# EpicDuckPotato/stereo_vo

Measured on AMD Instinct MI355X. Metric: stereo frames/sec on 1241x376 KITTI pairs, higher is better.
Workload: dtype u8/f32/f64; 1 GPU; kitti_1241x376_1500corners_5kf_window (BASELINE configs[1]); streams_per_gpu=96, max_corners=1500, window=5, pipeline_groups=3, hardware_queues=4

## Files before the change

### include/svo.h

```cpp
#ifndef SVO_H_
#define SVO_H_

#include <stddef.h>
#include <stdint.h>

#ifdef __cplusplus
extern "C" {
#endif

typedef enum svo_status {
  SVO_OK = 0,
  SVO_ERR_INVALID = -1,
  SVO_ERR_HIP = -2,
  SVO_ERR_CAPACITY = -3,
  SVO_ERR_NO_DEVICE = -4,
  SVO_ERR_NUMERIC = -5
} svo_status;

typedef struct svo_camera_info {
  double focal, cx, cy;
  double k1, k2, p1, p2;
  double baseline;
} svo_camera_info;

// ... 297 lines not shown
int svo_ba_set_bulk_control(svo_ba* ba, int mode);
int svo_ba_last_stats(svo_ba* ba, svo_lm_stats* stats);
int svo_ba_wave_chunks_limit(void);
int svo_ba_set_wave_chunks(svo_ba* ba, int k);
int svo_ba_solve_forms(svo_ba* ba, long* counts, int n, long* gave_up);
int svo_ba_set_yield_iterations(svo_ba* ba, int n);
int svo_ba_solve_problem(svo_ba* ba, svo_ba_summary* summary);
int svo_ba_solve_problems(svo_ba** bas, int n, svo_ba_summary* summaries);
int svo_ba_read_problem(svo_ba* ba, double* poses7, double* points3);

typedef struct svo_pipeline svo_pipeline;
typedef struct svo_pipeline_params {
  svo_camera_info cam;
  int width, height;
  int max_corners;
  double quality;
  float min_feature_distance;
  float parallax_thresh;
  int window_size;
  int max_features;
  int ba_max_iterations;
  double ba_max_time_s;
} svo_pipeline_params;

typedef struct svo_frame_result {
  int n_detected, n_tracked, n_inliers, n_new;
  int is_keyframe;
  float av_parallax, percent_lost;
  double pose7[7];
  int ba_iterations;
} svo_frame_result;

void svo_pipeline_default_params(svo_pipeline_params* p);
int svo_pipeline_create(svo_ctx* ctx, svo_pipeline** out, const svo_pipeline_params* p);
void svo_pipeline_destroy(svo_pipeline* p);
int svo_pipeline_reset(svo_pipeline* p);
int svo_pipeline_process_batch_dev(svo_pipeline* p, const uint8_t* left, const uint8_t* right,
                                   int batch, svo_frame_result* results);
int svo_pipeline_process_batch(svo_pipeline* p, const uint8_t* left, const uint8_t* right,
                               int batch, svo_frame_result* results);
int svo_pipeline_set_rectification(svo_pipeline* p, const svo_rectify_eye* left, const svo_rectify_eye* right);
int svo_pipeline_set_keyframe_clouds(svo_pipeline* p, const svo_cloud_params* params, int max_keyframes_per_call);
int svo_pipeline_set_keyframe_speckle_filter(svo_pipeline* p, const svo_speckle_params* params);
int svo_pipeline_set_keyframe_lr_check(svo_pipeline* p, const svo_lr_check_params* params);
int svo_pipeline_set_keyframe_sgm(svo_pipeline* p, const svo_sgm_params* params);
typedef struct svo_keyframe_cloud {
  int frame;
  int lane;
  int n_total, n_stored;
  const svo_cloud_point* dev;
} svo_keyframe_cloud;
int svo_pipeline_keyframe_clouds(svo_pipeline* p, int* n, const svo_keyframe_cloud** table);
int svo_pipeline_copy_keyframe_cloud(svo_pipeline* p, int i, svo_cloud_point* host, int capacity);
int svo_pipeline_keyframe_disparity(svo_pipeline* p, int i, const int16_t** dev);
int svo_pipeline_copy_keyframe_disparity(svo_pipeline* p, int i, int16_t* host);
int svo_pipeline_get_tracked(svo_pipeline* p, int64_t* ids, float* xy, int capacity, int* n);

typedef struct svo_pipeline_group svo_pipeline_group;
int svo_pipeline_group_create(svo_ctx* ctx, svo_pipeline_group** out, const svo_pipeline_params* p, int n_lanes);
void svo_pipeline_group_destroy(svo_pipeline_group* g);
int svo_pipeline_group_reset(svo_pipeline_group* g);
int svo_pipeline_group_lanes(const svo_pipeline_group* g);
int svo_pipeline_group_process_batch_dev(svo_pipeline_group* g, const uint8_t* left, const uint8_t* right, size_t lane_stride,
                                         int batch, svo_frame_result* results);
int svo_pipeline_group_staging(svo_pipeline_group* g, int slot, uint8_t** left, uint8_t** right, size_t* lane_stride);
int svo_pipeline_group_upload(svo_pipeline_group* g, int slot, int batch);
int svo_pipeline_group_process_uploaded(svo_pipeline_group* g, int slot, svo_frame_result* results);
int svo_pipeline_group_process_batch(svo_pipeline_group* g, const uint8_t* left, const uint8_t* right, size_t lane_stride,
                                     int batch, svo_frame_result* results);
int svo_pipeline_group_set_rectification(svo_pipeline_group* g, int lane, const svo_rectify_eye* left, const svo_rectify_eye* right);
int svo_pipeline_group_set_keyframe_clouds(svo_pipeline_group* g, int lane, const svo_cloud_params* params, int max_keyframes_per_call);
int svo_pipeline_group_set_keyframe_speckle_filter(svo_pipeline_group* g, const svo_speckle_params* params);
int svo_pipeline_group_set_keyframe_lr_check(svo_pipeline_group* g, const svo_lr_check_params* params);
int svo_pipeline_group_set_keyframe_sgm(svo_pipeline_group* g, const svo_sgm_params* params);
int svo_pipeline_group_keyframe_clouds(svo_pipeline_group* g, int* n, const svo_keyframe_cloud** table);
int svo_pipeline_group_copy_keyframe_cloud(svo_pipeline_group* g, int i, svo_cloud_point* host, int capacity);
int svo_pipeline_group_keyframe_disparity(svo_pipeline_group* g, int i, const int16_t** dev);
int svo_pipeline_group_copy_keyframe_disparity(svo_pipeline_group* g, int i, int16_t* host);
int svo_pipeline_group_get_tracked(svo_pipeline_group* g, int lane, int64_t* ids, float* xy, int capacity, int* n);
int svo_pipeline_group_last_stats(const svo_pipeline_group* g, long* launches6, long* lanes6);
int svo_pipeline_group_solve_work(svo_pipeline_group* g, double* out4, int reset);
int svo_pipeline_group_solve_forms(svo_pipeline_group* g, long* counts, int n, long* gave_up);
int svo_pipeline_group_set_solve_yield(svo_pipeline_group* g, int n);

int svo_draw_track(const uint8_t* gray, int width, int height, int row_stride, const float* from_xy,
                   const float* to_xy, int n, uint8_t* rgb);
int svo_pipeline_draw_track(svo_pipeline* p, const uint8_t* keyframe_gray, int row_stride, uint8_t* rgb);

typedef struct svo_synth_params {
  uint64_t seed;
  int width, height;
  double focal, cx, cy, baseline;
  double step_z, step_x, yaw_per_frame;
  int n_billboards;
} svo_synth_params;
void svo_synth_default_params(svo_synth_params* p, int width, int height);
int svo_synth_render(const svo_synth_params* p, int frame, uint8_t* left, uint8_t* right);
int svo_synth_pose(const svo_synth_params* p, int frame, double* rt12);

int svo_image_read_gray(const char* path, uint8_t* buf, size_t capacity, int* width, int* height);
int svo_kitti_read_poses(const char* poses_file, double* rt12, int capacity_frames, int* n_frames);
int svo_ate_rmse(const double* est_xyz, const double* gt_xyz, int n, int with_scale, double* rmse);
typedef struct svo_run_stats {
  int frames, keyframes;
  double ate_rmse;
  double seconds;
} svo_run_stats;
int svo_kitti_run(svo_ctx* ctx, const svo_pipeline_params* params, const char* data_path, int sequence,
                  int max_frames, double* traj_rt12, svo_run_stats* stats);

#ifdef __cplusplus
}
#endif
#endif
```

### stereo_vo_amd/api.py

```python
import ctypes as C
import os

import numpy as np

_HERE = os.path.dirname(os.path.abspath(__file__))
_LIB = None


class SvoError(RuntimeError):
    pass


def lib_path():
    return os.path.join(_HERE, "libsvo_hip.so")


class Limits(C.Structure):
    _fields_ = [("max_width", C.c_int), ("max_height", C.c_int), ("max_batch", C.c_int),
                ("max_corners", C.c_int), ("max_candidates", C.c_int), ("max_features", C.c_int)]


class CameraInfo(C.Structure):
    _fields_ = [(n, C.c_double) for n in ("focal", "cx", "cy", "k1", "k2", "p1", "p2", "baseline")]

# ... 270 lines not shown
    return {n: getattr(c, n) for n in REFERENCE_CONSTANT_NAMES}


class LmStats(C.Structure):
    _fields_ = [("linearize_calls", C.c_int), ("step_calls", C.c_int), ("speculations", C.c_int), ("speculation_hits", C.c_int),
                ("single_exchange", C.c_int), ("collectives", C.c_int), ("device_control", C.c_int), ("fallbacks", C.c_int),
                ("host_us", C.c_double)]


class LmStepCtl(C.Structure):
    _fields_ = [("cost", C.c_double), ("mcc", C.c_double), ("decrease_factor", C.c_double), ("spec_radius", C.c_double),
                ("chain", C.c_int)]


LM_LINEARIZE_FN = C.CFUNCTYPE(C.c_int, C.c_void_p, C.c_double, C.c_int, C.POINTER(C.c_double))
LM_STEP_FN = C.CFUNCTYPE(C.c_int, C.c_void_p, C.POINTER(C.c_double), C.POINTER(C.c_double), C.c_double, C.POINTER(LmStepCtl),
                         C.POINTER(C.c_double), C.POINTER(C.c_double), C.POINTER(C.c_double), C.POINTER(C.c_int))
LM_ACCEPT_FN = C.CFUNCTYPE(C.c_int, C.c_void_p)


class LmOps(C.Structure):
    _fields_ = [("user", C.c_void_p), ("linearize", LM_LINEARIZE_FN), ("step", LM_STEP_FN), ("accept", LM_ACCEPT_FN)]


def lm_decide_step(cost, mcc, radius, decrease_factor, cost_new, model_change_points):
    acc, rad = C.c_int(0), C.c_double(0.0)
    lib().svo_lm_decide_step(C.c_double(cost), C.c_double(mcc), C.c_double(radius), C.c_double(decrease_factor), C.c_double(cost_new),
                             C.c_double(model_change_points), C.byref(acc), C.byref(rad))
    return bool(acc.value), rad.value


def lm_solve(poses7, linearize, step, accept, max_iterations=50, max_time_s=0.0):
    poses = np.ascontiguousarray(poses7, np.float64).copy()
    K = poses.shape[0]
    n = 6 * (K - 1)
    pay1 = n * n + 3 * n + 2

    def _lin(user, radius, first, out):
        np.ctypeslib.as_array(out, shape=(pay1,))[:] = linearize(radius, first)
        return 0

    def _step(user, dc, cand, radius, ctl, out2, out1, out_radius, out_at_cand):
        d = np.ctypeslib.as_array(dc, shape=(max(n, 1),))[:n].copy()
        c = np.ctypeslib.as_array(cand, shape=(K, 7)).copy()
        p2, p1, nr, at_cand = step(d, c, radius, ctl.contents)
        np.ctypeslib.as_array(out2, shape=(4,))[:] = p2
        if p1 is not None:
            np.ctypeslib.as_array(out1, shape=(pay1,))[:] = p1
        out_radius[0] = nr if p1 is not None else 0.0
        out_at_cand[0] = int(bool(at_cand))
        return 0

    def _acc(user):
        accept()
        return 0
    ops = LmOps(None, LM_LINEARIZE_FN(_lin), LM_STEP_FN(_step), LM_ACCEPT_FN(_acc))
    opt = ba_default_options()
    opt.max_iterations, opt.max_time_s = max_iterations, max_time_s
    s, st = BASummary(), LmStats()
    rc = lib().svo_lm_solve(K, _p(poses), C.byref(ops), C.byref(opt), C.byref(s), C.byref(st))
    if rc:
        raise SvoError(f"svo_lm_solve failed ({rc})")
    return poses, s, st


ALLREDUCE_FN = C.CFUNCTYPE(C.c_int, C.c_void_p, C.c_size_t, C.c_void_p)

SYMBOLS = [
    "svo_create", "svo_destroy", "svo_last_error", "svo_stream", "svo_sync", "svo_version", "svo_reference_constants",
    "svo_profile_select", "svo_profile_read", "svo_measure_peak",
    "svo_reproj_eval", "svo_reproj_eval_dev",
    "svo_corner_detect", "svo_corner_detect_batch_dev", "svo_corner_response",
    "svo_stereo_bm", "svo_stereo_disparity_at", "svo_stereo_disparity_at_dev",
    "svo_triangulate", "svo_lk_track", "svo_build_pyramid", "svo_track_features", "svo_dedup",
    "svo_pnp_ransac",
    "svo_ba_default_options", "svo_ba_create", "svo_ba_destroy", "svo_ba_reset", "svo_ba_add_keyframe", "svo_ba_solve",
    "svo_ba_get_pose", "svo_ba_window_count", "svo_ba_get_points", "svo_ba_load_problem",
    "svo_ba_set_allreduce", "svo_ba_set_device_lm", "svo_ba_set_bulk_control", "svo_ba_set_solve_form", "svo_ba_wave_chunks_limit", "svo_ba_set_wave_chunks", "svo_ba_set_yield_iterations", "svo_ba_solve_forms", "svo_ba_solve_problem", "svo_ba_solve_problems", "svo_ba_read_problem", "svo_ba_set_comm", "svo_ba_last_stats", "svo_lm_solve", "svo_lm_decide_step",
    "svo_rccl_unique_id", "svo_rccl_comm_create", "svo_rccl_comm_destroy",
    "svo_pipeline_default_params", "svo_pipeline_create", "svo_pipeline_destroy", "svo_pipeline_reset",
    "svo_pipeline_process_batch_dev", "svo_pipeline_process_batch", "svo_pipeline_get_tracked",
    "svo_pipeline_group_create", "svo_pipeline_group_destroy", "svo_pipeline_group_reset", "svo_pipeline_group_lanes",
    "svo_pipeline_group_process_batch_dev", "svo_pipeline_group_get_tracked", "svo_pipeline_group_last_stats",
    "svo_pipeline_group_solve_work", "svo_pipeline_group_solve_forms", "svo_pipeline_group_set_solve_yield", "svo_pipeline_group_staging", "svo_pipeline_group_upload", "svo_pipeline_group_process_uploaded", "svo_pipeline_group_process_batch",
    "svo_synth_default_params", "svo_synth_render", "svo_synth_pose",
    "svo_image_read_gray", "svo_kitti_read_poses", "svo_ate_rmse", "svo_kitti_run", "svo_cholesky_solve", "svo_cholesky_solve_dev", "svo_draw_track", "svo_pipeline_draw_track",
    "svo_rectify_eye_from_camera_info", "svo_rectify_build_map", "svo_rectify_remap", "svo_rectify_remap_batch_dev",
    "svo_pipeline_set_rectification", "svo_pipeline_group_set_rectification",
    "svo_stereo_bm_batch_dev", "svo_cloud_default_params", "svo_disparity_cloud_batch_dev", "svo_stereo_cloud",
    "svo_pipeline_set_keyframe_clouds", "svo_pipeline_keyframe_clouds", "svo_pipeline_copy_keyframe_cloud",
    "svo_pipeline_group_set_keyframe_clouds", "svo_pipeline_group_keyframe_clouds", "svo_pipeline_group_copy_keyframe_cloud",
    "svo_speckle_workspace_bytes", "svo_disparity_speckle_filter_batch_dev", "svo_disparity_speckle_filter",
    "svo_pipeline_set_keyframe_speckle_filter", "svo_pipeline_group_set_keyframe_speckle_filter",
    "svo_stereo_bm_cost_batch_dev", "svo_disparity_lr_check_batch_dev", "svo_disparity_lr_check",
    "svo_pipeline_set_keyframe_lr_check", "svo_pipeline_group_set_keyframe_lr_check",
    "svo_sgm_default_params", "svo_sgm_workspace_bytes", "svo_stereo_sgm_batch_dev", "svo_stereo_sgm",
    "svo_pipeline_set_keyframe_sgm", "svo_pipeline_group_set_keyframe_sgm",
    "svo_voxel_map_default_params", "svo_voxel_map_bytes", "svo_voxel_map_create", "svo_voxel_map_destroy", "svo_voxel_map_clear",
    "svo_voxel_map_insert_dev", "svo_pose7_to_cam_to_world", "svo_voxel_map_insert_pose7_dev", "svo_voxel_map_stats",
    "svo_voxel_map_extract_dev", "svo_voxel_map_extract", "svo_voxel_map_download",
    "svo_voxel_carve_default_params", "svo_voxel_map_carve_dev", "svo_pose7_to_world_to_cam", "svo_voxel_map_carve_pose7_dev",
    "svo_voxel_map_carve", "svo_voxel_map_copy_live_dev", "svo_pipeline_keyframe_disparity", "svo_pipeline_group_keyframe_disparity",
    "svo_pipeline_copy_keyframe_disparity", "svo_pipeline_group_copy_keyframe_disparity",
    "svo_voxel_render_default_params", "svo_voxel_render_workspace_bytes", "svo_voxel_map_render_dev", "svo_voxel_map_render_pose7_dev",
    "svo_voxel_map_render", "svo_voxel_render_set_mode",
    "svo_voxel_map_remove_dev", "svo_voxel_map_remove_pose7_dev", "svo_voxel_map_remove_sync", "svo_voxel_map_move_dev", "svo_voxel_map_move_pose7_dev",
    "svo_voxel_ledger_bytes", "svo_voxel_ledger_create", "svo_voxel_ledger_destroy", "svo_voxel_ledger_insert_pose7_dev",
    "svo_voxel_ledger_update_pose7", "svo_voxel_ledger_retire", "svo_voxel_ledger_remove", "svo_voxel_ledger_ids", "svo_voxel_ledger_get",
]


def lib():
    global _LIB
    if _LIB is None:
        p = lib_path()
        if not os.path.exists(p):
            raise SvoError(f"{p} not built — run `python -c 'import __graft_entry__ as g; g.build()'`")
        L = C.CDLL(p)
        L.svo_version.restype = C.c_char_p
        L.svo_last_error.restype = C.c_char_p
        L.svo_last_error.argtypes = [C.c_void_p]
        L.svo_stream.restype = C.c_void_p
        L.svo_stream.argtypes = [C.c_void_p]
        L.svo_destroy.argtypes = [C.c_void_p]
        L.svo_destroy.restype = None
        vp, ci, sz = C.c_void_p, C.c_int, C.c_size_t
        L.svo_cloud_default_params.argtypes = [vp, ci, ci]
        L.svo_stereo_bm_batch_dev.argtypes = [vp, vp, vp, ci, ci, ci, ci, sz, ci, ci, vp]
        L.svo_disparity_cloud_batch_dev.argtypes = [vp, vp, vp, ci, ci, ci, ci, sz, vp, vp, vp, vp, vp]
        L.svo_stereo_cloud.argtypes = [vp, vp, vp, ci, ci, ci, ci, ci, vp, vp, vp, vp, vp, vp]
        L.svo_pipeline_set_keyframe_clouds.argtypes = [vp, vp, ci]
        L.svo_pipeline_keyframe_clouds.argtypes = [vp, vp, vp]
        L.svo_pipeline_copy_keyframe_cloud.argtypes = [vp, ci, vp, ci]
        L.svo_pipeline_group_set_keyframe_clouds.argtypes = [vp, ci, vp, ci]
        L.svo_pipeline_group_keyframe_clouds.argtypes = [vp, vp, vp]
        L.svo_pipeline_group_copy_keyframe_cloud.argtypes = [vp, ci, vp, ci]
        for f in ("svo_cloud_default_params", "svo_stereo_bm_batch_dev", "svo_disparity_cloud_batch_dev", "svo_stereo_cloud",
                  "svo_pipeline_set_keyframe_clouds", "svo_pipeline_keyframe_clouds", "svo_pipeline_copy_keyframe_cloud",
                  "svo_pipeline_group_set_keyframe_clouds", "svo_pipeline_group_keyframe_clouds", "svo_pipeline_group_copy_keyframe_cloud"):
            getattr(L, f).restype = ci
        L.svo_speckle_workspace_bytes.argtypes = [ci, ci, ci]
        L.svo_speckle_workspace_bytes.restype = sz
        L.svo_disparity_speckle_filter_batch_dev.argtypes = [vp, vp, ci, ci, ci, vp, vp, sz, vp]
        L.svo_disparity_speckle_filter.argtypes = [vp, vp, ci, ci, vp, vp]
        L.svo_pipeline_set_keyframe_speckle_filter.argtypes = [vp, vp]
        L.svo_pipeline_group_set_keyframe_speckle_filter.argtypes = [vp, vp]
        for f in ("svo_disparity_speckle_filter_batch_dev", "svo_disparity_speckle_filter", "svo_pipeline_set_keyframe_speckle_filter",
                  "svo_pipeline_group_set_keyframe_speckle_filter"):
            getattr(L, f).restype = ci
        L.svo_stereo_bm_cost_batch_dev.argtypes = [vp, vp, vp, ci, ci, ci, ci, sz, ci, ci, vp, vp]
        L.svo_disparity_lr_check_batch_dev.argtypes = [vp, vp, vp, ci, ci, ci, vp, vp]
        L.svo_disparity_lr_check.argtypes = [vp, vp, vp, ci, ci, vp, vp]
        L.svo_pipeline_set_keyframe_lr_check.argtypes = [vp, vp]
        L.svo_pipeline_group_set_keyframe_lr_check.argtypes = [vp, vp]
        for f in ("svo_stereo_bm_cost_batch_dev", "svo_disparity_lr_check_batch_dev", "svo_disparity_lr_check",
                  "svo_pipeline_set_keyframe_lr_check", "svo_pipeline_group_set_keyframe_lr_check"):
            getattr(L, f).restype = ci
        L.svo_sgm_default_params.argtypes = [vp, ci]
        L.svo_sgm_workspace_bytes.argtypes = [ci, ci, ci, ci, ci]
        L.svo_sgm_workspace_bytes.restype = sz
        L.svo_stereo_sgm_batch_dev.argtypes = [vp, vp, vp, ci, ci, ci, ci, sz, ci, ci, vp, vp, sz, vp, vp]
        L.svo_stereo_sgm.argtypes = [vp, vp, vp, ci, ci, ci, ci, ci, vp, vp, vp]
        L.svo_pipeline_set_keyframe_sgm.argtypes = [vp, vp]
        L.svo_pipeline_group_set_keyframe_sgm.argtypes = [vp, vp]
        for f in ("svo_sgm_default_params", "svo_stereo_sgm_batch_dev", "svo_stereo_sgm", "svo_pipeline_set_keyframe_sgm",
                  "svo_pipeline_group_set_keyframe_sgm"):
            getattr(L, f).restype = ci
# ... 818 lines not shown

    def close(self):
        if self.h:
            self.L.svo_pipeline_group_destroy(self.h)
            self.h = C.c_void_p()

    def __del__(self):
        try:
            self.close()
        except Exception:
            pass

    def reset(self):
        self.ctx._chk(self.L.svo_pipeline_group_reset(self.h), "svo_pipeline_group_reset")

    def set_rectification(self, lane, left=None, right=None):
        self.L.svo_pipeline_group_set_rectification.argtypes = [C.c_void_p, C.c_int, C.c_void_p, C.c_void_p]
        self.ctx._chk(self.L.svo_pipeline_group_set_rectification(self.h, lane, _ref(left), _ref(right)), "svo_pipeline_group_set_rectification")

    def set_keyframe_clouds(self, lane=-1, params=None, max_keyframes_per_call=0):
        if params is True:
            params = cloud_default_params(self.prm.width, self.prm.height)
        self.ctx._chk(self.L.svo_pipeline_group_set_keyframe_clouds(self.h, lane, _ref(params), max_keyframes_per_call),
                      "svo_pipeline_group_set_keyframe_clouds")

    def process_batch_dev(self, left_ptr, right_ptr, lane_stride, batch):
        res = (FrameResult * (self.n_lanes * batch))()
        self.ctx._chk(self.L.svo_pipeline_group_process_batch_dev(self.h, C.c_void_p(left_ptr), C.c_void_p(right_ptr), C.c_size_t(lane_stride),
                                                                  batch, res), "svo_pipeline_group_process_batch_dev")
        self.last_raw = bytes(res)
        return [list(res[l * batch:(l + 1) * batch]) for l in range(self.n_lanes)]

    def staging(self, slot):
        lp, rp, stride = C.POINTER(C.c_uint8)(), C.POINTER(C.c_uint8)(), C.c_size_t(0)
        self.L.svo_pipeline_group_staging.argtypes = [C.c_void_p, C.c_int, C.c_void_p, C.c_void_p, C.c_void_p]
        self.ctx._chk(self.L.svo_pipeline_group_staging(self.h, slot, C.byref(lp), C.byref(rp), C.byref(stride)), "svo_pipeline_group_staging")
        h, w = self.prm.height, self.prm.width
        mb = stride.value // (h * w)
        shape = (self.n_lanes, mb, h, w)
        n = self.n_lanes * mb * h * w
        return (np.ctypeslib.as_array(lp, shape=(n,)).reshape(shape), np.ctypeslib.as_array(rp, shape=(n,)).reshape(shape))

    def upload(self, slot, batch):
        self.ctx._chk(self.L.svo_pipeline_group_upload(self.h, slot, batch), "svo_pipeline_group_upload")

    def process_uploaded(self, slot, batch):
        res = (FrameResult * (self.n_lanes * batch))()
        self.L.svo_pipeline_group_process_uploaded.argtypes = [C.c_void_p, C.c_int, C.c_void_p]
        self.ctx._chk(self.L.svo_pipeline_group_process_uploaded(self.h, slot, res), "svo_pipeline_group_process_uploaded")
        self.last_raw = bytes(res)
        return [list(res[l * batch:(l + 1) * batch]) for l in range(self.n_lanes)]

    def process_batch(self, left, right):
        left, right = _u8(left), _u8(right)
        batch = left.shape[1]
        res = (FrameResult * (self.n_lanes * batch))()
        self.L.svo_pipeline_group_process_batch.argtypes = [C.c_void_p, C.c_void_p, C.c_void_p, C.c_size_t, C.c_int, C.c_void_p]
        self.ctx._chk(self.L.svo_pipeline_group_process_batch(self.h, _p(left), _p(right), C.c_size_t(batch * left.shape[2] * left.shape[3]), batch, res),
                      "svo_pipeline_group_process_batch")
        self.last_raw = bytes(res)
        return [list(res[l * batch:(l + 1) * batch]) for l in range(self.n_lanes)]

    def get_tracked(self, lane, capacity=8192):
        ids = np.empty(capacity, np.int64)
        xy = np.empty((capacity, 2), np.float32)
        n = C.c_int(0)
        self.ctx._chk(self.L.svo_pipeline_group_get_tracked(self.h, lane, _p(ids), _p(xy), capacity, C.byref(n)), "svo_pipeline_group_get_tracked")
        return ids[:n.value].copy(), xy[:n.value].copy()

    def solve_work(self, reset=False):
        out = (C.c_double * 4)()
        self.ctx._chk(self.L.svo_pipeline_group_solve_work(self.h, out, int(reset)), "svo_pipeline_group_solve_work")
        return list(out)

    def solve_forms(self):
        n = self.L.svo_ba_wave_chunks_limit() + 1
        out, gu = (C.c_long * n)(), C.c_long(0)
        self.ctx._chk(self.L.svo_pipeline_group_solve_forms(self.h, out, n, C.byref(gu)), "svo_pipeline_group_solve_forms")
        return list(out), gu.value

    def set_solve_yield(self, n):
        self.ctx._chk(self.L.svo_pipeline_group_set_solve_yield(self.h, int(n)), "svo_pipeline_group_set_solve_yield")

    def solve_resumes(self):
        n = self.L.svo_ba_wave_chunks_limit() + 2
        out = (C.c_long * n)()
        self.ctx._chk(self.L.svo_pipeline_group_solve_forms(self.h, out, n, None), "svo_pipeline_group_solve_forms")
        return out[n - 1]

    def last_stats(self):
        a, b = (C.c_long * 6)(), (C.c_long * 6)()
        self.ctx._chk(self.L.svo_pipeline_group_last_stats(self.h, a, b), "svo_pipeline_group_last_stats")
        return {s: (a[i], b[i]) for i, s in enumerate(self.STAGES) if s != "unused"}


class RunStats(C.Structure):
    _fields_ = [("frames", C.c_int), ("keyframes", C.c_int), ("ate_rmse", C.c_double), ("seconds", C.c_double)]


def image_read_gray(path, max_pixels=1 << 24):
    buf = np.empty(max_pixels, np.uint8)
    w, h = C.c_int(0), C.c_int(0)
    rc = lib().svo_image_read_gray(path.encode(), _p(buf), C.c_size_t(max_pixels), C.byref(w), C.byref(h))
    if rc:
        raise SvoError(f"svo_image_read_gray({path}) rc={rc}")
    return buf[:w.value * h.value].reshape(h.value, w.value).copy()


def kitti_read_poses(path, max_frames=100000):
    rt = np.empty((max_frames, 12))
    n = C.c_int(0)
    rc = lib().svo_kitti_read_poses(path.encode(), _p(rt), max_frames, C.byref(n))
    if rc:
        raise SvoError(f"svo_kitti_read_poses({path}) rc={rc}")
    return rt[:n.value].reshape(-1, 3, 4).copy()


def ate_rmse(est_xyz, gt_xyz, with_scale=False):
    est_xyz, gt_xyz = _f64(est_xyz), _f64(gt_xyz)
    out = C.c_double(0)
    rc = lib().svo_ate_rmse(_p(est_xyz), _p(gt_xyz), est_xyz.shape[0], int(with_scale), C.byref(out))
    if rc:
        raise SvoError(f"svo_ate_rmse rc={rc}")
    return out.value


def kitti_run(ctx, params, data_path, sequence, max_frames):
    traj = np.zeros((max_frames, 12))
    st = RunStats()
    ctx._chk(lib().svo_kitti_run(ctx.h, C.byref(params), data_path.encode(), sequence, max_frames, _p(traj), C.byref(st)),
             "svo_kitti_run")
    return traj[:st.frames].reshape(-1, 3, 4).copy(), st


def cholesky_solve(A, b):
    A = np.array(A, np.float64, order="C")
    b = np.array(b, np.float64)
    rc = lib().svo_cholesky_solve(_p(A), _p(b), b.shape[0])
    if rc != 0:
        raise SvoError(f"svo_cholesky_solve rc={rc}")
    return b


def draw_track(gray, from_xy, to_xy):
    g = np.ascontiguousarray(gray, np.uint8)
    a = np.ascontiguousarray(from_xy, np.float32).reshape(-1, 2)
    b = np.ascontiguousarray(to_xy, np.float32).reshape(-1, 2)
    out = np.empty(g.shape + (3,), np.uint8)
    rc = lib().svo_draw_track(_p(g), g.shape[1], g.shape[0], g.shape[1], _p(a), _p(b), a.shape[0], _p(out))
    if rc:
        raise SvoError(f"svo_draw_track rc={rc}")
    return out
```

### stereo_vo_amd/csrc/corner.hip

```cpp
#include "common.h"

namespace {
constexpr int SEL_THREADS = 1024;
constexpr int SEL_MAX_ACCEPT = 16384;
constexpr int SEL_CAP_K = 12288;
constexpr int SEL_CAP_C = 8192;
constexpr int SEL_LDS_BYTES = SEL_CAP_K * 8 + SEL_CAP_C * 2 + SEL_CAP_K + SEL_CAP_K * 2;
constexpr int NC_STRIDE = 32;

__device__ __forceinline__ unsigned f32_key(float v) {
  const unsigned b = __float_as_uint(v);
  return (b & 0x80000000u) ? ~b : (b | 0x80000000u);
}
__device__ __forceinline__ float key_f32(unsigned k) {
  return __uint_as_float((k & 0x80000000u) ? (k & 0x7fffffffu) : ~k);
}
__device__ __forceinline__ unsigned pack_xy(int x, int y) { return ((unsigned)y << 16) | (unsigned)x; }
__device__ __forceinline__ int key_x(unsigned lo) { return (int)(lo & 0xFFFFu); }
__device__ __forceinline__ int key_y(unsigned lo) { return (int)(lo >> 16); }
template <typename T>
__device__ __forceinline__ T ld_l2(const T* p) { return __hip_atomic_load(p, __ATOMIC_RELAXED, __HIP_MEMORY_SCOPE_AGENT); }
template <typename T>
__device__ __forceinline__ void st_l2(T* p, T v) { __hip_atomic_store(p, v, __ATOMIC_RELAXED, __HIP_MEMORY_SCOPE_AGENT); }
}

namespace {
constexpr int RS_COLS = 62;
constexpr int RS_ROWS = 48;
constexpr int RS_PF = 3;

__device__ __forceinline__ int wave_from_lower(int v) { return __builtin_amdgcn_mov_dpp(v, 0x138, 0xf, 0xf, false); }
__device__ __forceinline__ int wave_from_upper(int v) { return __builtin_amdgcn_mov_dpp(v, 0x130, 0xf, 0xf, false); }
__device__ __forceinline__ float wave_from_lower(float v) { return __int_as_float(wave_from_lower(__float_as_int(v))); }
__device__ __forceinline__ float wave_from_upper(float v) { return __int_as_float(wave_from_upper(__float_as_int(v))); }
}

__global__ __launch_bounds__(256) void corner_response_kernel(const uint8_t* __restrict__ imgs, int W, int H,
                                                              int row_stride, size_t image_stride,
                                                              float* __restrict__ eig,
                                                              unsigned* __restrict__ maxkey) {
  const int b = blockIdx.z;
  const uint8_t* img = imgs + (size_t)b * image_stride;
  const int lane = threadIdx.x & 63;
  const int ncs = (W + RS_COLS - 1) / RS_COLS, nrs = (H + RS_ROWS - 1) / RS_ROWS;
  const int wid = blockIdx.x * 4 + __builtin_amdgcn_readfirstlane(threadIdx.x >> 6);
  if (wid >= ncs * nrs) return;
  const int cs = wid % ncs, rs = wid / ncs;
  const int x = cs * RS_COLS - 1 + lane;
  const int y0 = rs * RS_ROWS, y1 = min(y0 + RS_ROWS, H);
  const int xr = reflect101(x, W);
  const int xe = reflect101(lane == 0 ? x - 1 : x + 1, W);
  const bool edge = lane == 0 || lane == 63;
  const bool fix_lo = x == -1, fix_hi = x == W;
  const bool border_wave = cs == 0 || (cs + 1) * RS_COLS - 1 + 1 >= W;
  const double scale = 1.0 / (4.0 * 3.0 * 255.0);
  const float k1 = (float)(1.0 * scale), k0 = (float)(2.0 * scale);
  float* E = eig + (size_t)b * W * H;
  const bool out_lane = lane >= 1 && lane <= RS_COLS && x < W;

  const int j0 = y0 > 0 ? y0 - 1 : 0, j1 = y1 < H ? y1 : H - 1;
  auto load_row = [&](int py, int& c, int& e) {
    const uint8_t* row = img + (size_t)reflect101(py, H) * row_stride;
    c = row[xr];
    e = edge ? (int)row[xe] : 0;
  };
  auto row_terms = [&](int c, int e, float& rdx, float& rdy) {
    int l = wave_from_lower(c), r = wave_from_upper(c);
    if (lane == 0) l = e;
    if (lane == 63) r = e;
    rdx = (float)(r - l);
    rdy = (float)c * k0 + (float)(l + r) * k1;
  };
  const int p_first = j0 - 1;
  const int p_last = j1 + 1;
  unsigned lmax = 0u;
  auto emit = [&](int y, const double* top, const double* mid, const double* bot) {
    const float a = (float)((top[0] + mid[0]) + bot[0]) * 0.5f;
    const float bq = (float)((top[1] + mid[1]) + bot[1]);
    const float c = (float)((top[2] + mid[2]) + bot[2]) * 0.5f;
    const float d = a - c;
    const float e = (a + c) - sqrtf(d * d + bq * bq);
    if (out_lane) {
      E[(size_t)y * W + x] = e;
      const unsigned k = f32_key(e);
      lmax = k > lmax ? k : lmax;
    }
  };
  auto step = [&](int p, int& c, int& e, float& dxA, float& dyA, float& dxB, float& dyB, float& dxC, float& dyC, double* HA,
                  double* HB, double* HC) {
    const int cc = c, ee = e;
    if (p + RS_PF <= p_last) load_row(p + RS_PF, c, e);
    row_terms(cc, ee, dxC, dyC);
    const int j = p - 1;
    if (j < j0) return;
    const float dx = (dxA + dxC) * k1 + dxB * k0;
    const float dy = dyC - dyA;
    float xx = dx * dx, xy = dx * dy, yy = dy * dy;
    if (border_wave) {
      const int src = fix_lo ? lane + 2 : lane - 2;
      const float x2 = __shfl(xx, src), y2 = __shfl(xy, src), z2 = __shfl(yy, src);
      if (fix_lo || fix_hi) { xx = x2; xy = y2; yy = z2; }
    }
    HC[0] = ((double)wave_from_lower(xx) + (double)xx) + (double)wave_from_upper(xx);
    HC[1] = ((double)wave_from_lower(xy) + (double)xy) + (double)wave_from_upper(xy);
    HC[2] = ((double)wave_from_lower(yy) + (double)yy) + (double)wave_from_upper(yy);
    const int y = j - 1;
    if (y < y0) return;
    if (y == 0) emit(0, HC, HB, HC);
    else emit(y, HA, HB, HC);
  };
  int c0, e0, c1, e1, c2, e2;
  load_row(p_first, c0, e0); load_row(p_first + 1, c1, e1); load_row(p_first + 2, c2, e2);
  float dx0 = 0.f, dy0 = 0.f, dx1 = 0.f, dy1 = 0.f, dx2 = 0.f, dy2 = 0.f;
  double h0[3] = {0, 0, 0}, h1[3] = {0, 0, 0}, h2[3] = {0, 0, 0};
  int p = p_first;
  for (; p + 2 <= p_last; p += 3) {
    step(p, c0, e0, dx1, dy1, dx2, dy2, dx0, dy0, h1, h2, h0);
    step(p + 1, c1, e1, dx2, dy2, dx0, dy0, dx1, dy1, h2, h0, h1);
    step(p + 2, c2, e2, dx0, dy0, dx1, dy1, dx2, dy2, h0, h1, h2);
  }
  double hp[3] = {h1[0], h1[1], h1[2]}, hl[3] = {h2[0], h2[1], h2[2]};
  if (p <= p_last) {
    step(p, c0, e0, dx1, dy1, dx2, dy2, dx0, dy0, h1, h2, h0);
    for (int q = 0; q < 3; ++q) { hp[q] = h2[q]; hl[q] = h0[q]; }
    ++p;
    if (p <= p_last) {
      step(p, c1, e1, dx2, dy2, dx0, dy0, dx1, dy1, h2, h0, h1);
      for (int q = 0; q < 3; ++q) { hp[q] = h0[q]; hl[q] = h1[q]; }
    }
  }
  if (j1 == H - 1 && y1 == H && H - 1 >= y0) emit(H - 1, hp, hl, hp);
  for (int off = 32; off > 0; off >>= 1) {
    const unsigned o = __shfl_xor(lmax, off);
    lmax = o > lmax ? o : lmax;
  }
  if (lane == 0 && lmax) atomicMax(&maxkey[b], lmax);
}


constexpr int RN_HALO = 2, RN_COLS = 64 - 2 * RN_HALO;
constexpr int RN_BUF = 320;
constexpr int NC_RAW = 16;

__global__ __launch_bounds__(256) void corner_response_nms_kernel(const uint8_t* __restrict__ imgs, int W, int H, int row_stride,
                                                                  size_t image_stride, unsigned* __restrict__ maxkey, double quality,
                                                                  unsigned long long* __restrict__ raw, size_t raw_stride ,
                                                                  int* __restrict__ ncand, int* __restrict__ status) {
  __shared__ unsigned long long sBuf[4][RN_BUF];
  const int b = blockIdx.z;
  const uint8_t* img = imgs + (size_t)b * image_stride;
  const int lane = threadIdx.x & 63, wave = __builtin_amdgcn_readfirstlane(threadIdx.x >> 6);
  const int ncs = (W + RN_COLS - 1) / RN_COLS, nrs = (H + RS_ROWS - 1) / RS_ROWS;
  const int wid = blockIdx.x * 4 + wave;
  if (wid >= ncs * nrs) return;
  const int cs = wid % ncs, rs = wid / ncs;
  const int x = cs * RN_COLS - RN_HALO + lane;
  const int y0 = rs * RS_ROWS, y1 = min(y0 + RS_ROWS, H);
  const int ey0 = y0 > 0 ? y0 - 1 : 0, ey1 = y1 < H ? y1 + 1 : H;
  const int xr = reflect101(x, W);
  const int xe = reflect101(lane == 0 ? x - 1 : x + 1, W);
  const bool edge = lane == 0 || lane == 63;
  const bool fix_lo = x == -1, fix_hi = x == W;
  const bool border_wave = cs == 0 || cs * RN_COLS - RN_HALO + 63 >= W;
  const double scale = 1.0 / (4.0 * 3.0 * 255.0);
  const float k1 = (float)(1.0 * scale), k0 = (float)(2.0 * scale);
  const bool test_lane = lane >= RN_HALO && lane < RN_HALO + RN_COLS && x >= 1 && x <= W - 2;
  unsigned long long* list = raw + (size_t)b * raw_stride;
  int* count = &ncand[b * NC_STRIDE + NC_RAW];
  unsigned long long* buf = sBuf[wave];
  int nbuf = 0;
  auto flush = [&]() {
    if (nbuf == 0) return;
    __builtin_amdgcn_fence(__ATOMIC_RELEASE, "workgroup");
    __builtin_amdgcn_wave_barrier();
    __builtin_amdgcn_fence(__ATOMIC_ACQUIRE, "workgroup");
    int base = 0;
    if (lane == 0) base = atomicAdd(count, nbuf);
    base = __builtin_amdgcn_readfirstlane(base);
    for (int i = lane; i < nbuf; i += 64) {
      if ((size_t)(base + i) < raw_stride) list[base + i] = buf[i];
      else atomicOr(status, 8);
    }
    __builtin_amdgcn_fence(__ATOMIC_RELEASE, "workgroup");
    __builtin_amdgcn_wave_barrier();
    __builtin_amdgcn_fence(__ATOMIC_ACQUIRE, "workgroup");
    nbuf = 0;
  };

  const int j0 = ey0 > 0 ? ey0 - 1 : 0, j1 = ey1 < H ? ey1 : H - 1;
  auto load_row = [&](int py, int& c, int& e) {
    const uint8_t* row = img + (size_t)reflect101(py, H) * row_stride;
    c = row[xr];
    e = edge ? (int)row[xe] : 0;
  };
  auto row_terms = [&](int c, int e, float& rdx, float& rdy) {
    int l = wave_from_lower(c), r = wave_from_upper(c);
    if (lane == 0) l = e;
    if (lane == 63) r = e;
    rdx = (float)(r - l);
    rdy = (float)c * k0 + (float)(l + r) * k1;
  };
  const int p_first = j0 - 1, p_last = j1 + 1;
  unsigned lmax = 0u;
  float thr_lb = (float)((double)key_f32(ld_l2(&maxkey[b])) * quality);
  if (!(thr_lb >= 0.0f)) thr_lb = 0.0f;
  float eA = 0.f, eB = 0.f;
  auto emit = [&](int y, const double* top, const double* mid, const double* bot) {
    const float a = (float)((top[0] + mid[0]) + bot[0]) * 0.5f;
    const float bq = (float)((top[1] + mid[1]) + bot[1]);
    const float c = (float)((top[2] + mid[2]) + bot[2]) * 0.5f;
    const float d = a - c;
    const float e = (a + c) - sqrtf(d * d + bq * bq);
    if (lane >= 1 && lane <= 62 && x >= 0 && x < W && y >= y0 && y < y1) {
      if (lane >= RN_HALO && lane < RN_HALO + RN_COLS) { const unsigned k = f32_key(e); lmax = k > lmax ? k : lmax; }
    }
    const int yt = y - 1;
    if (yt >= y0 && yt < y1 && yt >= 1 && yt <= H - 2) {
      const float m0 = fmaxf(fmaxf(wave_from_lower(eA), eA), wave_from_upper(eA));
      const float m2 = fmaxf(fmaxf(wave_from_lower(e), e), wave_from_upper(e));
      const float m1 = fmaxf(wave_from_lower(eB), wave_from_upper(eB));
      const bool cand = test_lane && eB > thr_lb && eB >= fmaxf(fmaxf(m0, m1), m2);
      const unsigned long long mask = __ballot(cand);
      if (mask) {
        if (cand) buf[nbuf + __popcll(mask & ((1ull << lane) - 1ull))] = ((unsigned long long)f32_key(eB) << 32) | pack_xy(x, yt);
        nbuf += __popcll(mask);
        if (nbuf > RN_BUF - 64) {
          flush();
          unsigned wm = lmax;
          for (int off = 32; off > 0; off >>= 1) { const unsigned o = __shfl_xor(wm, off); wm = o > wm ? o : wm; }
          const unsigned gm = ld_l2(&maxkey[b]);
          const float lb = (float)((double)key_f32(gm > wm ? gm : wm) * quality);
          if (lb > thr_lb) thr_lb = lb;
        }
      }
    }
    eA = eB; eB = e;
  };
  auto step = [&](int p, int& c, int& e, float& dxA, float& dyA, float& dxB, float& dyB, float& dxC, float& dyC, double* HA,
                  double* HB, double* HC) {
    const int cc = c, ee = e;
    if (p + RS_PF <= p_last) load_row(p + RS_PF, c, e);
    row_terms(cc, ee, dxC, dyC);
    const int j = p - 1;
    if (j < j0) return;
    const float dx = (dxA + dxC) * k1 + dxB * k0;
    const float dy = dyC - dyA;
    float xx = dx * dx, xy = dx * dy, yy = dy * dy;
    if (border_wave) {
      const int src = fix_lo ? lane + 2 : lane - 2;
      const float x2 = __shfl(xx, src), y2 = __shfl(xy, src), z2 = __shfl(yy, src);
      if (fix_lo || fix_hi) { xx = x2; xy = y2; yy = z2; }
    }
    HC[0] = ((double)wave_from_lower(xx) + (double)xx) + (double)wave_from_upper(xx);
    HC[1] = ((double)wave_from_lower(xy) + (double)xy) + (double)wave_from_upper(xy);
    HC[2] = ((double)wave_from_lower(yy) + (double)yy) + (double)wave_from_upper(yy);
    const int y = j - 1;
    if (y < ey0) return;
    if (y == 0) emit(0, HC, HB, HC);
    else emit(y, HA, HB, HC);
  };
  int c0, e0, c1, e1, c2, e2;
  load_row(p_first, c0, e0); load_row(p_first + 1, c1, e1); load_row(p_first + 2, c2, e2);
  float dx0 = 0.f, dy0 = 0.f, dx1 = 0.f, dy1 = 0.f, dx2 = 0.f, dy2 = 0.f;
  double h0[3] = {0, 0, 0}, h1[3] = {0, 0, 0}, h2[3] = {0, 0, 0};
  int p = p_first;
  for (; p + 2 <= p_last; p += 3) {
    step(p, c0, e0, dx1, dy1, dx2, dy2, dx0, dy0, h1, h2, h0);
    step(p + 1, c1, e1, dx2, dy2, dx0, dy0, dx1, dy1, h2, h0, h1);
    step(p + 2, c2, e2, dx0, dy0, dx1, dy1, dx2, dy2, h0, h1, h2);
  }
  double hp[3] = {h1[0], h1[1], h1[2]}, hl[3] = {h2[0], h2[1], h2[2]};
  if (p <= p_last) {
    step(p, c0, e0, dx1, dy1, dx2, dy2, dx0, dy0, h1, h2, h0);
    for (int q = 0; q < 3; ++q) { hp[q] = h2[q]; hl[q] = h0[q]; }
    ++p;
    if (p <= p_last) {
      step(p, c1, e1, dx2, dy2, dx0, dy0, dx1, dy1, h2, h0, h1);
      for (int q = 0; q < 3; ++q) { hp[q] = h0[q]; hl[q] = h1[q]; }
    }
  }
  if (j1 == H - 1 && ey1 == H && H - 1 >= ey0) emit(H - 1, hp, hl, hp);
  flush();
  for (int off = 32; off > 0; off >>= 1) {
    const unsigned o = __shfl_xor(lmax, off);
    lmax = o > lmax ? o : lmax;
  }
  if (lane == 0 && lmax) atomicMax(&maxkey[b], lmax);
}

__global__ __launch_bounds__(256) void corner_threshold_kernel(const unsigned long long* __restrict__ raw, size_t raw_stride,
                                                               const unsigned* __restrict__ maxkey, double quality,
                                                               unsigned long long* __restrict__ cand, int* __restrict__ ncand, int cap,
                                                               int* __restrict__ status) {
  const int b = blockIdx.z;
  const int n = min(ncand[b * NC_STRIDE + NC_RAW], (int)raw_stride);
  const float thr = (float)((double)key_f32(maxkey[b]) * quality);
  __shared__ int sCount, sBase;
  for (int i0 = blockIdx.x * 256; i0 < n; i0 += gridDim.x * 256) {
    if (threadIdx.x == 0) sCount = 0;
    __syncthreads();
    const int i = i0 + (int)threadIdx.x;
    unsigned long long e = 0;
    bool keep = false;
    if (i < n) {
      e = raw[(size_t)b * raw_stride + i];
      keep = key_f32((unsigned)(e >> 32)) > thr;
    }
    int local = 0;
    if (keep) local = atomicAdd(&sCount, 1);
    __syncthreads();
    if (threadIdx.x == 0 && sCount > 0) sBase = atomicAdd(&ncand[b * NC_STRIDE], sCount);
    __syncthreads();
    if (keep) {
      const int pos = sBase + local;
      if (pos < cap) cand[(size_t)b * cap + pos] = e;
      else atomicOr(status, 1);
    }
    __syncthreads();
  }
}

constexpr int NMS_ROWS = 8;
__global__ __launch_bounds__(256) void corner_nms_kernel(const float* __restrict__ eig, int W, int H,
                                                         const unsigned* __restrict__ maxkey, double quality,
                                                         unsigned long long* __restrict__ cand,
                                                         int* __restrict__ ncand, int cap, int* __restrict__ status) {
  const int b = blockIdx.z;
  const float* E = eig + (size_t)b * W * H;
  const float maxv = key_f32(maxkey[b]);
  const float thr = (float)((double)maxv * quality);
  const int x = blockIdx.x * 64 + (threadIdx.x & 63);
  const int yb = blockIdx.y * (4 * NMS_ROWS) + (threadIdx.x >> 6);
  __shared__ int sCount, sBase;
  if (threadIdx.x == 0) sCount = 0;
  __syncthreads();
  float val[NMS_ROWS];
  unsigned found = 0u;
#pragma unroll
  for (int k = 0; k < NMS_ROWS; ++k) {
    const int y = yb + 4 * k;
    val[k] = 0.f;
    if (x < 1 || x > W - 2 || y < 1 || y > H - 2) continue;
    const float c = E[(size_t)y * W + x];
    const float v = c > thr ? c : 0.0f;
    if (v == 0.0f) continue;
    float m = v;
#pragma unroll
    for (int j = -1; j <= 1; ++j)
#pragma unroll
      for (int i = -1; i <= 1; ++i) {
        const float nv = E[(size_t)(y + j) * W + (x + i)];
        const float t = nv > thr ? nv : 0.0f;
        m = t > m ? t : m;
      }
    if (v == m) { val[k] = v; found |= 1u << k; }
  }
  int local = 0;
  if (found) local = atomicAdd(&sCount, __popc(found));
  __syncthreads();
  if (threadIdx.x == 0 && sCount > 0) sBase = atomicAdd(&ncand[b * NC_STRIDE], sCount);
  __syncthreads();
  if (found) {
    int pos = sBase + local;
#pragma unroll
    for (int k = 0; k < NMS_ROWS; ++k) {
      if (!((found >> k) & 1u)) continue;
      if (pos < cap)
        cand[(size_t)b * cap + pos] = ((unsigned long long)f32_key(val[k]) << 32) | pack_xy(x, yb + 4 * k);
      else
        atomicOr(status, 1);
      ++pos;
    }
  }
}

__global__ __launch_bounds__(SEL_THREADS) void corner_select_kernel(
    const unsigned long long* __restrict__ cand, const int* __restrict__ ncand, int cap, int W, int H,
    float min_distance, int max_corners, int* __restrict__ cell_count, int* __restrict__ cell_start, int max_cells,
    unsigned long long* __restrict__ sorted, uint8_t* __restrict__ state_g, float* __restrict__ out_xy,
    int* __restrict__ out_n, int* __restrict__ status) {
  extern __shared__ __align__(16) unsigned char lds_raw[];
  unsigned long long* sKeys = reinterpret_cast<unsigned long long*>(lds_raw);
  __shared__ int sPart[SEL_THREADS];
  __shared__ int sFlag, sCount;
  const int b = blockIdx.x, tid = threadIdx.x;
  const unsigned long long* C = cand + (size_t)b * cap;
  int n = ncand[b * NC_STRIDE];
  if (n > cap) n = cap;
  float* oxy = out_xy + (size_t)b * max_corners * 2;
  if (min_distance < 1.0f) {
    if (n > SEL_MAX_ACCEPT) { if (tid == 0) { atomicOr(status, 2); out_n[b] = 0; } return; }
    int np2 = 1; while (np2 < n) np2 <<= 1;
    for (int i = tid; i < np2; i += SEL_THREADS) sKeys[i] = i < n ? C[i] : 0ull;
    __syncthreads();
    for (int k = 2; k <= np2; k <<= 1)
      for (int j = k >> 1; j > 0; j >>= 1) {
        for (int i = tid; i < np2; i += SEL_THREADS) {
          const int l = i ^ j;
          if (l > i) {
            const unsigned long long a = sKeys[i], c = sKeys[l];
            const bool desc = (i & k) == 0;
            if (desc ? a < c : a > c) { sKeys[i] = c; sKeys[l] = a; }
          }
        }
        __syncthreads();
      }
    const int m = n < max_corners ? n : max_corners;
    for (int i = tid; i < m; i += SEL_THREADS) {
      const unsigned idx = (unsigned)(sKeys[i] & 0xffffffffu);
      oxy[2 * i] = (float)key_x(idx); oxy[2 * i + 1] = (float)key_y(idx);
    }
    if (tid == 0) out_n[b] = m;
    return;
  }
  const int cell = (int)rintf(min_distance);
  const int gw = (W + cell - 1) / cell, gh = (H + cell - 1) / cell;
  const int ncell = gw * gh;
  int* cc = cell_count + (size_t)b * max_cells;
  int* cs = cell_start + (size_t)b * (max_cells + 1);
  unsigned long long* S = sorted + (size_t)b * cap;
  uint8_t* st = state_g + (size_t)b * cap;
  if (ncell > max_cells) { if (tid == 0) { atomicOr(status, 4); out_n[b] = 0; } return; }
  unsigned long long* keysL = reinterpret_cast<unsigned long long*>(lds_raw);
  unsigned short* cellL = reinterpret_cast<unsigned short*>(lds_raw + (size_t)SEL_CAP_K * 8);
  uint8_t* stateL = lds_raw + (size_t)SEL_CAP_K * 8 + (size_t)SEL_CAP_C * 2;
  unsigned short* blkL = reinterpret_cast<unsigned short*>(lds_raw + (size_t)SEL_CAP_K * 8 + (size_t)SEL_CAP_C * 2 + SEL_CAP_K);
  const bool use_lds = n <= SEL_CAP_K && ncell + 1 <= SEL_CAP_C;
  if (use_lds) {
    static_assert(3 * SEL_CAP_K >= 4 * SEL_CAP_C, "the cell counters must fit the state + blocker arrays");
    int* cntL = reinterpret_cast<int*>(stateL);
    for (int i = tid; i < ncell; i += SEL_THREADS) cntL[i] = 0;
    __syncthreads();
    for (int i = tid; i < n; i += SEL_THREADS) {
      const unsigned idx = (unsigned)(C[i] & 0xffffffffu);
      atomicAdd(&cntL[(key_y(idx) / cell) * gw + key_x(idx) / cell], 1);
    }
    __syncthreads();
    {
      const int chunk = (ncell + SEL_THREADS - 1) / SEL_THREADS;
      const int lo = tid * chunk, hi = (lo + chunk < ncell) ? lo + chunk : ncell;
      int s = 0;
      for (int i = lo; i < hi; ++i) s += cntL[i];
      sPart[tid] = s;
      __syncthreads();
      for (int off = 1; off < SEL_THREADS; off <<= 1) {
        int v = tid >= off ? sPart[tid - off] : 0;
        __syncthreads();
        sPart[tid] += v;
        __syncthreads();
      }
      int run = sPart[tid] - s;
      for (int i = lo; i < hi; ++i) { cellL[i] = (unsigned short)run; run += cntL[i]; }
      if (tid == 0) cellL[ncell] = (unsigned short)n;
    }
    __syncthreads();
    for (int i = tid; i < n; i += SEL_THREADS) {
      const unsigned long long k = C[i];
      const unsigned idx = (unsigned)(k & 0xffffffffu);
      const int cid = (key_y(idx) / cell) * gw + key_x(idx) / cell;
      const int slot = atomicSub(&cntL[cid], 1) - 1;
      keysL[(int)cellL[cid] + slot] = k;
    }
    __syncthreads();
    for (int i = tid; i < n; i += SEL_THREADS) { stateL[i] = 0; blkL[i] = 0xFFFFu; }
    __syncthreads();
  } else {
  for (int i = tid; i < ncell; i += SEL_THREADS) st_l2(&cc[i], 0);
  __syncthreads();
// ... 100 lines not shown
      for (int yy = y1; yy <= y2 && !rejected; ++yy) {
        const int p0 = CELL(yy * gw + x1), p1 = CELL(yy * gw + x2 + 1);
        for (int p = p0; p < p1; ++p) {
          const unsigned long long km = KEY(p);
          if (km <= k) continue;
          const unsigned im = (unsigned)(km & 0xffffffffu);
          const float dx = (float)(x - key_x(im)), dy = (float)(y - key_y(im));
          if (!(dx * dx + dy * dy < md2)) continue;
          const uint8_t sm = STATE(p);
          if (sm == 1) { rejected = true; break; }
          if (sm == 0) blocked = true;
        }
      }
      if (rejected) SET_STATE(i, (uint8_t)2);
      else if (!blocked) SET_STATE(i, (uint8_t)1);
      else pending = 1;
    }
    }
    }
    if (pending) sFlag = 1;
    __syncthreads();
    const int again = sFlag;
    __syncthreads();
    if (!again) break;
  }
  if (tid == 0) sCount = 0;
  __syncthreads();
  int A, np2 = 1;
  if (use_lds) {
    constexpr int PER = SEL_CAP_K / SEL_THREADS;
    unsigned long long mine[PER];
    int cnt = 0;
#pragma unroll
    for (int r = 0; r < PER; ++r) {
      const int i = tid + r * SEL_THREADS;
      const bool acc = i < n && stateL[i] == 1;
      mine[r] = acc ? keysL[i] : 0ull;
      cnt += acc;
    }
    __syncthreads();
    int pos = cnt ? atomicAdd(&sCount, cnt) : 0;
    __syncthreads();
    A = sCount;
    while (np2 < A) np2 <<= 1;
#pragma unroll
    for (int r = 0; r < PER; ++r) if (mine[r]) sKeys[pos++] = mine[r];
    for (int i = A + tid; i < np2; i += SEL_THREADS) sKeys[i] = 0ull;
    __syncthreads();
  } else {
    unsigned long long* Cw = const_cast<unsigned long long*>(C);
    for (int i = tid; i < n; i += SEL_THREADS) {
      if (STATE(i) == 1) {
        const int p = atomicAdd(&sCount, 1);
        if (p < SEL_MAX_ACCEPT) st_l2(&Cw[p], KEY(i));
      }
    }
    __syncthreads();
    A = sCount;
    if (A > SEL_MAX_ACCEPT) { if (tid == 0) { atomicOr(status, 2); out_n[b] = 0; } return; }
    while (np2 < A) np2 <<= 1;
    for (int i = tid; i < np2; i += SEL_THREADS) sKeys[i] = i < A ? ld_l2(&Cw[i]) : 0ull;
    __syncthreads();
  }
  for (int k = 2; k <= np2; k <<= 1)
    for (int j = k >> 1; j > 0; j >>= 1) {
      for (int i = tid; i < np2; i += SEL_THREADS) {
        const int l = i ^ j;
        if (l > i) {
          const unsigned long long a = sKeys[i], c = sKeys[l];
          const bool desc = (i & k) == 0;
          if (desc ? a < c : a > c) { sKeys[i] = c; sKeys[l] = a; }
        }
      }
      __syncthreads();
    }
  const int m = A < max_corners ? A : max_corners;
  for (int i = tid; i < m; i += SEL_THREADS) {
    const unsigned idx = (unsigned)(sKeys[i] & 0xffffffffu);
    oxy[2 * i] = (float)key_x(idx); oxy[2 * i + 1] = (float)key_y(idx);
  }
  if (tid == 0) out_n[b] = m;
}

static int corner_launch(svo_ctx* ctx, const uint8_t* imgs, int batch, int W, int H, int row_stride,
                         size_t image_stride, int max_corners, double quality, double min_distance,
                         float* xy, int* n) {
  SVO_REQUIRE(ctx, W <= 65535 && H <= 65535, "corner_detect: image sides above 65535 (candidate keys pack y << 16 | x)");
  hipStream_t st = ctx->stream;
  SVO_HIP_CHECK(ctx, hipMemsetAsync(ctx->d_maxkey, 0, sizeof(unsigned) * batch, st));
  SVO_HIP_CHECK(ctx, hipMemsetAsync(ctx->d_ncand, 0, sizeof(int) * NC_STRIDE * batch, st));
  static const bool two_pass = [] { const char* e = getenv("SVO_CORNER_TWO_PASS"); return e && *e && atoi(e) != 0; }();
  if (two_pass) {
    { const int rce = svo_ensure_eig(ctx, (size_t)ctx->lim.max_batch); if (rce) return rce; }
    {
      SvoProfScope prof(ctx, SVO_PROF_CORNER_RESPONSE);
      hipLaunchKernelGGL(corner_response_kernel, dim3(svo_div_up(svo_div_up(W, RS_COLS) * svo_div_up(H, RS_ROWS), 4), 1, batch), dim3(256), 0, st,
                         imgs, W, H, row_stride, image_stride, ctx->d_eig, ctx->d_maxkey);
    }
    SvoProfScope prof(ctx, SVO_PROF_CORNER_NMS);
    hipLaunchKernelGGL(corner_nms_kernel, dim3(svo_div_up(W, 64), svo_div_up(H, 4 * NMS_ROWS), batch), dim3(256), 0, st,
                       ctx->d_eig, W, H, ctx->d_maxkey, quality, ctx->d_cand, ctx->d_ncand, ctx->lim.max_candidates,
                       ctx->d_status);
  } else {
    unsigned long long* raw = ctx->d_raw;
    const size_t raw_stride = ctx->raw_cap;
    {
      SvoProfScope prof(ctx, SVO_PROF_CORNER_RESPONSE);
      hipLaunchKernelGGL(corner_response_nms_kernel, dim3(svo_div_up(svo_div_up(W, RN_COLS) * svo_div_up(H, RS_ROWS), 4), 1, batch), dim3(256), 0, st,
                         imgs, W, H, row_stride, image_stride, ctx->d_maxkey, quality, raw, raw_stride, ctx->d_ncand, ctx->d_status);
    }
    SvoProfScope prof(ctx, SVO_PROF_CORNER_NMS);
    hipLaunchKernelGGL(corner_threshold_kernel, dim3(32, 1, batch), dim3(256), 0, st, raw, raw_stride, ctx->d_maxkey, quality, ctx->d_cand,
                       ctx->d_ncand, ctx->lim.max_candidates, ctx->d_status);
  }
  static bool attr_set = false;
  if (!attr_set) {
    SVO_HIP_CHECK(ctx, hipFuncSetAttribute((const void*)corner_select_kernel,
                                           hipFuncAttributeMaxDynamicSharedMemorySize, SEL_LDS_BYTES));
    attr_set = true;
  }
  SvoProfScope ps(ctx, SVO_PROF_CORNER_SELECT);
  hipLaunchKernelGGL(corner_select_kernel, dim3(batch), dim3(SEL_THREADS), SEL_LDS_BYTES, st, ctx->d_cand,
                     ctx->d_ncand, ctx->lim.max_candidates, W, H, (float)min_distance, max_corners,
                     ctx->d_cell_count, ctx->d_cell_start, ctx->max_cells, ctx->d_sorted, ctx->d_state, xy, n,
                     ctx->d_status);
  SVO_HIP_CHECK(ctx, hipGetLastError());
  return SVO_OK;
}

static int corner_check_args(svo_ctx* ctx, const void* img, int batch, int W, int H, int row_stride,
                             int max_corners, const void* xy, const void* n) {
  if (!ctx) return SVO_ERR_INVALID;
  svo_use_device(ctx);
  SVO_REQUIRE(ctx, img && xy && n, "corner_detect: null buffer");
  SVO_REQUIRE(ctx, W >= 3 && H >= 3 && W <= ctx->lim.max_width && H <= ctx->lim.max_height && row_stride >= W,
              "corner_detect: image size outside the limits given to svo_create");
  SVO_REQUIRE(ctx, batch >= 1 && batch <= ctx->lim.max_batch, "corner_detect: batch outside limits");
  SVO_REQUIRE(ctx, max_corners >= 1, "corner_detect: max_corners must be >= 1");
  return SVO_OK;
}

static int corner_status(svo_ctx* ctx) {
  int* h = (int*)ctx->h_pinned;
  SVO_HIP_CHECK(ctx, hipMemcpyAsync(h, ctx->d_status, sizeof(int), hipMemcpyDeviceToHost, ctx->stream));
  SVO_HIP_CHECK(ctx, hipStreamSynchronize(ctx->stream));
  if (*h) {
    const int s = *h;
    (void)hipMemsetAsync(ctx->d_status, 0, sizeof(int), ctx->stream);
    ctx->err = (s & 1)   ? "corner_detect: more NMS candidates than svo_limits.max_candidates"
               : (s & 8) ? "corner_detect: more raw local maxima than the streaming pass's list holds (svo_ctx raw_cap: width x height / 4 per image under a 1 GiB budget)"
               : (s & 2) ? "corner_detect: more accepted corners than the select kernel holds (16384)"
                         : "corner_detect: min-distance grid larger than the workspace";
    return SVO_ERR_CAPACITY;
  }
  return SVO_OK;
}

extern "C" int svo_corner_detect_batch_dev(svo_ctx* ctx, const uint8_t* imgs, int batch, int width, int height,
                                           int row_stride, size_t image_stride, int max_corners, double quality,
                                           double min_distance, float* xy, int* n) {
  int rc = corner_check_args(ctx, imgs, batch, width, height, row_stride, max_corners, xy, n);
  if (rc) return rc;
  return corner_launch(ctx, imgs, batch, width, height, row_stride, image_stride, max_corners, quality,
                       min_distance, xy, n);
}

extern "C" int svo_corner_detect(svo_ctx* ctx, const uint8_t* img, int width, int height, int row_stride,
                                 int max_corners, double quality, double min_distance, float* xy, int* n) {
  int rc = corner_check_args(ctx, img, 1, width, height, row_stride, max_corners, xy, n);
  if (rc) return rc;
  SvoScratch s(ctx);
  uint8_t* d_img = s.take<uint8_t>((size_t)width * height);
  float* d_xy = s.take<float>(2 * (size_t)max_corners);
  int* d_n = s.take<int>(1);
  if (!d_img || !d_xy || !d_n) { ctx->err = "corner_detect: workspace too small"; return SVO_ERR_CAPACITY; }
  hipStream_t st = ctx->stream;
  SVO_HIP_CHECK(ctx, hipMemcpy2DAsync(d_img, width, img, row_stride, width, height, hipMemcpyHostToDevice, st));
  rc = corner_launch(ctx, d_img, 1, width, height, width, (size_t)width * height, max_corners, quality,
                     min_distance, d_xy, d_n);
  if (rc) return rc;
  SVO_HIP_CHECK(ctx, hipMemcpyAsync(n, d_n, sizeof(int), hipMemcpyDeviceToHost, st));
  rc = corner_status(ctx);
  if (rc) return rc;
  if (*n > 0) SVO_HIP_CHECK(ctx, hipMemcpy(xy, d_xy, sizeof(float) * 2 * (size_t)*n, hipMemcpyDeviceToHost));
  return SVO_OK;
}

extern "C" int svo_corner_response(svo_ctx* ctx, const uint8_t* img, int width, int height, int row_stride,
                                   float* eig) {
  if (!ctx) return SVO_ERR_INVALID;
  svo_use_device(ctx);
  SVO_REQUIRE(ctx, img && eig, "corner_response: null buffer");
  SVO_REQUIRE(ctx, width >= 3 && height >= 3 && width <= ctx->lim.max_width && height <= ctx->lim.max_height,
              "corner_response: image size outside limits");
  SvoScratch s(ctx);
  uint8_t* d_img = s.take<uint8_t>((size_t)width * height);
  if (!d_img) { ctx->err = "corner_response: workspace too small"; return SVO_ERR_CAPACITY; }
  hipStream_t st = ctx->stream;
  SVO_HIP_CHECK(ctx, hipMemcpy2DAsync(d_img, width, img, row_stride, width, height, hipMemcpyHostToDevice, st));
  { const int rce = svo_ensure_eig(ctx, 1); if (rce) return rce; }
  SVO_HIP_CHECK(ctx, hipMemsetAsync(ctx->d_maxkey, 0, sizeof(unsigned), st));
  hipLaunchKernelGGL(corner_response_kernel, dim3(svo_div_up(svo_div_up(width, RS_COLS) * svo_div_up(height, RS_ROWS), 4), 1, 1), dim3(256), 0,
                     st, d_img, width, height, width, (size_t)width * height, ctx->d_eig, ctx->d_maxkey);
  SVO_HIP_CHECK(ctx, hipGetLastError());
  SVO_HIP_CHECK(ctx, hipMemcpyAsync(eig, ctx->d_eig, sizeof(float) * (size_t)width * height, hipMemcpyDeviceToHost, st));
  SVO_HIP_CHECK(ctx, hipStreamSynchronize(st));
  return SVO_OK;
}
```

### stereo_vo_amd/csrc/kernels.h

```cpp
#ifndef SVO_KERNELS_H_
#define SVO_KERNELS_H_
#include "common.h"

struct SvoMat4 { float m[16]; };

SvoMat4 svo_k_reprojection_matrix(const float* pose16, float focal, float cx, float cy, float baseline);
SvoMat4 svo_k_reprojection_q(float focal, float cx, float cy, float baseline);
int svo_k_triangulate(svo_ctx* ctx, const float* xy, const float* disp, const int* n_dev, int n_max,
                      const SvoMat4& M, float* kept_xy, float* xyz, int* kept_index, int* n_kept,
                      const SvoPublish* pub = nullptr);
int svo_k_stereo_triangulate(svo_ctx* ctx, const uint8_t* left, const uint8_t* right, int width, int height, int row_stride,
                             int num_disparities, int block_size, const float* xy, const int* n_dev, int n_max, float* disp,
                             const SvoMat4& M, float* kept_xy, float* xyz, int* kept_index, int* n_kept, int word, SvoPublish* pub_out);
int svo_k_dedup(svo_ctx* ctx, const float* det_xy, const int* n_det_dev, int n_det_max, const float* trk_xy,
                const int* n_trk_dev, int n_trk_max, float min_distance, float* kept_xy, int* n_kept);
size_t svo_k_pyramid_bytes(int w, int h);
int svo_k_build_pyramid(svo_ctx* ctx, const uint8_t* imgs, int batch, int w, int h, int row_stride,
                        size_t image_stride, uint8_t* pyr, size_t pyr_stride, bool level0_in_place = false);
int svo_k_pyramid_level0(svo_ctx* ctx, const uint8_t* imgs, int batch, int w, int h, int row_stride, size_t image_stride, uint8_t* pyr,
                         size_t pyr_stride, hipStream_t st);
struct SvoTrackCarry {
  const float* init_src = nullptr; const long long* ids_src = nullptr;
  float* init_dst = nullptr; long long* ids_dst = nullptr;
  int* host_n = nullptr; float* host_av = nullptr;
  float* host_xy = nullptr; long long* host_ids = nullptr;
  SvoPublish pub;
};
int svo_k_track(svo_ctx* ctx, const uint8_t* pyr_prev, const uint8_t* pyr_next, int w, int h, const float* xy,
                const float* initial_xy, const int* n_dev, int n_max, float* fwd_xy, uint8_t* keep_flag,
                float* parallax, float* kept_xy, int* kept_index, int* n_kept, float* av_parallax,
                const SvoTrackCarry* carry = nullptr);
int svo_k_lk(svo_ctx* ctx, const uint8_t* pyr_prev, const uint8_t* pyr_next, int w, int h, const float* xy,
             int n, float* out_xy, uint8_t* status);
int svo_k_gather_track(svo_ctx* ctx, const int* idx, const int* n_dev, int n_max, const float* init_src,
                       const long long* ids_src, float* init_dst, long long* ids_dst);
int svo_k_tracker_init(svo_ctx* ctx, const float* h_xy, const float* h_init, const long long* h_ids, int n, float* d_xy, float* d_init,
                       long long* d_ids, const SvoPublish* pub);
int svo_k_gather_xy_ids(svo_ctx* ctx, const int* idx, int n, const float* xy_src, const long long* ids_src,
                        float* xy_dst, long long* ids_dst);
int svo_k_pnp(svo_ctx* ctx, SvoScratch& s, const float* d_xyz, const float* d_xy, int n, float focal, float cx, float cy,
              double* rvec3, double* tvec3, int iterations, float reproj_err, double confidence, int* d_inliers,
              int* n_inliers, int* h_inliers = nullptr ,
              float* d_inlier_xy = nullptr );
constexpr int SVO_RECT_MAX_LANES = 64;
constexpr int SVO_RECT_SENTINEL = (int)0x80008000u;
struct SvoRectifyArgs {
  const uint8_t* src[2];
  uint8_t* dst[2];
  size_t src_lane_stride, src_image_stride, dst_lane_stride, dst_image_stride;
  int src_row_stride, width, height, frames, eyes, n_active;
  const int* map[SVO_RECT_MAX_LANES][2];
  unsigned char lane[SVO_RECT_MAX_LANES];
};
int svo_k_rectify_remap(svo_ctx* ctx, const SvoRectifyArgs& a, hipStream_t st);
struct SvoRectModel {
  svo_rectify_eye eye[2];
  int* d_map[2] = {nullptr, nullptr};
  int refs = 0;
};
int svo_rect_model_create(svo_ctx* ctx, const svo_rectify_eye* left, const svo_rectify_eye* right, const svo_camera_info* cam,
                          int width, int height, SvoRectModel** out);
void svo_rect_model_destroy(SvoRectModel* m);
struct SvoCloudPair { const uint8_t* left; const uint8_t* right; };
struct SvoDensePairs {
  const uint8_t* left;
  const uint8_t* right;
  size_t image_stride;
  const SvoCloudPair* tab;
};
int svo_k_stereo_dense_batch(svo_ctx* ctx, const SvoDensePairs& src, int batch, int W, int H, int stride, int ndisp, int block, int16_t* disp16,
                             uint16_t* cost16 = nullptr);
int svo_k_cloud(svo_ctx* ctx, const int16_t* disp16, const SvoDensePairs& src, int batch, int W, int H, int stride, const svo_camera_info* cam,
                const float* pose16, const svo_cloud_params* prm, svo_cloud_point* points, int* counts, int* seg);
int svo_k_speckle(svo_ctx* ctx, int16_t* disp16, int batch, int W, int H, const svo_speckle_params* prm, void* workspace, int* n_removed);
int svo_k_lr_check(svo_ctx* ctx, int16_t* disp16, const uint16_t* cost16, int batch, int W, int H, const svo_lr_check_params* prm, int* n_removed);
int svo_k_stereo_sgm(svo_ctx* ctx, const SvoDensePairs& src, int batch, int W, int H, int stride, int ndisp, int block,
                     const svo_sgm_params* prm, void* workspace, int16_t* disp16, uint16_t* cost16);
struct SvoKfClouds;
int svo_kfc_create(svo_ctx* ctx, const svo_cloud_params* params, int W, int H, int max_keyframes, SvoKfClouds** out);
void svo_kfc_destroy(SvoKfClouds* k);
int svo_kfc_replace(svo_ctx* ctx, SvoKfClouds** slot, const svo_cloud_params* params, int W, int H, int max_keyframes);
const svo_cloud_params* svo_kfc_params(const SvoKfClouds* k);
int svo_kfc_max_keyframes(const SvoKfClouds* k);
void svo_kfc_clear(SvoKfClouds* k);
int svo_kfc_set_speckle(SvoKfClouds* k, const svo_speckle_params* prm);
int svo_kfc_set_lr_check(SvoKfClouds* k, const svo_lr_check_params* prm);
int svo_kfc_set_sgm(SvoKfClouds* k, const svo_sgm_params* prm);
int svo_kfc_run(SvoKfClouds* k, const svo_camera_info* cam, const SvoCloudPair* pairs, const int* frame, const int* lane, int n);
int svo_kfc_table(SvoKfClouds* k, int* n, const svo_keyframe_cloud** table);
int svo_kfc_copy(SvoKfClouds* k, int i, svo_cloud_point* host, int capacity);
int svo_kfc_disparity(SvoKfClouds* k, int i, const int16_t** dev);
int svo_kfc_copy_disparity(SvoKfClouds* k, int i, int16_t* host);
const char* svo_rectify_error_text();
#endif
```

### stereo_vo_amd/csrc/lk.hip

```cpp
#include "kernels.h"
#include "group_kernels.h"
#include "tail_device.h"

namespace {
#include "ref_constants.h"
#ifndef SVO_LK_MAX_ITER
#define SVO_LK_MAX_ITER svo_ref::LK_MAX_ITERATIONS
#endif
constexpr int WIN = svo_ref::LK_WIN, HALF = WIN / 2, LEVELS = svo_ref::LK_MAX_LEVEL + 1, MAX_ITER = SVO_LK_MAX_ITER;
static_assert(WIN == 21 && LEVELS == 4, "the LDS layout and the exact-sum bounds below are derived for a 21x21 window, 4 levels");
constexpr int G = WIN + 1;
constexpr int RP = WIN + 3;
constexpr float MIN_EIG = svo_ref::LK_MIN_EIG_THRESHOLD;
constexpr double LK_EPS = svo_ref::LK_EPSILON;
constexpr float FLT_SCALE = 1.0f / (float)(1 << 20);
constexpr float FLT_EPS = 1.1920928955078125e-7f;

struct Pyr {
  const uint8_t* base;
  const uint8_t* l0;
  int w0, h0;
};

__device__ __forceinline__ Pyr make_pyr(const uint8_t* base, int w, int h, const uint8_t* l0 = nullptr) { return Pyr{base, l0 ? l0 : base, w, h}; }
// ... 369 lines not shown
    const float A11 = (float)(double)sA[0] * FLT_SCALE;
    const float A12 = (float)(double)sA[1] * FLT_SCALE;
    const float A22 = (float)(double)sA[2] * FLT_SCALE;
    float D = A11 * A22 - A12 * A12;
    const float dif = A11 - A22;
    const float minEig = (A22 + A11 - sqrtf(dif * dif + 4.f * A12 * A12)) / (float)(2 * WIN * WIN);
    if (minEig < MIN_EIG || D < FLT_EPS) {
      if (level == 0) status = 0;
      continue;
    }
    D = 1.f / D;
    float outx = nx, outy = ny;
    nx -= (float)HALF; ny -= (float)HALF;
    float pdx = 0.f, pdy = 0.f;
    int rx0 = 0, ry0 = 0;
    bool staged = false;
    const uint32_t* jw = reinterpret_cast<const uint32_t*>(S.jreg);
    for (int j = 0; j < MAX_ITER; ++j) {
      const int inx = __builtin_amdgcn_readfirstlane((int)floorf(nx)), iny = __builtin_amdgcn_readfirstlane((int)floorf(ny));
      if (inx < -WIN || inx >= Jw_ || iny < -WIN || iny >= Jh_) {
        if (level == 0) status = 0;
        break;
      }
      a = nx - (float)inx; b = ny - (float)iny;
      iw00 = __float2int_rn((1.f - a) * (1.f - b) * (float)(1 << 14));
      iw01 = __float2int_rn(a * (1.f - b) * (float)(1 << 14));
      iw10 = __float2int_rn((1.f - a) * b * (float)(1 << 14));
      iw11 = (1 << 14) - iw00 - iw01 - iw10;
      if (!staged || inx < rx0 || inx > rx0 + 2 * RM || iny < ry0 || iny > ry0 + 2 * RM) {
        rx0 = inx - RM; ry0 = iny - RM;
        lk_sync();
        stage_tile<RS, RS * RS>(S.jreg, Jp, Jw_, Jh_, rx0, ry0, lane);
        lk_sync();
        staged = true;
      }
      const int base = (iny - ry0 + r) * RS + (inx - rx0) + c0;
      const int wi = base >> 2, sh = base & 3;
      const uint32_t u0 = jw[wi], u1 = jw[wi + 1], u2 = jw[wi + 2];
      const uint32_t v0 = jw[wi + RS / 4], v1 = jw[wi + RS / 4 + 1], v2 = jw[wi + RS / 4 + 2];
      const uint32_t tl = __builtin_amdgcn_alignbyte(u1, u0, sh), th = __builtin_amdgcn_alignbyte(u2, u1, sh);
      const uint32_t bl = __builtin_amdgcn_alignbyte(v1, v0, sh), bh = __builtin_amdgcn_alignbyte(v2, v1, sh);
      const lk_s2 wtop = pack_s2(iw00, iw01), wbot = pack_s2(iw10, iw11);
      int diff[8];
#pragma unroll
      for (int p = 0; p < 7; ++p) {
        const uint32_t sel = 0x0c000c00u | ((uint32_t)(p + 1) << 16) | (uint32_t)p;
        const lk_s2 tp = __builtin_bit_cast(lk_s2, __builtin_amdgcn_perm(th, tl, sel)), bp = __builtin_bit_cast(lk_s2, __builtin_amdgcn_perm(bh, bl, sel));
        diff[p] = __builtin_amdgcn_sdot2(tp, wtop, __builtin_amdgcn_sdot2(bp, wbot, tI[p], false), false) >> 9;
      }
      diff[7] = 0;
      int pb[2] = {0, 0};
#pragma unroll
      for (int q = 3; q >= 0; --q) {
        const lk_s2 d = pack_s2(diff[2 * q], diff[2 * q + 1]);
        pb[0] = __builtin_amdgcn_sdot2(d, tXp[q], pb[0], false);
        pb[1] = __builtin_amdgcn_sdot2(d, tYp[q], pb[1], false);
      }
      const float b1 = wave_sum_f32(pb[0]) * FLT_SCALE;
      const float b2 = wave_sum_f32(pb[1]) * FLT_SCALE;
      const float dx = (A12 * b2 - A22 * b1) * D;
      const float dy = (A12 * b1 - A11 * b2) * D;
      nx += dx; ny += dy;
      outx = nx + (float)HALF; outy = ny + (float)HALF;
      if (step_below_eps(dx, dy)) break;
      if (j > 0 && ((int)below_eps(dx + pdx) & (int)below_eps(dy + pdy))) {
        outx -= dx * 0.5f; outy -= dy * 0.5f;
        break;
      }
      pdx = dx; pdy = dy;
    }
    nx = outx; ny = outy;
    if (status && level == 0) {
      const float fx = nx - (float)HALF, fy = ny - (float)HALF;
      const int ix = (int)floorf(fx), iy = (int)floorf(fy);
      if (ix < -WIN || ix >= Jw_ || iy < -WIN || iy >= Jh_) status = 0;
    }
  }
  *ox = nx; *oy = ny;
  return status;
}
}

__global__ __launch_bounds__(256) void pyr_copy_kernel(const uint8_t* __restrict__ imgs, int w, int h, int row_stride,
                                                       size_t image_stride, uint8_t* __restrict__ pyr, size_t pyr_stride) {
  const int x = blockIdx.x * 64 + (threadIdx.x & 63), y = blockIdx.y * 4 + (threadIdx.x >> 6);
  if (x >= w || y >= h) return;
  pyr[(size_t)blockIdx.z * pyr_stride + (size_t)y * w + x] = imgs[(size_t)blockIdx.z * image_stride + (size_t)y * row_stride + x];
}

__global__ __launch_bounds__(256) void pyr_down_kernel(uint8_t* __restrict__ pyr, size_t pyr_stride, size_t src_off, int sw,
                                                       int sh, size_t dst_off, int dw, int dh, const uint8_t* __restrict__ src_imgs,
                                                       size_t src_image_stride, int src_row_stride) {
  const int x = blockIdx.x * 64 + (threadIdx.x & 63), y = blockIdx.y * 4 + (threadIdx.x >> 6);
  if (x >= dw || y >= dh) return;
  const uint8_t* src = src_imgs ? src_imgs + (size_t)blockIdx.z * src_image_stride : pyr + (size_t)blockIdx.z * pyr_stride + src_off;
  const int k[5] = {1, 4, 6, 4, 1};
  int s = 0;
#pragma unroll
  for (int j = 0; j < 5; ++j) {
    const uint8_t* row = src + (size_t)reflect101(2 * y + j - 2, sh) * (src_imgs ? src_row_stride : sw);
    int r = 0;
#pragma unroll
    for (int i = 0; i < 5; ++i) r += k[i] * row[reflect101(2 * x + i - 2, sw)];
    s += k[j] * r;
  }
  pyr[(size_t)blockIdx.z * pyr_stride + dst_off + (size_t)y * dw + x] = (uint8_t)((s + 128) >> 8);
}

constexpr int PB_T1W = 128, PB_T1H = 64;
constexpr int PB_R0W = 2 * PB_T1W + 21, PB_R0H = 2 * PB_T1H + 21;
constexpr int PB_R1W = PB_T1W + 9, PB_R1H = PB_T1H + 9;
constexpr int PB_R2W = PB_T1W / 2 + 3, PB_R2H = PB_T1H / 2 + 3;
constexpr int PB_P0 = 280, PB_P1 = 140, PB_P2 = 68;
__global__ __launch_bounds__(256) void pyr_build_kernel(const uint8_t* __restrict__ imgs, size_t image_stride, int row_stride, int w0, int h0,
                                                        uint8_t* __restrict__ pyr, size_t pyr_stride, int tiles_x, int tiles_y, int n_images) {
  __shared__ __align__(16) uint8_t s0[PB_R0H * PB_P0];
  __shared__ __align__(16) uint8_t s1[PB_R1H * PB_P1];
  __shared__ __align__(16) uint8_t s2[PB_R2H * PB_P2];
  const int per_img = tiles_x * tiles_y, total = per_img * n_images;
  const int per_xcd = (total + 7) >> 3, v = ((int)blockIdx.x & 7) * per_xcd + ((int)blockIdx.x >> 3);
  if (v >= total) return;
  const int img = v / per_img, t = v - img * per_img, ty = t / tiles_x, tx = t - ty * tiles_x;
  const int w1 = (w0 + 1) >> 1, h1 = (h0 + 1) >> 1, w2 = (w1 + 1) >> 1, h2 = (h1 + 1) >> 1, w3 = (w2 + 1) >> 1, h3 = (h2 + 1) >> 1;
  const int x0lo = max(0, 2 * PB_T1W * tx - 14), x0hi = min(w0 - 1, 2 * PB_T1W * tx + 2 * PB_T1W + 6);
  const int y0lo = max(0, 2 * PB_T1H * ty - 14), y0hi = min(h0 - 1, 2 * PB_T1H * ty + 2 * PB_T1H + 6);
  const int x1lo = max(0, PB_T1W * tx - 6), x1hi = min(w1 - 1, PB_T1W * tx + PB_T1W + 2);
  const int y1lo = max(0, PB_T1H * ty - 6), y1hi = min(h1 - 1, PB_T1H * ty + PB_T1H + 2);
  const int x2lo = max(0, PB_T1W / 2 * tx - 2), x2hi = min(w2 - 1, PB_T1W / 2 * tx + PB_T1W / 2);
  const int y2lo = max(0, PB_T1H / 2 * ty - 2), y2hi = min(h2 - 1, PB_T1H / 2 * ty + PB_T1H / 2);
  const uint8_t* src = imgs + (size_t)img * image_stride;
  uint8_t* dst = pyr + (size_t)img * pyr_stride;
  const size_t off1 = (size_t)w0 * h0, off2 = off1 + (size_t)w1 * h1, off3 = off2 + (size_t)w2 * h2;
  {
    const int rw = x0hi - x0lo + 1, rh = y0hi - y0lo + 1, dw = rw >> 2;
    for (int i = threadIdx.x; i < rh * dw; i += 256) {
      const int r = i / dw, c = i - r * dw;
      uint32_t val;
      __builtin_memcpy(&val, src + (size_t)(y0lo + r) * row_stride + x0lo + 4 * c, 4);
      *reinterpret_cast<uint32_t*>(&s0[r * PB_P0 + 4 * c]) = val;
    }
    const int tail = rw - 4 * dw;
    for (int i = threadIdx.x; i < rh * tail; i += 256) {
      const int r = i / tail, c = 4 * dw + (i - r * tail);
      s0[r * PB_P0 + c] = src[(size_t)(y0lo + r) * row_stride + x0lo + c];
    }
  }
  __syncthreads();
  const int k5[5] = {1, 4, 6, 4, 1};
  {
    const int rw = x1hi - x1lo + 1, rh = y1hi - y1lo + 1;
    for (int i = threadIdx.x; i < rw * rh; i += 256) {
      const int ry = i / rw, rx = i - ry * rw, x = x1lo + rx, y = y1lo + ry;
      int sum = 0;
#pragma unroll
      for (int j = 0; j < 5; ++j) {
        const uint8_t* row = &s0[(reflect101(2 * y + j - 2, h0) - y0lo) * PB_P0];
        int r = 0;
#pragma unroll
        for (int q = 0; q < 5; ++q) r += k5[q] * row[reflect101(2 * x + q - 2, w0) - x0lo];
        sum += k5[j] * r;
      }
      const uint8_t o = (uint8_t)((sum + 128) >> 8);
      s1[ry * PB_P1 + rx] = o;
      if (x >= PB_T1W * tx && x < PB_T1W * tx + PB_T1W && y >= PB_T1H * ty && y < PB_T1H * ty + PB_T1H) dst[off1 + (size_t)y * w1 + x] = o;
    }
  }
  __syncthreads();
  {
    const int rw = x2hi - x2lo + 1, rh = y2hi - y2lo + 1;
    for (int i = threadIdx.x; i < rw * rh; i += 256) {
      const int ry = i / rw, rx = i - ry * rw, x = x2lo + rx, y = y2lo + ry;
      int sum = 0;
#pragma unroll
      for (int j = 0; j < 5; ++j) {
        const uint8_t* row = &s1[(reflect101(2 * y + j - 2, h1) - y1lo) * PB_P1];
        int r = 0;
#pragma unroll
        for (int q = 0; q < 5; ++q) r += k5[q] * row[reflect101(2 * x + q - 2, w1) - x1lo];
        sum += k5[j] * r;
      }
      const uint8_t o = (uint8_t)((sum + 128) >> 8);
      s2[ry * PB_P2 + rx] = o;
      if (x >= PB_T1W / 2 * tx && x < PB_T1W / 2 * tx + PB_T1W / 2 && y >= PB_T1H / 2 * ty && y < PB_T1H / 2 * ty + PB_T1H / 2) dst[off2 + (size_t)y * w2 + x] = o;
    }
  }
  __syncthreads();
  {
    const int x3lo = PB_T1W / 4 * tx, y3lo = PB_T1H / 4 * ty, rw = min(w3, x3lo + PB_T1W / 4) - x3lo, rh = min(h3, y3lo + PB_T1H / 4) - y3lo;
    for (int i = threadIdx.x; i < rw * rh; i += 256) {
      const int ry = i / rw, rx = i - ry * rw, x = x3lo + rx, y = y3lo + ry;
      int sum = 0;
#pragma unroll
      for (int j = 0; j < 5; ++j) {
        const uint8_t* row = &s2[(reflect101(2 * y + j - 2, h2) - y2lo) * PB_P2];
        int r = 0;
#pragma unroll
        for (int q = 0; q < 5; ++q) r += k5[q] * row[reflect101(2 * x + q - 2, w2) - x2lo];
        sum += k5[j] * r;
      }
      dst[off3 + (size_t)y * w3 + x] = (uint8_t)((sum + 128) >> 8);
    }
  }
}

__global__ __launch_bounds__(LKT * FPB) void lk_kernel(const uint8_t* __restrict__ pyrA, const uint8_t* __restrict__ pyrB, int w,
// ... 100 lines not shown
  }
  if (lane == 0) {
    *a.host_n = base;
    *a.host_av = n > 0 ? sum / (float)n : 0.f;
  }
  __builtin_amdgcn_fence(__ATOMIC_RELEASE, "");
  if (lane == 0) __hip_atomic_store(a.word, a.seq, __ATOMIC_RELAXED, __HIP_MEMORY_SCOPE_SYSTEM);
}

__global__ __launch_bounds__(1024) void track_compact_kernel(const float* __restrict__ fwd, const uint8_t* __restrict__ keep,
                                                             const float* __restrict__ parallax, const int* __restrict__ n_dev,
                                                             int n_host, float* __restrict__ kept_xy, int* __restrict__ kept_index,
                                                             int* __restrict__ n_kept, float* __restrict__ av_parallax,
                                                             SvoTrackCarry carry) {
  svo_latency_critical();
  __shared__ int sWave[16];
  __shared__ __align__(16) float sPar[4096];
  const int n = n_dev ? *n_dev : n_host;
  const int lane = threadIdx.x & 63, wave = threadIdx.x >> 6;
  int base = 0;
  for (int c0 = 0; c0 < n; c0 += 1024) {
    const int i = c0 + threadIdx.x;
    const bool k = i < n && keep[i];
    if (i < 4096) sPar[i] = k ? parallax[i] : 0.0f;
    const unsigned long long mask = __ballot(k);
    if (lane == 0) sWave[wave] = __popcll(mask);
    __syncthreads();
    int off = 0, total = 0;
    for (int w = 0; w < 16; ++w) { const int c = sWave[w]; if (w < wave) off += c; total += c; }
    if (k) {
      const int slot = base + off + __popcll(mask & ((1ull << lane) - 1ull));
      kept_xy[2 * slot] = fwd[2 * i]; kept_xy[2 * slot + 1] = fwd[2 * i + 1];
      kept_index[slot] = i;
      if (carry.init_src) {
        carry.init_dst[2 * slot] = carry.init_src[2 * i]; carry.init_dst[2 * slot + 1] = carry.init_src[2 * i + 1];
        const long long id = carry.ids_src[i];
        carry.ids_dst[slot] = id;
        if (carry.host_xy) { carry.host_xy[2 * slot] = fwd[2 * i]; carry.host_xy[2 * slot + 1] = fwd[2 * i + 1]; carry.host_ids[slot] = id; }
      }
    }
    base += total;
    __syncthreads();
  }
  float sum = 0.f;
  for (int c0 = 0; c0 < n; c0 += 4096) {
    if (c0 > 0) {
      __syncthreads();
      for (int i = threadIdx.x; i < 4096 && c0 + i < n; i += 1024) sPar[i] = keep[c0 + i] ? parallax[c0 + i] : 0.0f;
      __syncthreads();
    }
    if (threadIdx.x == 0) {
      const int m = n - c0 < 4096 ? n - c0 : 4096;
      int i = 0;
      for (; i + 32 <= m; i += 32) {
        float4 q[8];
#pragma unroll
        for (int u = 0; u < 8; ++u) q[u] = *reinterpret_cast<const float4*>(&sPar[i + 4 * u]);
#pragma unroll
        for (int u = 0; u < 8; ++u) { sum += q[u].x; sum += q[u].y; sum += q[u].z; sum += q[u].w; }
      }
      for (; i < m; ++i) sum += sPar[i];
    }
  }
  if (threadIdx.x == 0) {
    const float av = n > 0 ? sum / (float)n : 0.f;
    *n_kept = base;
    *av_parallax = av;
    if (carry.host_n) {
      *carry.host_n = base;
      *carry.host_av = av;
    }
  }
  svo_publish_block(carry.pub);
}

size_t svo_k_pyramid_bytes(int w, int h) {
  size_t s = 0;
  for (int l = 0; l < LEVELS; ++l) { s += (size_t)w * h; w = (w + 1) / 2; h = (h + 1) / 2; }
  return s;
}

int svo_k_build_pyramid(svo_ctx* ctx, const uint8_t* imgs, int batch, int w, int h, int row_stride, size_t image_stride,
                        uint8_t* pyr, size_t pyr_stride, bool level0_in_place) {
  hipStream_t st = ctx->stream;
  if (!level0_in_place)
    hipLaunchKernelGGL(pyr_copy_kernel, dim3(svo_div_up(w, 64), svo_div_up(h, 4), batch), dim3(256), 0, st, imgs, w, h,
                       row_stride, image_stride, pyr, pyr_stride);
  static const bool per_level = [] { const char* e = getenv("SVO_PYR_PER_LEVEL"); return e && *e && atoi(e) != 0; }();
  if (LEVELS == 4 && !per_level && w >= 64 && h >= 64) {
    const int w1 = (w + 1) / 2, h1 = (h + 1) / 2, tiles_x = svo_div_up(w1, PB_T1W), tiles_y = svo_div_up(h1, PB_T1H);
    const long long total = (long long)tiles_x * tiles_y * batch;
    if (total > 0 && total < (1ll << 30)) {
      SvoProfScope prof(ctx, SVO_PROF_PYR_DOWN);
      hipLaunchKernelGGL(pyr_build_kernel, dim3((unsigned)(8 * ((total + 7) / 8))), dim3(256), 0, st, imgs, image_stride, row_stride, w, h, pyr, pyr_stride,
                         tiles_x, tiles_y, batch);
      SVO_HIP_CHECK(ctx, hipGetLastError());
      return SVO_OK;
    }
  }
  size_t src_off = 0;
  int sw = w, sh = h;
  for (int l = 1; l < LEVELS; ++l) {
    const size_t dst_off = src_off + (size_t)sw * sh;
    const int dw = (sw + 1) / 2, dh = (sh + 1) / 2;
    SvoProfScope prof(ctx, SVO_PROF_PYR_DOWN);
    const bool from_images = level0_in_place && l == 1;
    hipLaunchKernelGGL(pyr_down_kernel, dim3(svo_div_up(dw, 64), svo_div_up(dh, 4), batch), dim3(256), 0, st, pyr, pyr_stride,
                       src_off, sw, sh, dst_off, dw, dh, from_images ? imgs : (const uint8_t*)nullptr, image_stride, row_stride);
    src_off = dst_off; sw = dw; sh = dh;
  }
  SVO_HIP_CHECK(ctx, hipGetLastError());
  return SVO_OK;
}

int svo_k_pyramid_level0(svo_ctx* ctx, const uint8_t* imgs, int batch, int w, int h, int row_stride, size_t image_stride, uint8_t* pyr,
                         size_t pyr_stride, hipStream_t st) {
  hipLaunchKernelGGL(pyr_copy_kernel, dim3(svo_div_up(w, 64), svo_div_up(h, 4), batch), dim3(256), 0, st, imgs, w, h, row_stride, image_stride,
                     pyr, pyr_stride);
  SVO_HIP_CHECK(ctx, hipGetLastError());
  return SVO_OK;
}

int svo_k_lk(svo_ctx* ctx, const uint8_t* pyr_prev, const uint8_t* pyr_next, int w, int h, const float* xy, int n,
             float* out_xy, uint8_t* status) {
  if (n <= 0) return SVO_OK;
  hipLaunchKernelGGL(lk_kernel, dim3(svo_div_up(n, FPB)), dim3(LKT * FPB), 0, ctx->stream, pyr_prev, pyr_next, w, h, xy, n, out_xy, status);
  SVO_HIP_CHECK(ctx, hipGetLastError());
  return SVO_OK;
}

int svo_k_track(svo_ctx* ctx, const uint8_t* pyr_prev, const uint8_t* pyr_next, int w, int h, const float* xy,
                const float* initial_xy, const int* n_dev, int n_max, float* fwd_xy, uint8_t* keep_flag, float* parallax,
                float* kept_xy, int* kept_index, int* n_kept, float* av_parallax, const SvoTrackCarry* carry) {
  if (n_max > 0) {
    SvoProfScope prof(ctx, SVO_PROF_LK_FB);
    hipLaunchKernelGGL(lk_fb_kernel, dim3(svo_div_up(n_max, FPB)), dim3(LKT * FPB), 0, ctx->stream, pyr_prev, pyr_next, w, h, xy, initial_xy, n_dev,
                       n_max, fwd_xy, keep_flag, parallax);
  }
  hipLaunchKernelGGL(track_compact_kernel, dim3(1), dim3(1024), 0, ctx->stream, fwd_xy, keep_flag, parallax, n_dev, n_max,
                     kept_xy, kept_index, n_kept, av_parallax, carry ? *carry : SvoTrackCarry{});
  SVO_HIP_CHECK(ctx, hipGetLastError());
  return SVO_OK;
}

int svo_kg_track(svo_ctx* ctx, hipStream_t st, const SvoLkLanes& lanes, int n_lanes, int grid_x) {
  SvoProfScope prof(ctx, SVO_PROF_LK_FB, st);
  if (lanes.map.per_chunk > 0) hipLaunchKernelGGL(lk_fb_group_kernel, dim3(lanes.map.grid()), dim3(64), 0, st, lanes);
  else hipLaunchKernelGGL(lk_fb_group_kernel, dim3(grid_x, n_lanes), dim3(64), 0, st, lanes);
  SVO_HIP_CHECK(ctx, hipGetLastError());
  return SVO_OK;
}

static int lk_check(svo_ctx* ctx, const void* a, const void* b, int w, int h, int stride) {
  if (!ctx) return SVO_ERR_INVALID;
  svo_use_device(ctx);
  SVO_REQUIRE(ctx, a && b, "lk: null image");
  SVO_REQUIRE(ctx, w >= 8 && h >= 8 && w <= ctx->lim.max_width && h <= ctx->lim.max_height && stride >= w,
              "lk: image size outside limits");
  return SVO_OK;
}

extern "C" int svo_build_pyramid(svo_ctx* ctx, const uint8_t* img, int width, int height, int row_stride, uint8_t* levels,
                                 size_t levels_bytes) {
  int rc = lk_check(ctx, img, levels, width, height, row_stride);
  if (rc) return rc;
  const size_t pb = svo_k_pyramid_bytes(width, height);
  SVO_REQUIRE(ctx, levels_bytes >= pb, "build_pyramid: output buffer too small");
  SvoScratch s(ctx);
  uint8_t* dI = s.take<uint8_t>((size_t)width * height);
  uint8_t* dP = s.take<uint8_t>(pb);
  if (!dI || !dP) { ctx->err = "build_pyramid: workspace too small"; return SVO_ERR_CAPACITY; }
  hipStream_t st = ctx->stream;
  SVO_HIP_CHECK(ctx, hipMemcpy2DAsync(dI, width, img, row_stride, width, height, hipMemcpyHostToDevice, st));
  rc = svo_k_build_pyramid(ctx, dI, 1, width, height, width, (size_t)width * height, dP, pb);
  if (rc) return rc;
  SVO_HIP_CHECK(ctx, hipMemcpyAsync(levels, dP, pb, hipMemcpyDeviceToHost, st));
  SVO_HIP_CHECK(ctx, hipStreamSynchronize(st));
  return SVO_OK;
}

static int lk_upload(svo_ctx* ctx, SvoScratch& s, const uint8_t* prev, const uint8_t* next, int w, int h, int stride,
                     uint8_t** pA, uint8_t** pB) {
  const size_t pb = svo_k_pyramid_bytes(w, h);
  uint8_t* dI = s.take<uint8_t>(2 * (size_t)w * h);
  uint8_t* dP = s.take<uint8_t>(2 * pb);
  if (!dI || !dP) { ctx->err = "lk: workspace too small"; return SVO_ERR_CAPACITY; }
  hipStream_t st = ctx->stream;
  SVO_HIP_CHECK(ctx, hipMemcpy2DAsync(dI, w, prev, stride, w, h, hipMemcpyHostToDevice, st));
  SVO_HIP_CHECK(ctx, hipMemcpy2DAsync(dI + (size_t)w * h, w, next, stride, w, h, hipMemcpyHostToDevice, st));
  int rc = svo_k_build_pyramid(ctx, dI, 2, w, h, w, (size_t)w * h, dP, pb);
  if (rc) return rc;
  *pA = dP; *pB = dP + pb;
  return SVO_OK;
}

extern "C" int svo_lk_track(svo_ctx* ctx, const uint8_t* prev, const uint8_t* next, int width, int height, int row_stride,
                            const float* xy, int n, float* out_xy, uint8_t* status) {
  int rc = lk_check(ctx, prev, next, width, height, row_stride);
  if (rc) return rc;
  SVO_REQUIRE(ctx, n >= 0 && (n == 0 || (xy && out_xy && status)), "lk_track: null buffer");
  if (n == 0) return SVO_OK;
// ... 60 lines not shown
```

### stereo_vo_amd/host/group.cpp

```cpp
#include <math.h>
#include <stdio.h>
#include <stdlib.h>
#include <string.h>

#include <sched.h>

#include <algorithm>
#include <atomic>
#include <chrono>
#include <condition_variable>
#include <deque>
#include <mutex>
#include <thread>
#include <vector>

#include "chain_math.h"
#include "dense_args.h"
#include "det_trig.h"
#include "group_kernels.h"
#include "group_lines.h"
#include "ref_constants.h"
#include "svo.h"

namespace {

constexpr int GROUP_SOLVE_YIELD_DEFAULT = 8;
int group_solve_yield_default() {
  const char* e = getenv("SVO_BA_YIELD_ITERS");
  return e && *e ? std::max(0, atoi(e)) : GROUP_SOLVE_YIELD_DEFAULT;
}

enum LaneState { L_IDLE = 0, L_TRACK_WAIT, L_NEED_SOLVE, L_PNP_WAIT, L_TRI_WAIT, L_DONE };
enum BaState { BA_NONE = 0, BA_ASSEMBLING, BA_READY, BA_INFLIGHT, BA_HOST_SOLVING, BA_HOST_DONE };
enum Word { W_TRACK = 0, W_PNP, W_TRI, W_COUNT };
enum Counter { C_LK = 0, C_PNP, C_TRI, C_COUNT };
enum Stat { ST_TRACK = 0, ST_PNP, ST_HOST_US, ST_TRI, ST_SOLVE, ST_FRONT_END, ST_COUNT };

struct Lane {
  int lk_line = 0, chain_line = 0;
  float* d_xy[2] = {nullptr, nullptr}; float* d_init[2] = {nullptr, nullptr}; long long* d_ids[2] = {nullptr, nullptr};
  float* d_fwd = nullptr; float* d_par = nullptr; uint8_t* d_keep = nullptr;
  float* h_xy[2] = {nullptr, nullptr}; long long* h_ids[2] = {nullptr, nullptr};
  float* h_kf_xy = nullptr; long long* h_kf_ids = nullptr;
  int* h_n = nullptr; float* h_av = nullptr;
  int cur = 0, n = 0, n_initial = 0;
  bool from_host = false;
  const uint8_t* last_pyr = nullptr;
  const uint8_t* last_l0 = nullptr;
  uint8_t* d_own_pyr = nullptr;
  float4* d_store = nullptr; unsigned store_mask = 0;
  double* d_hyp_pose = nullptr; int* d_hyp_count = nullptr; unsigned long long* d_hyp_mask = nullptr;
  double* d_out = nullptr; int* d_nin = nullptr; int* d_inl = nullptr; float* d_trk_xy = nullptr;
  bool pnp_all = false;
  int* h_best = nullptr; int* h_bad = nullptr; double* h_out = nullptr; int* h_nin = nullptr; int* h_inl = nullptr;
  float* d_disp = nullptr;
  int* h_tri_cnt = nullptr; float* h_tri_xy = nullptr; float* h_tri_xyz = nullptr;
  int* words = nullptr;
  int seq[W_COUNT] = {};
  unsigned* d_arrive = nullptr;
  unsigned arrive_total[C_COUNT] = {0, 0, 0};
  svo_ba* ba = nullptr;
  std::atomic<int> ba_state{BA_NONE};
  svo_ba_summary ba_summary{};
  int ba_rc = 0;
  int ba_launch = 0, ba_line = 0;
  unsigned long long ba_ready_seq = 0;
  bool ba_yielded = false;
  bool has_keyframe = false;
  double solved_pose[7] = {1, 0, 0, 0, 0, 0, 0};
  int last_iterations = 0;
  float rvec[3] = {0, 0, 0}, tvec[3] = {0, 0, 0};
  int state = L_IDLE;
  bool queued = false;
  int frame = 0;
  int pending_from = -1;
  bool first_keyframe = false;
  SvoChainRec* d_chain = nullptr;
  double t_q = 0.0;
  bool fused = false;
  int m_tracked = 0, num_inliers = 0, best = -1;
  float rmat[9], quat[4];
  std::vector<long long> kf_tracked_ids; std::vector<float> kf_tracked_xy;
  std::vector<long long> ids64; std::vector<int64_t> new_ids;
};

struct Pool {
  std::vector<std::thread> th;
  std::mutex mu;
  std::condition_variable cv;
  std::deque<std::pair<Lane*, int>> jobs;
  bool quit = false;
  int device = 0;
  void start(int n, int dev) {
    device = dev;
    for (int i = 0; i < n; ++i) th.emplace_back([this] { run(); });
  }
  void post(Lane* l, int what) {
    { std::lock_guard<std::mutex> g(mu); jobs.emplace_back(l, what); }
    cv.notify_one();
  }
  void run() {
    (void)hipSetDevice(device);
    for (;;) {
      std::pair<Lane*, int> j;
      {
        std::unique_lock<std::mutex> lk(mu);
        cv.wait(lk, [this] { return quit || !jobs.empty(); });
        if (quit && jobs.empty()) return;
        j = jobs.front(); jobs.pop_front();
      }
      Lane* l = j.first;
      if (j.second == 0) {
        l->ba_rc = svo_ba_solve_prepare(l->ba);
        l->ba_state.store(BA_READY, std::memory_order_release);
      } else {
        l->ba_rc = svo_ba_solve_finish(l->ba, &l->ba_summary);
        l->ba_state.store(BA_HOST_DONE, std::memory_order_release);
      }
    }
  }
  void stop() {
    { std::lock_guard<std::mutex> g(mu); quit = true; }
    cv.notify_all();
    for (auto& t : th) t.join();
    th.clear();
  }
};

}

struct svo_pipeline_group {
  svo_ctx* ctx = nullptr;
  svo_pipeline_params prm{};
  int n_lanes = 0, max_batch = 0;
  float K[9];
  std::vector<Lane*> lanes;
  std::vector<void*> dev_allocs, pin_allocs;
  static constexpr int MAX_LINES = 8;
  int n_lk = 1, n_chain = 1, n_ba = 2;
  int n_cmp = 0;
  int xcd_chunks = SVO_XCD_CHUNKS;
  bool xcd_map = true, xcd_map_tri = true;
  double t_get_points = 0, t_add_keyframe = 0, t_finish = 0, t_loop = 0; long n_kf = 0; bool timing = false;
  double gather_us = 0.0;
  hipStream_t st_lk[MAX_LINES] = {}, st_chain[MAX_LINES] = {}, st_ba[MAX_LINES] = {};
  int ba_launch_id = 0;
  unsigned long long ba_ready_counter = 0;
  float* d_corners = nullptr; int* d_ncorners = nullptr; uint8_t* d_pyr[2] = {nullptr, nullptr}; int pyr_cur = 0;
  size_t pyr_stride = 0;
  int* h_counts = nullptr;
  Pool pool;
  int pnp_iterations = 0, mask_words_cap = 0;
  long launches[ST_COUNT] = {}, lanes_carried[ST_COUNT] = {};
  uint8_t* h_stage[2][2] = {{nullptr, nullptr}, {nullptr, nullptr}};
  uint8_t* d_stage[2][2] = {{nullptr, nullptr}, {nullptr, nullptr}};
  hipStream_t st_copy = nullptr;
  hipEvent_t ev_up[2] = {nullptr, nullptr};
  int up_batch[2] = {0, 0};
  std::vector<SvoRectModel*> rect_models;
  SvoRectModel* lane_rect[SVO_MAX_LANES] = {};
  uint8_t* d_rect[2] = {nullptr, nullptr};
  SvoKfClouds* kfc = nullptr;
  bool lane_cloud[SVO_MAX_LANES] = {};
};

namespace {

int fail(svo_pipeline_group* g, const char* what, hipError_t e) {
  g->ctx->err = std::string("pipeline group: ") + what + ": " + hipGetErrorString(e);
  return SVO_ERR_HIP;
}

template <typename T>
int dev_alloc(svo_pipeline_group* g, T** p, size_t count) {
  const hipError_t e = hipMalloc((void**)p, sizeof(T) * (count ? count : 1));
  if (e != hipSuccess) return fail(g, "hipMalloc", e);
  g->dev_allocs.push_back(*p);
  return SVO_OK;
}

int word_ready(const Lane* l, int w) { return __atomic_load_n(&l->words[16 * w], __ATOMIC_ACQUIRE) == l->seq[w]; }

SvoPublish make_pub(Lane* l, int w, int counter, int nblocks) {
  SvoPublish p;
  p.word = &l->words[16 * w];
  p.seq = ++l->seq[w];
  if (counter >= 0) {
    l->arrive_total[counter] += (unsigned)nblocks;
    p.arrive = l->d_arrive + 16 * counter;
    p.target = l->arrive_total[counter];
  }
  return p;
}

void fill_pending(Lane* l, svo_frame_result* res, int upto) {
  if (l->pending_from < 0) return;
  for (int j = l->pending_from; j < upto; ++j) {
    memcpy(res[j].pose7, l->solved_pose, sizeof(res[j].pose7));
    if (j == l->pending_from && res[j].is_keyframe) res[j].ba_iterations = l->last_iterations;
  }
  l->pending_from = -1;
}

int finish_solve(svo_pipeline_group* g, Lane* l) {
  const int st = l->ba_state.load(std::memory_order_acquire);
  l->ba_ready_seq = 0;
  l->ba_yielded = false;
  if (st == BA_NONE) return SVO_OK;
  int rc = SVO_OK;
  const auto tf0 = std::chrono::steady_clock::now();
  if (st == BA_INFLIGHT) rc = svo_ba_solve_finish(l->ba, &l->ba_summary);
  else rc = l->ba_rc;
  if (g->timing) g->t_finish += std::chrono::duration<double, std::nano>(std::chrono::steady_clock::now() - tf0).count();
  l->ba_state.store(BA_NONE, std::memory_order_release);
  if (rc) return rc;
  l->last_iterations = l->ba_summary.iterations;
  double p[7];
  if ((rc = svo_ba_get_pose(l->ba, -1, p))) return rc;
  for (int i = 0; i < 7; ++i) l->solved_pose[i] = (double)(float)p[i];
  (void)g;
  return SVO_OK;
}

void quiesce_after_error(svo_pipeline_group* g) {
  for (int i = 0; i < svo_pipeline_group::MAX_LINES; ++i) {
    if (g->st_lk[i]) (void)hipStreamSynchronize(g->st_lk[i]);
    if (g->st_chain[i]) (void)hipStreamSynchronize(g->st_chain[i]);
    if (g->st_ba[i]) (void)hipStreamSynchronize(g->st_ba[i]);
  }
  for (Lane* l : g->lanes) {
    (void)hipMemset(l->d_arrive, 0, sizeof(unsigned) * 16 * C_COUNT);
    for (int c = 0; c < C_COUNT; ++c) l->arrive_total[c] = 0;
    for (int w = 0; w < W_COUNT; ++w) { l->seq[w] = 0; l->words[16 * w] = 0; }
    if (l->h_bad) *l->h_bad = 0;
    l->fused = false; l->pnp_all = false;
    l->queued = false;
  }
  (void)hipDeviceSynchronize();
}

}

extern "C" void svo_pipeline_group_destroy(svo_pipeline_group* g) {
  if (!g) return;
  (void)hipSetDevice(g->ctx->device);
  g->pool.stop();
  for (Lane* l : g->lanes) {
    if (l->ba_state.load() == BA_INFLIGHT) { svo_ba_summary s; (void)svo_ba_solve_finish(l->ba, &s); }
  }
  if (g->timing && g->n_kf)
    fprintf(stderr, "[svo group] %d lanes, %ld keyframes; group thread per keyframe (us): get_world_points %.1f, add_keyframe %.1f, join + write-back of the solve %.1f\n",
            g->n_lanes, g->n_kf, 1e-3 * g->t_get_points / g->n_kf, 1e-3 * g->t_add_keyframe / g->n_kf, 1e-3 * g->t_finish / g->n_kf);
  (void)hipStreamSynchronize(g->ctx->stream);
  for (Lane* l : g->lanes) { if (l->ba) { svo_ba_destroy(l->ba); l->ba = nullptr; } }
  for (int i = 0; i < svo_pipeline_group::MAX_LINES; ++i) {
    if (g->st_lk[i] && g->st_lk[i] != g->ctx->stream) { (void)hipStreamSynchronize(g->st_lk[i]); (void)hipStreamDestroy(g->st_lk[i]); }
    if (g->st_chain[i]) { (void)hipStreamSynchronize(g->st_chain[i]); (void)hipStreamDestroy(g->st_chain[i]); }
    if (g->st_ba[i]) { (void)hipStreamSynchronize(g->st_ba[i]); (void)hipStreamDestroy(g->st_ba[i]); }
  }
  if (g->st_copy) { (void)hipStreamSynchronize(g->st_copy); (void)hipStreamDestroy(g->st_copy); }
  for (int sl = 0; sl < 2; ++sl) {
    if (g->ev_up[sl]) (void)hipEventDestroy(g->ev_up[sl]);
    for (int e = 0; e < 2; ++e) { if (g->h_stage[sl][e]) (void)hipHostFree(g->h_stage[sl][e]); if (g->d_stage[sl][e]) (void)hipFree(g->d_stage[sl][e]); }
  }
  for (Lane* l : g->lanes) { if (l->ba) svo_ba_destroy(l->ba); delete l; }
  svo_kfc_destroy(g->kfc);
  for (SvoRectModel* m : g->rect_models) svo_rect_model_destroy(m);
  for (int e = 0; e < 2; ++e) if (g->d_rect[e]) (void)hipFree(g->d_rect[e]);
  for (void* p : g->dev_allocs) (void)hipFree(p);
  for (void* p : g->pin_allocs) (void)hipHostFree(p);
  delete g;
}

extern "C" int svo_pipeline_group_create(svo_ctx* ctx, svo_pipeline_group** out, const svo_pipeline_params* p, int n_lanes) {
  if (!ctx || !out || !p) return SVO_ERR_INVALID;
  *out = nullptr;
  SVO_HIP_CHECK(ctx, hipSetDevice(ctx->device));
  SVO_REQUIRE(ctx, n_lanes >= 1 && n_lanes <= SVO_MAX_LANES, "pipeline_group_create: 1..64 lanes");
  SVO_REQUIRE(ctx, p->width >= 32 && p->height >= 32 && p->width <= ctx->lim.max_width && p->height <= ctx->lim.max_height,
              "pipeline_group_create: image size outside the context limits");
  SVO_REQUIRE(ctx, p->max_corners >= 4 && p->max_corners <= ctx->lim.max_corners && p->max_features >= 4 &&
                       p->max_features <= ctx->lim.max_features, "pipeline_group_create: feature counts outside the context limits");
  SVO_REQUIRE(ctx, p->window_size >= 1 && p->window_size <= 63, "pipeline_group_create: window size must be 1..63");
  SVO_REQUIRE(ctx, ctx->lim.max_batch >= n_lanes, "pipeline_group_create: svo_limits.max_batch must hold lanes x frames per call");
  {
    static std::atomic<bool> warned{false};
    const char* q = getenv("GPU_MAX_HW_QUEUES");
    const int nq = q && *q ? atoi(q) : 4;
    if (n_lanes > 4 && nq < 8 && !warned.exchange(true))
      fprintf(stderr, "[svo] pipeline group of %d lanes with GPU_MAX_HW_QUEUES=%d: its launches will share hardware queues and serialise; "
                      "export GPU_MAX_HW_QUEUES=16 before the first HIP call (INTEGRATION.md)\n", n_lanes, nq);
  }
  svo_pipeline_group* g = new svo_pipeline_group();
  g->ctx = ctx; g->prm = *p; g->n_lanes = n_lanes;
  g->max_batch = ctx->lim.max_batch / n_lanes;
  const float K[9] = {(float)p->cam.focal, 0.f, (float)p->cam.cx, 0.f, (float)p->cam.focal, (float)p->cam.cy, 0.f, 0.f, 1.f};
  memcpy(g->K, K, sizeof(K));
  g->pnp_iterations = svo_ref::PNP_ITERATIONS;
  const size_t mc = (size_t)p->max_corners, mf = (size_t)ctx->lim.max_features, B = (size_t)g->max_batch, S = (size_t)n_lanes;
  const int words = (int)((mf + 63) / 64);
  g->mask_words_cap = words;
  int rc = SVO_OK;
  auto chk = [&](hipError_t e, const char* what) { if (rc == SVO_OK && e != hipSuccess) rc = fail(g, what, e); };
  {
    auto knob = [](const char* name, int dflt, int hi) { const char* e = getenv(name); int v = e && *e ? atoi(e) : dflt; return v < 1 ? 1 : (v > hi ? hi : v); };
    g->n_lk = knob("SVO_GROUP_LK_LINES", 1, svo_pipeline_group::MAX_LINES);
    g->timing = getenv("SVO_TIMING") != nullptr;
    { const char* e = getenv("SVO_GROUP_GATHER_US"); g->gather_us = e && *e ? std::max(0.0, atof(e)) : 0.0; }
    g->n_chain = knob("SVO_GROUP_CHAIN_LINES", 2, svo_pipeline_group::MAX_LINES);
    { const char* e = getenv("SVO_GROUP_LK_XCD"); g->xcd_map = !(e && *e && atoi(e) == 0); }
    { const char* e = getenv("SVO_GROUP_TRI_XCD"); g->xcd_map_tri = !(e && *e && atoi(e) == 0); }
    { const char* e = getenv("SVO_GROUP_XCD_CHUNKS"); if (e && *e) g->xcd_chunks = std::max(8, std::min(64, atoi(e) / 8 * 8)); }
    g->n_ba = knob("SVO_GROUP_BA_LINES", 4, svo_pipeline_group::MAX_LINES);
    { const char* e = getenv("SVO_GROUP_COMPACT_LINES"); g->n_cmp = e && *e ? std::max(0, std::min(atoi(e), svo_pipeline_group::MAX_LINES - g->n_ba)) : 0; }
    g->st_lk[0] = ctx->stream;
    for (int i = 1; i < g->n_lk; ++i) chk(hipStreamCreateWithFlags(&g->st_lk[i], hipStreamNonBlocking), "stream");
    for (int i = 0; i < g->n_chain; ++i) chk(hipStreamCreateWithFlags(&g->st_chain[i], hipStreamNonBlocking), "stream");
    for (int i = 0; i < g->n_ba + g->n_cmp; ++i) chk(hipStreamCreateWithFlags(&g->st_ba[i], hipStreamNonBlocking), "stream");
  }
  g->pyr_stride = svo_k_pyramid_bytes(p->width, p->height);
  if (!rc) rc = dev_alloc(g, &g->d_corners, 2 * mc * S * B);
  if (!rc) {
    const char* e = getenv("SVO_GROUP_TOUCH");
    if (!(e && *e && atoi(e) == 0)) {
      hipStream_t order[3 * svo_pipeline_group::MAX_LINES];
      int no = 0;
      for (int i = 0; i < g->n_ba + g->n_cmp; ++i) order[no++] = g->st_ba[i];
      for (int i = 0; i < g->n_chain; ++i) order[no++] = g->st_chain[i];
      for (int i = 0; i < g->n_lk; ++i) order[no++] = g->st_lk[i];
      for (int i = 0; i < no && !rc; ++i) {
        chk(hipMemsetAsync(g->d_corners, 0, 16, order[i]), "hipMemsetAsync");
        chk(hipStreamSynchronize(order[i]), "hipStreamSynchronize");
      }
    }
  }
  if (!rc) rc = dev_alloc(g, &g->d_ncorners, S * B);
  if (!rc) rc = dev_alloc(g, &g->d_pyr[0], g->pyr_stride * S * B);
  if (!rc) rc = dev_alloc(g, &g->d_pyr[1], g->pyr_stride * S * B);
  if (!rc) {
    void* hp = nullptr;
    chk(hipHostMalloc(&hp, sizeof(int) * (S * B + 16), hipHostMallocDefault), "hipHostMalloc");
    if (hp) { g->pin_allocs.push_back(hp); g->h_counts = (int*)hp; memset(hp, 0, sizeof(int) * (S * B + 16)); }
  }
  for (int li = 0; li < n_lanes && !rc; ++li) {
    Lane* l = new Lane();
    g->lanes.push_back(l);
    for (int b = 0; b < 2 && !rc; ++b) {
      rc = dev_alloc(g, &l->d_xy[b], 2 * mf);
      if (!rc) rc = dev_alloc(g, &l->d_init[b], 2 * mf);
      if (!rc) rc = dev_alloc(g, &l->d_ids[b], mf);
    }
    if (!rc) rc = dev_alloc(g, &l->d_fwd, 2 * mf);
    if (!rc) rc = dev_alloc(g, &l->d_par, mf);
    if (!rc) rc = dev_alloc(g, &l->d_keep, mf);
    {
      size_t cap = 1, keyframes = 256;
      if (const char* e = getenv("SVO_GROUP_STORE_KEYFRAMES")) keyframes = (size_t)std::max(1, atoi(e));
      while (cap < keyframes * mf) cap <<= 1;
      l->store_mask = (unsigned)(cap - 1);
      if (!rc) rc = dev_alloc(g, &l->d_store, cap);
      if (!rc) chk(hipMemset(l->d_store, 0xFF, sizeof(float4) * cap), "hipMemset");
    }
    if (!rc) rc = dev_alloc(g, &l->d_hyp_pose, 7 * (size_t)g->pnp_iterations);
    if (!rc) rc = dev_alloc(g, &l->d_hyp_count, (size_t)g->pnp_iterations);
    if (!rc) rc = dev_alloc(g, &l->d_hyp_mask, (size_t)g->pnp_iterations * words);
    if (!rc) rc = dev_alloc(g, &l->d_out, 8);
    if (!rc) rc = dev_alloc(g, &l->d_nin, 16);
    if (!rc) rc = dev_alloc(g, &l->d_inl, mf);
    if (!rc) rc = dev_alloc(g, &l->d_trk_xy, 2 * mf);
    if (!rc) rc = dev_alloc(g, &l->d_chain, 1);
    if (!rc) rc = dev_alloc(g, &l->d_disp, mc);
    if (!rc) rc = dev_alloc(g, &l->d_own_pyr, g->pyr_stride);
    if (!rc) rc = dev_alloc(g, &l->d_arrive, 16 * C_COUNT);
    if (!rc) chk(hipMemset(l->d_arrive, 0, sizeof(unsigned) * 16 * C_COUNT), "hipMemset");
    if (rc) break;
    const size_t f2 = sizeof(float) * 2 * mf, i8 = sizeof(long long) * mf;
    size_t off = 0;
    auto take = [&](size_t bytes) { const size_t o = off; off = (off + bytes + 127) & ~(size_t)127; return o; };
    const size_t o_xy0 = take(f2), o_xy1 = take(f2), o_id0 = take(i8), o_id1 = take(i8), o_kxy = take(f2), o_kid = take(i8), o_n = take(64),
                 o_cnt = take(64), o_out = take(64), o_nin = take(64),
                 o_inl = take(sizeof(int) * mf), o_tc = take(64), o_txy = take(sizeof(float) * 2 * mc), o_txyz = take(sizeof(float) * 3 * mc),
                 o_words = take(64 * W_COUNT);
    void* hp = nullptr;
    chk(hipHostMalloc(&hp, off, hipHostMallocDefault), "hipHostMalloc");
    if (rc) break;
    g->pin_allocs.push_back(hp);
    memset(hp, 0, off);
    char* h = (char*)hp;
    l->h_xy[0] = (float*)(h + o_xy0); l->h_xy[1] = (float*)(h + o_xy1); l->h_ids[0] = (long long*)(h + o_id0); l->h_ids[1] = (long long*)(h + o_id1);
    l->h_kf_xy = (float*)(h + o_kxy); l->h_kf_ids = (long long*)(h + o_kid);
    l->h_n = (int*)(h + o_n); l->h_av = (float*)(h + o_n + 16);
    l->h_best = (int*)(h + o_cnt); l->h_bad = (int*)(h + o_cnt) + 1; l->h_out = (double*)(h + o_out); l->h_nin = (int*)(h + o_nin);
    l->h_inl = (int*)(h + o_inl); l->h_tri_cnt = (int*)(h + o_tc); l->h_tri_xy = (float*)(h + o_txy); l->h_tri_xyz = (float*)(h + o_txyz);
    l->words = (int*)(h + o_words);
    svo_ba_options opt;
    svo_ba_default_options(&opt);
    opt.max_features = p->max_features;
    opt.max_iterations = p->ba_max_iterations;
    opt.max_time_s = p->ba_max_time_s;
    const int max_obs = (p->window_size + 1) * p->max_features + 64;
    rc = svo_ba_create(ctx, &l->ba, p->window_size, &p->cam, &opt, max_obs, max_obs);
    if (!rc) rc = svo_ba_attach_store(l->ba, l->d_store, l->store_mask);
    if (!rc) rc = svo_ba_use_stream(l->ba, g->st_ba[li % g->n_ba]);
    if (!rc) rc = svo_ba_set_yield_iterations(l->ba, group_solve_yield_default());
  }
  if (rc) { svo_pipeline_group_destroy(g); return rc; }
  {
    const char* e = getenv("SVO_GROUP_WORKERS");
    int nw = e ? atoi(e) : (n_lanes < 8 ? n_lanes : 8);
    if (nw < 1) nw = 1;
    if (nw > 8) nw = 8;
    g->pool.start(nw, ctx->device);
  }
  (void)hipDeviceSynchronize();
  *out = g;
  return SVO_OK;
}

extern "C" int svo_pipeline_group_reset(svo_pipeline_group* g) {
  if (!g) return SVO_ERR_INVALID;
  (void)hipSetDevice(g->ctx->device);
  int rc_join = SVO_OK;
  for (Lane* l : g->lanes) {
    const int rcf = finish_solve(g, l);
    if (rcf && !rc_join) rc_join = rcf;
    svo_ba_reset(l->ba);
    l->has_keyframe = false; l->n = l->n_initial = 0; l->from_host = false; l->last_pyr = nullptr; l->last_l0 = nullptr; l->cur = 0;
    l->rvec[0] = l->rvec[1] = l->rvec[2] = l->tvec[0] = l->tvec[1] = l->tvec[2] = 0.f;
    l->state = L_IDLE; l->queued = false; l->pending_from = -1; l->last_iterations = 0;
    const double id7[7] = {1, 0, 0, 0, 0, 0, 0};
    memcpy(l->solved_pose, id7, sizeof(id7));
    if (l->h_bad) *l->h_bad = 0;
    l->fused = false; l->pnp_all = false;
    if (l->d_store && hipMemsetAsync(l->d_store, 0xFF, sizeof(float4) * ((size_t)l->store_mask + 1), g->ctx->stream) != hipSuccess && !rc_join) rc_join = SVO_ERR_HIP;
  }
  if (hipStreamSynchronize(g->ctx->stream) != hipSuccess && !rc_join) rc_join = SVO_ERR_HIP;
  if (rc_join) { quiesce_after_error(g); return rc_join; }
  return SVO_OK;
}

extern "C" int svo_pipeline_group_lanes(const svo_pipeline_group* g) { return g ? g->n_lanes : 0; }

extern "C" int svo_pipeline_group_get_tracked(svo_pipeline_group* g, int lane, int64_t* ids, float* xy, int capacity, int* n) {
  if (!g || !n || lane < 0 || lane >= g->n_lanes) return SVO_ERR_INVALID;
  const Lane* l = g->lanes[lane];
  *n = l->n;
  const float* sx = l->from_host ? l->h_kf_xy : l->h_xy[l->cur];
  const long long* si = l->from_host ? l->h_kf_ids : l->h_ids[l->cur];
  for (int i = 0; i < l->n && i < capacity; ++i) {
    if (ids) ids[i] = (int64_t)si[i];
    if (xy) { xy[2 * i] = sx[2 * i]; xy[2 * i + 1] = sx[2 * i + 1]; }
  }
  return SVO_OK;
}

extern "C" int svo_pipeline_group_set_solve_yield(svo_pipeline_group* g, int n) {
  if (!g || n < 0) return SVO_ERR_INVALID;
  for (Lane* l : g->lanes) {
    const int rc = svo_ba_set_yield_iterations(l->ba, n);
    if (rc) return rc;
  }
  return SVO_OK;
}

extern "C" int svo_pipeline_group_solve_work(svo_pipeline_group* g, double* out4, int reset) {
  if (!g || !out4) return SVO_ERR_INVALID;
  out4[0] = out4[1] = out4[2] = out4[3] = 0.0;
  for (Lane* l : g->lanes) {
    double w[4];
    svo_ba_work(l->ba, w, reset);
    for (int i = 0; i < 4; ++i) out4[i] += w[i];
  }
  return SVO_OK;
}

extern "C" int svo_pipeline_group_solve_forms(svo_pipeline_group* g, long* counts, int n, long* gave_up) {
  if (!g || !counts || n < 1) return SVO_ERR_INVALID;
  std::vector<long> c((size_t)n);
  for (int i = 0; i < n; ++i) counts[i] = 0;
  if (gave_up) *gave_up = 0;
  for (Lane* l : g->lanes) {
    long gu = 0;
    const int rc = svo_ba_solve_forms(l->ba, c.data(), n, &gu);
    if (rc) return rc;
    for (int i = 0; i < n; ++i) counts[i] += c[(size_t)i];
    if (gave_up) *gave_up += gu;
  }
  return SVO_OK;
}

extern "C" int svo_pipeline_group_last_stats(const svo_pipeline_group* g, long* launches6, long* lanes6) {
  if (!g || !launches6 || !lanes6) return SVO_ERR_INVALID;
  static_assert(ST_COUNT == 6, "svo_pipeline_group_last_stats returns six slots");
  for (int i = 0; i < ST_COUNT; ++i) { launches6[i] = g->launches[i]; lanes6[i] = g->lanes_carried[i]; }
  return SVO_OK;
}

namespace {
bool trace_enabled() { static const bool on = getenv("SVO_GROUP_TRACE") != nullptr; return on; }
bool chain_fused_enabled() { static const bool on = [] { const char* e = getenv("SVO_GROUP_CHAIN_FUSED"); return !(e && *e && atoi(e) == 0); }(); return on; }
bool host_solves_only() { static const bool on = [] { const char* e = getenv("SVO_GROUP_HOST_SOLVES"); return e && *e && atoi(e) != 0; }(); return on; }

struct Batch {
  using Clock = std::chrono::steady_clock;
  struct Ev { double us; int lane; const char* what; int arg; };
  static constexpr int MAX_LINES = svo_pipeline_group::MAX_LINES;

  svo_pipeline_group* const g;
  svo_ctx* const ctx;
  const uint8_t* const* const lbase;
  const uint8_t* const* const rbase;
  const int batch;
  svo_frame_result* const results;
  const int W, H, S;
  const size_t istride;
  uint8_t* pyr = nullptr;
  int* hc = nullptr;
  std::vector<int> q_track, q_pnp, q_tri, q_ba;
  int error = SVO_OK;
  const int MODEL = svo_pnp_model_points();
  const bool trace_on = trace_enabled(), chain_fused = chain_fused_enabled();
  std::vector<Ev> evs;
  Clock::time_point t_begin, t_pass, last_progress;
  bool all_done = false, progressed = false;
  bool lk_busy[MAX_LINES] = {}, chain_busy[MAX_LINES] = {}, ba_line_busy[MAX_LINES] = {};
  double t_now_us = 0.0;
  unsigned idle_spins = 0;
  double busy_us = 0.0;

  Batch(svo_pipeline_group* g_, const uint8_t* const* lb, const uint8_t* const* rb, int batch_, svo_frame_result* res)
      : g(g_), ctx(g_->ctx), lbase(lb), rbase(rb), batch(batch_), results(res), W(g_->prm.width), H(g_->prm.height), S(g_->n_lanes),
        istride((size_t)g_->prm.width * g_->prm.height) {}

  svo_frame_result& RES(int lane, int f) const { return results[(size_t)lane * batch + f]; }
  const uint8_t* IMG(const uint8_t* const* base, int lane, int f) const { return base[lane] + (size_t)f * istride; }
  uint8_t* PYR(int lane, int f) const { return pyr + ((size_t)lane * batch + f) * g->pyr_stride; }
  const uint8_t* L0(int lane, int f) const { return f == batch - 1 ? PYR(lane, f) : IMG(lbase, lane, f); }
  float* DET(int lane, int f) const { return g->d_corners + ((size_t)lane * batch + f) * 2 * g->prm.max_corners; }
  double now_us() const { return std::chrono::duration<double, std::micro>(Clock::now() - t_begin).count(); }
  void EV(int lane, const char* what, int arg) { if (trace_on) evs.push_back({now_us(), lane, what, arg}); }
  void enqueue(std::vector<int>& q, int li, int state) {
    Lane* l = g->lanes[li];
    q.push_back(li); l->queued = true; l->t_q = now_us(); l->state = state;
  }
  void count(Stat s, int lanes) { g->launches[s]++; g->lanes_carried[s] += lanes; progressed = true; }

  void frame_done(int li) {
    Lane* l = g->lanes[li];
    svo_frame_result* res = &RES(li, 0);
    const int i = l->frame;
    if (l->has_keyframe && !(res[i].is_keyframe) && l->pending_from < 0) l->pending_from = i;
    l->frame = i + 1;
    l->state = l->frame < batch ? L_IDLE : L_DONE;
  }

  int keyframe_tail(int li) {
    Lane* l = g->lanes[li];
    svo_frame_result* res = &RES(li, 0);
    const int i = l->frame;
    const int m_new = *l->h_tri_cnt;
    double pose7[7];
    if (l->first_keyframe) {
      const double id7[7] = {1, 0, 0, 0, 0, 0, 0};
      memcpy(pose7, id7, sizeof(id7));
      l->kf_tracked_ids.clear(); l->kf_tracked_xy.clear();
    } else {
      pose7[0] = l->quat[0]; pose7[1] = l->quat[1]; pose7[2] = l->quat[2]; pose7[3] = l->quat[3];
      pose7[4] = l->tvec[0]; pose7[5] = l->tvec[1]; pose7[6] = l->tvec[2];
    }
    const int nt = (int)l->kf_tracked_ids.size();
    l->new_ids.assign((size_t)(m_new > 0 ? m_new : 1), 0);
    int kept = 0;
    std::vector<int64_t> tid(l->kf_tracked_ids.begin(), l->kf_tracked_ids.end());
    const auto ta0 = Clock::now();
    int rc2 = svo_ba_add_keyframe(l->ba, pose7, tid.data(), l->kf_tracked_xy.data(), nt, l->h_tri_xy, l->h_tri_xyz, m_new, l->new_ids.data(), &kept);
    if (g->timing) { g->t_add_keyframe += std::chrono::duration<double, std::nano>(Clock::now() - ta0).count(); g->n_kf++; }
    if (rc2) return rc2;
    fill_pending(l, res, i);
    l->pending_from = i;
    l->has_keyframe = true;
    l->ba_state.store(BA_ASSEMBLING, std::memory_order_release);
    g->pool.post(l, 0);
    EV(li, "assembly_posted", i);
    int n = nt + kept;
    if (n > ctx->lim.max_features) n = ctx->lim.max_features;
    for (int k = 0; k < nt && k < n; ++k) { l->h_kf_xy[2 * k] = l->kf_tracked_xy[2 * k]; l->h_kf_xy[2 * k + 1] = l->kf_tracked_xy[2 * k + 1]; l->h_kf_ids[k] = l->kf_tracked_ids[k]; }
    for (int k = nt; k < n; ++k) { l->h_kf_xy[2 * k] = l->h_tri_xy[2 * (k - nt)]; l->h_kf_xy[2 * k + 1] = l->h_tri_xy[2 * (k - nt) + 1]; l->h_kf_ids[k] = (long long)l->new_ids[k - nt]; }
    l->n = l->n_initial = n;
    l->from_host = true;
    l->last_pyr = PYR(li, i);
    l->last_l0 = L0(li, i);
    if (l->first_keyframe) { l->tvec[0] = l->tvec[1] = l->tvec[2] = 0.f; l->rvec[0] = l->rvec[1] = l->rvec[2] = 0.f; }
    res[i].is_keyframe = 1;
    res[i].n_new = kept;
    frame_done(li);
    return SVO_OK;
  }

  int consume_pnp(int li) {
    Lane* l = g->lanes[li];
// ... 3 lines not shown
      return -1;
    }
    l->best = *l->h_best;
    if (l->best == -2) {
      l->pnp_all = true;
      enqueue(q_pnp, li, L_PNP_WAIT);
      return -1;
    }
    if (l->best >= 0) {
      double rv[3];
      svo_det_rvec_from_quat(l->h_out, rv);
      for (int k = 0; k < 3; ++k) { l->rvec[k] = (float)rv[k]; l->tvec[k] = (float)l->h_out[4 + k]; }
      l->num_inliers = *l->h_nin;
    }
    return 0;
  }

  void after_pnp(int li, bool queue_tri = true) {
    Lane* l = g->lanes[li];
    svo_frame_result* res = &RES(li, 0);
    res[l->frame].n_inliers = l->num_inliers;
    svo_det_rodrigues_f(l->rvec, l->rmat);
    svo_det_quat_from_R(l->rmat, l->quat);
    const float* txy = l->h_xy[l->cur];
    const long long* tids = l->h_ids[l->cur];
    l->kf_tracked_ids.resize(l->num_inliers); l->kf_tracked_xy.resize(2 * (size_t)l->num_inliers);
    for (int k = 0; k < l->num_inliers; ++k) {
      const int idx = l->h_inl[k];
      l->kf_tracked_ids[k] = tids[idx];
      l->kf_tracked_xy[2 * k] = txy[2 * idx]; l->kf_tracked_xy[2 * k + 1] = txy[2 * idx + 1];
    }
    l->first_keyframe = false;
    if (queue_tri) enqueue(q_tri, li, L_TRI_WAIT);
  }

  int continue_keyframe(int li) {
    Lane* l = g->lanes[li];
    const int m = l->n;
    l->m_tracked = m;
    l->num_inliers = 0; l->best = -1;
    if (m >= MODEL) enqueue(q_pnp, li, L_PNP_WAIT);
    else after_pnp(li);
    return SVO_OK;
  }

  int after_track(int li) {
    Lane* l = g->lanes[li];
    svo_frame_result& r = RES(li, l->frame);
    const float av = *l->h_av;
    const float pl = (float)(1.0 - (double)((float)l->n / (float)l->n_initial));
    r.n_tracked = l->n; r.av_parallax = av; r.percent_lost = pl;
    if (av <= g->prm.parallax_thresh && (double)pl < svo_ref::KEYFRAME_PERCENT_LOST) { frame_done(li); return SVO_OK; }
    if (l->ba_state.load(std::memory_order_acquire) != BA_NONE) { l->state = L_NEED_SOLVE; EV(li, "need_solve", l->ba_state.load()); return SVO_OK; }
    return continue_keyframe(li);
  }

  int start_frame(int li) {
    Lane* l = g->lanes[li];
    const int i = l->frame;
    svo_frame_result& r = RES(li, i);
    const int n_det = hc[li * batch + i];
    r.n_detected = n_det;
    if (n_det < svo_ref::MIN_DETECTED) { frame_done(li); return SVO_OK; }
    if (!l->has_keyframe) {
      l->first_keyframe = true;
      l->num_inliers = 0;
      enqueue(q_tri, li, L_TRI_WAIT);
      return SVO_OK;
    }
    if (l->n <= 0) {
      l->n = 0; *l->h_av = 0.f;
      return after_track(li);
    }
    enqueue(q_track, li, L_TRACK_WAIT);
    return SVO_OK;
  }

  void advance_lane(int li) {
    Lane* l = g->lanes[li];
    for (bool again = true; again && !error;) {
      again = false;
      switch (l->state) {
        case L_IDLE:
          error = start_frame(li);
          progressed = true;
          again = l->state == L_IDLE;
          break;
        case L_TRACK_WAIT:
          if (l->queued || !word_ready(l, W_TRACK)) break;
          EV(li, "track_done", l->frame);
          l->cur ^= 1; l->from_host = false;
          l->n = *l->h_n;
          l->last_pyr = PYR(li, l->frame);
          l->last_l0 = L0(li, l->frame);
          error = after_track(li);
          progressed = true; again = l->state == L_IDLE;
          break;
        case L_NEED_SOLVE:
          if (!solve_came_back(l)) break;
          EV(li, "solve_joined_for_pnp", l->frame);
          error = finish_solve(g, l);
          if (!error) error = continue_keyframe(li);
          progressed = true; again = l->state == L_IDLE;
          break;
        case L_PNP_WAIT:
          if (l->queued || !word_ready(l, W_PNP)) break;
          EV(li, "pnp_done", l->frame);
          progressed = true;
          if (consume_pnp(li) < 0) break;
          after_pnp(li, true);
          break;
        case L_TRI_WAIT:
          if (l->queued || !word_ready(l, W_TRI)) break;
          EV(li, "tri_done", l->frame);
          progressed = true;
          if (l->fused) {
            l->fused = false;
            if (consume_pnp(li) < 0) break;
            after_pnp(li, false);
          }
          error = keyframe_tail(li);
          again = l->state == L_IDLE;
          break;
        default: break;
      }
    }
  }

  int front_end() {
    const int mc = g->prm.max_corners;
    hipStream_t st = ctx->stream;
    bool tight = true;
    for (int l = 1; l < S; ++l) tight = tight && lbase[l] == lbase[0] + (size_t)l * batch * istride;
    const uint8_t* const left = lbase[0];
    const size_t lane_stride = istride * (size_t)batch;
    for (int i = 0; i < ST_COUNT; ++i) { g->launches[i] = 0; g->lanes_carried[i] = 0; }
    g->pyr_cur ^= 1;
    pyr = g->d_pyr[g->pyr_cur];
    int rc = SVO_OK;
    const uint8_t* lo = pyr;
    const uint8_t* hi = pyr + g->pyr_stride * (size_t)g->n_lanes * (size_t)g->max_batch;
    for (Lane* l : g->lanes) {
      if (!l->last_pyr || l->last_pyr < lo || l->last_pyr >= hi) continue;
      SVO_HIP_CHECK(ctx, hipMemcpyAsync(l->d_own_pyr, l->last_pyr, g->pyr_stride, hipMemcpyDeviceToDevice, ctx->stream));
      l->last_pyr = l->d_own_pyr;
      l->last_l0 = l->d_own_pyr;
    }
    if (tight) {
      rc = svo_corner_detect_batch_dev(ctx, left, S * batch, W, H, W, istride, mc, g->prm.quality, (double)g->prm.min_feature_distance, g->d_corners, g->d_ncorners);
      if (!rc) rc = svo_k_build_pyramid(ctx, left, S * batch, W, H, W, istride, pyr, g->pyr_stride, true);
      if (!rc) rc = svo_k_pyramid_level0(ctx, left + (size_t)(batch - 1) * istride, S, W, H, W, lane_stride, pyr + (size_t)(batch - 1) * g->pyr_stride,
                                         (size_t)batch * g->pyr_stride, st);
    } else {
      for (int l = 0; l < S && !rc; ++l) {
        rc = svo_corner_detect_batch_dev(ctx, lbase[l], batch, W, H, W, istride, mc, g->prm.quality, (double)g->prm.min_feature_distance,
                                         g->d_corners + (size_t)l * batch * 2 * mc, g->d_ncorners + (size_t)l * batch);
        if (!rc) rc = svo_k_build_pyramid(ctx, lbase[l], batch, W, H, W, istride, pyr + (size_t)l * batch * g->pyr_stride, g->pyr_stride, true);
        if (!rc) rc = svo_k_pyramid_level0(ctx, lbase[l] + (size_t)(batch - 1) * istride, 1, W, H, W, istride,
                                           pyr + ((size_t)l * batch + (size_t)(batch - 1)) * g->pyr_stride, g->pyr_stride, st);
      }
    }
    if (rc) return rc;
    g->launches[ST_FRONT_END] += 7; g->lanes_carried[ST_FRONT_END] += 7 * S;
    hc = g->h_counts;
    SVO_HIP_CHECK(ctx, hipMemcpyAsync(hc, g->d_ncorners, sizeof(int) * S * batch, hipMemcpyDeviceToHost, st));
    SVO_HIP_CHECK(ctx, hipMemcpyAsync(hc + S * batch, ctx->d_status, sizeof(int), hipMemcpyDeviceToHost, st));
    SVO_HIP_CHECK(ctx, hipStreamSynchronize(st));
    if (hc[S * batch]) {
      (void)hipMemsetAsync(ctx->d_status, 0, sizeof(int), st);
      ctx->err = (hc[S * batch] & 8) ? "corner detection: more raw local maxima than the streaming pass's list holds (raw_cap: width x height / 4 per image under a 1 GiB budget)"
                           : "corner detection exceeded a workspace bound (svo_limits.max_candidates)";
      return SVO_ERR_CAPACITY;
    }
    return SVO_OK;
  }

  void advance_lanes() {
    all_done = true;
    for (int li = 0; li < S && !error; ++li) {
      advance_lane(li);
      if (g->lanes[li]->state != L_DONE) all_done = false;
    }
  }

  void scan_lines() {
    for (int i = 0; i < MAX_LINES; ++i) lk_busy[i] = chain_busy[i] = false;
    for (int li = 0; li < S; ++li) {
      const Lane* l = g->lanes[li];
      if (l->queued) continue;
      lk_busy[l->lk_line] |= l->state == L_TRACK_WAIT;
      chain_busy[l->chain_line] |= l->state == L_PNP_WAIT || l->state == L_TRI_WAIT;
    }
    t_now_us = now_us();
  }
  bool ripe(const std::vector<int>& q, int line, int n_lines, int near_state) const {
    return svo_line_ripe(q, S, line, n_lines, t_now_us, g->gather_us, [&](int li) { return g->lanes[li]->t_q; },
                         [&](int li) { return g->lanes[li]->state == near_state && !g->lanes[li]->queued; });
  }

  void fill_lk_lane(Lane* l, int li, SvoLkLane& x, int workgroups) {
    const int nxt = l->cur ^ 1;
    x.pyr_prev = l->last_pyr; x.pyr_next = PYR(li, l->frame);
    x.l0_prev = l->last_l0; x.l0_next = L0(li, l->frame);
    x.xy = l->from_host ? l->h_kf_xy : l->d_xy[l->cur];
    x.init_xy = l->from_host ? l->h_kf_xy : l->d_init[l->cur];
    x.ids = l->from_host ? l->h_kf_ids : l->d_ids[l->cur];
    x.n = l->n;
    x.fwd = l->d_fwd; x.keep = l->d_keep; x.parallax = l->d_par;
    x.kept_xy = l->d_xy[nxt]; x.init_dst = l->d_init[nxt]; x.ids_dst = l->d_ids[nxt];
    x.host_xy = l->h_xy[nxt]; x.host_ids = l->h_ids[nxt]; x.host_n = l->h_n; x.host_av = l->h_av;
    l->arrive_total[C_LK] += (unsigned)workgroups;
    x.arrive = l->d_arrive + 16 * C_LK; x.arrive_target = l->arrive_total[C_LK];
    x.word = &l->words[16 * W_TRACK]; x.seq = ++l->seq[W_TRACK];
    l->queued = false;
  }

  void launch_tracking() {
    scan_lines();
    for (int line = 0; line < g->n_lk && !error; ++line) {
      if (lk_busy[line] || !ripe(q_track, line, g->n_lk, L_TRI_WAIT)) continue;
      const std::vector<int> q_now = svo_line_take(q_track, line, g->n_lk);
      if (q_now.empty()) continue;
      for (int li : q_now) g->lanes[li]->lk_line = line;
      SvoLkLanes a;
      a.w = W; a.h = H;
      int gx = 1;
      for (int li : q_now) gx = std::max(gx, g->lanes[li]->n);
      a.map.per_chunk = 0; a.map.total = 0; a.map.chunks = 0;
      if (g->xcd_map) {
        int counts[SVO_MAX_LANES], j = 0;
        for (int li : q_now) counts[j++] = g->lanes[li]->n;
        svo_xcd_map_fill(a.map, counts, j, g->xcd_chunks);
      }
      int k = 0;
      for (int li : q_now) {
        Lane* l = g->lanes[li];
        fill_lk_lane(l, li, a.lane[k++], a.map.per_chunk > 0 ? std::max(1, l->n) : gx);
      }
      if ((error = svo_kg_track(ctx, g->st_lk[line], a, k, gx))) return;
      for (int li : q_now) EV(li, "track_launch", k);
      count(ST_TRACK, k);
    }
  }

  void fill_pnp_lane(Lane* l, int li, SvoPnpLane& x) {
    (void)li;
    const int m = l->m_tracked;
    x.ids = l->d_ids[l->cur]; x.store = l->d_store; x.store_mask = l->store_mask;
    x.xy = l->d_xy[l->cur]; x.n = m;
    x.f = (double)g->K[0]; x.cx = (double)g->K[2]; x.cy = (double)g->K[5];
    const double rv[3] = {l->rvec[0], l->rvec[1], l->rvec[2]};
    svo_det_quat_from_rvec(rv, x.q0);
    for (int c = 0; c < 3; ++c) x.t0[c] = (double)l->tvec[c];
    x.thr2 = (double)svo_ref::PNP_REPROJ_ERROR * (double)svo_ref::PNP_REPROJ_ERROR;
    x.confidence = svo_ref::PNP_CONFIDENCE; x.iterations = g->pnp_iterations;
    x.launched = l->pnp_all ? g->pnp_iterations : svo_kg_pnp_first(g->pnp_iterations);
    l->pnp_all = false;
// ... 181 lines not shown
    l->ba_ready_seq = 0;
    l->ba_state.store(BA_HOST_SOLVING, std::memory_order_release);
    g->pool.post(l, 1);
    progressed = true;
  }

  bool idle_or_report() {
    if (progressed) {
      idle_spins = 0;
      last_progress = Clock::now();
      busy_us += std::chrono::duration<double, std::micro>(last_progress - t_pass).count();
      return true;
    }
    __builtin_ia32_pause();
    if (++idle_spins > 2000u && (idle_spins & 255u) == 0) sched_yield();
    if ((idle_spins & 0xFFFFu) != 0) return true;
    if (std::chrono::duration<double>(Clock::now() - last_progress).count() <= 5.0) return true;
    std::string msg = "pipeline group: no progress for 5 s; lanes (state/frame/solve):";
    for (const Lane* l : g->lanes) {
      char b[64];
      snprintf(b, sizeof(b), " %d/%d/%d%s", l->state, l->frame, l->ba_state.load(), l->queued ? "q" : "");
      msg += b;
    }
    ctx->err = msg;
    error = SVO_ERR_HIP;
    return false;
  }

  void launch_last_solve(int li) {
    Lane* l = g->lanes[li];
    for (;;) {
      const int bs = l->ba_state.load(std::memory_order_acquire);
      if (bs == BA_NONE || bs == BA_INFLIGHT || bs == BA_HOST_DONE) return;
      if (bs == BA_READY) {
        if (l->ba_rc) {
          if (l->ba_rc != 1 && !error) error = l->ba_rc;
          l->ba_state.store(BA_NONE);
          return;
        }
        svo_ba* one = l->ba;
        if (svo_ba_solve_launch(&one, 1, g->st_ba[0], nullptr) == 1) solves_departed(&li, 1, 1ull, 0, 1, "ba_launch_at_end");
        else { l->ba_rc = svo_ba_solve_finish(l->ba, &l->ba_summary); l->ba_state.store(BA_HOST_DONE); }
        return;
      }
      __builtin_ia32_pause();
      if (std::chrono::duration<double>(Clock::now() - last_progress).count() > 60.0) {
        if (!error) { error = SVO_ERR_HIP; ctx->err = "pipeline group: a bundle-adjustment worker did not come back"; }
        return;
      }
    }
  }

  void clone_last_level0() {
    hipStream_t st = ctx->stream;
    bool copied = false;
    for (int li = 0; li < S && !error; ++li) {
      Lane* l = g->lanes[li];
      if (!l->last_pyr || l->last_l0 == l->last_pyr || !l->last_l0) continue;
      if (svo_k_pyramid_level0(ctx, l->last_l0, 1, W, H, W, istride, const_cast<uint8_t*>(l->last_pyr), g->pyr_stride, st)) { error = SVO_ERR_HIP; break; }
      l->last_l0 = l->last_pyr;
      copied = true;
    }
    if (copied && hipStreamSynchronize(st) != hipSuccess && !error) { error = SVO_ERR_HIP; ctx->err = "pipeline group: pyramid clone failed"; }
  }

  int end_of_batch() {
    g->launches[ST_HOST_US] += (long)busy_us;
    g->lanes_carried[ST_HOST_US] += (long)now_us();
    for (int li = 0; li < S; ++li) {
      Lane* l = g->lanes[li];
      launch_last_solve(li);
      const int rcf = finish_solve(g, l);
      if (rcf && !error) error = rcf;
      if (l->pending_from < 0) l->pending_from = batch;
      fill_pending(l, &RES(li, 0), batch);
    }
    clone_last_level0();
    if (trace_on) {
      static std::mutex trace_mu;
      std::lock_guard<std::mutex> lk(trace_mu);
      for (const Ev& e : evs) fprintf(stderr, "[svo group] %10.1f lane %2d %-22s %d\n", e.us, e.lane, e.what, e.arg);
      fprintf(stderr, "[svo group] %10.1f end\n", now_us());
    }
    if (error) { quiesce_after_error(g); return error; }
    if (!ctx->err.empty()) return SVO_ERR_HIP;
    return SVO_OK;
  }

  int run() {
    const int rc = front_end();
    if (rc) return rc;
    for (int li = 0; li < S; ++li) {
      Lane* l = g->lanes[li];
      l->frame = 0; l->state = L_IDLE; l->queued = false; l->pending_from = -1;
      memset(&RES(li, 0), 0, sizeof(svo_frame_result) * batch);
    }
    t_begin = last_progress = Clock::now();
    for (;;) {
      progressed = false;
      t_pass = Clock::now();
      advance_lanes();
      if (!error) launch_tracking();
      if (!error) launch_chains();
      if (!error) join_finished_solves();
      if (!error) launch_solves();
      if (error || all_done || !idle_or_report()) break;
    }
    return end_of_batch();
  }
};

int group_process(svo_pipeline_group* g, const uint8_t* const* lbase, const uint8_t* const* rbase, int batch, svo_frame_result* results) {
  return Batch(g, lbase, rbase, batch, results).run();
}
}

extern "C" int svo_pipeline_group_process_batch_dev(svo_pipeline_group* g, const uint8_t* left, const uint8_t* right, size_t lane_stride,
                                                    int batch, svo_frame_result* results) {
  if (!g) return SVO_ERR_INVALID;
  svo_ctx* ctx = g->ctx;
  SVO_REQUIRE(ctx, left && right && results && batch >= 1 && batch <= g->max_batch, "pipeline_group_process_batch: bad arguments");
  const int W = g->prm.width, H = g->prm.height, S = g->n_lanes;
  const size_t istride = (size_t)W * H;
  SVO_REQUIRE(ctx, lane_stride >= istride * (size_t)batch, "pipeline_group_process_batch: lanes overlap");
  ctx->err.clear();
  SVO_HIP_CHECK(ctx, hipSetDevice(ctx->device));
  if (g->kfc) svo_kfc_clear(g->kfc);
  const uint8_t *lbase[SVO_MAX_LANES], *rbase[SVO_MAX_LANES];
  for (int l = 0; l < S; ++l) { lbase[l] = left + (size_t)l * lane_stride; rbase[l] = right + (size_t)l * lane_stride; }
  if (!g->rect_models.empty()) {
    SvoRectifyArgs a{};
    const size_t ws_lane = istride * (size_t)batch;
    a.src[0] = left; a.src[1] = right; a.dst[0] = g->d_rect[0]; a.dst[1] = g->d_rect[1];
    a.src_lane_stride = lane_stride; a.dst_lane_stride = ws_lane;
    a.src_image_stride = a.dst_image_stride = istride;
    a.src_row_stride = W; a.width = W; a.height = H; a.frames = batch; a.eyes = 2;
    for (int l = 0; l < S; ++l) {
      const SvoRectModel* m = g->lane_rect[l];
      if (!m) continue;
      a.map[a.n_active][0] = m->d_map[0]; a.map[a.n_active][1] = m->d_map[1];
      a.lane[a.n_active++] = (unsigned char)l;
      lbase[l] = g->d_rect[0] + (size_t)l * ws_lane; rbase[l] = g->d_rect[1] + (size_t)l * ws_lane;
    }
    if (a.n_active) {
      const int rc = svo_k_rectify_remap(ctx, a, ctx->stream);
      if (rc) return rc;
    }
  }
  const int rc = group_process(g, lbase, rbase, batch, results);
  if (rc || !g->kfc) return rc;
  std::vector<SvoCloudPair> pairs;
  std::vector<int> frame, lane;
  for (int l = 0; l < S; ++l) {
    if (!g->lane_cloud[l]) continue;
    for (int i = 0; i < batch; ++i)
      if (results[(size_t)l * batch + i].is_keyframe) {
        pairs.push_back({lbase[l] + (size_t)i * istride, rbase[l] + (size_t)i * istride});
        frame.push_back(i); lane.push_back(l);
      }
  }
  return svo_kfc_run(g->kfc, &g->prm.cam, pairs.data(), frame.data(), lane.data(), (int)frame.size());
}

extern "C" int svo_pipeline_group_set_keyframe_clouds(svo_pipeline_group* g, int lane, const svo_cloud_params* params, int max_keyframes_per_call) {
  if (!g) return SVO_ERR_INVALID;
  svo_ctx* ctx = g->ctx;
  SVO_REQUIRE(ctx, lane >= -1 && lane < g->n_lanes, "pipeline_group_set_keyframe_clouds: no such lane");
  SVO_HIP_CHECK(ctx, hipSetDevice(ctx->device));
  bool others = false;
  for (int l = 0; l < g->n_lanes; ++l) others = others || (g->lane_cloud[l] && lane >= 0 && l != lane);
  if (params) {
    bool same = false;
    if (g->kfc) {
      const svo_cloud_params* have = svo_kfc_params(g->kfc);
      const int want_points = kfc_max_points(params->max_points, g->prm.width, g->prm.height);
      const int want_kf = kfc_max_keyframes(max_keyframes_per_call, ctx->lim.max_batch);
      same = have->step == params->step && have->min_disparity == params->min_disparity && have->max_points == want_points &&
             svo_kfc_max_keyframes(g->kfc) == want_kf;
    }
    SVO_REQUIRE(ctx, same || !others, "pipeline_group_set_keyframe_clouds: the lanes that have clouds on share one set of parameters and one bound");
    if (!same) {
      const int rc = svo_kfc_replace(ctx, &g->kfc, params, g->prm.width, g->prm.height, max_keyframes_per_call);
      if (rc) return rc;
    }
  }
  for (int l = 0; l < g->n_lanes; ++l)
    if (lane < 0 || l == lane) g->lane_cloud[l] = params != nullptr;
  bool any = false;
  for (int l = 0; l < g->n_lanes; ++l) any = any || g->lane_cloud[l];
  if (!any) { svo_kfc_destroy(g->kfc); g->kfc = nullptr; }
  return SVO_OK;
// ... 161 lines not shown
```

Baseline: 15310 frames/s.

## Split front-end corner/pyramid work into frame chunks overlapped with lane processing

Corner detection and pyramid building for a batch are split into frame chunks through an image map passed to each kernel. Chunks run on a separate front stream, and each one records an event. Lanes start processing frames as soon as the chunk holding them arrives, instead of waiting for the whole batch's front end to finish. This adds extra launches per chunk, 2D copies of corner counts, event polling, and more complex error recovery.

```diff
diff --git a/include/svo.h b/include/svo.h
--- a/include/svo.h
+++ b/include/svo.h
@@ -403,6 +403,7 @@
 int svo_pipeline_group_solve_work(svo_pipeline_group* g, double* out4, int reset);
 int svo_pipeline_group_solve_forms(svo_pipeline_group* g, long* counts, int n, long* gave_up);
 int svo_pipeline_group_set_solve_yield(svo_pipeline_group* g, int n);
+int svo_pipeline_group_set_front_chunks(svo_pipeline_group* g, const int* sizes, int n);
 
 int svo_draw_track(const uint8_t* gray, int width, int height, int row_stride, const float* from_xy,
                    const float* to_xy, int n, uint8_t* rgb);
diff --git a/stereo_vo_amd/api.py b/stereo_vo_amd/api.py
--- a/stereo_vo_amd/api.py
+++ b/stereo_vo_amd/api.py
@@ -376,7 +376,7 @@
     "svo_pipeline_process_batch_dev", "svo_pipeline_process_batch", "svo_pipeline_get_tracked",
     "svo_pipeline_group_create", "svo_pipeline_group_destroy", "svo_pipeline_group_reset", "svo_pipeline_group_lanes",
     "svo_pipeline_group_process_batch_dev", "svo_pipeline_group_get_tracked", "svo_pipeline_group_last_stats",
-    "svo_pipeline_group_solve_work", "svo_pipeline_group_solve_forms", "svo_pipeline_group_set_solve_yield", "svo_pipeline_group_staging", "svo_pipeline_group_upload", "svo_pipeline_group_process_uploaded", "svo_pipeline_group_process_batch",
+    "svo_pipeline_group_solve_work", "svo_pipeline_group_solve_forms", "svo_pipeline_group_set_solve_yield", "svo_pipeline_group_set_front_chunks", "svo_pipeline_group_staging", "svo_pipeline_group_upload", "svo_pipeline_group_process_uploaded", "svo_pipeline_group_process_batch",
     "svo_synth_default_params", "svo_synth_render", "svo_synth_pose",
     "svo_image_read_gray", "svo_kitti_read_poses", "svo_ate_rmse", "svo_kitti_run", "svo_cholesky_solve", "svo_cholesky_solve_dev", "svo_draw_track", "svo_pipeline_draw_track",
     "svo_rectify_eye_from_camera_info", "svo_rectify_build_map", "svo_rectify_remap", "svo_rectify_remap_batch_dev",
@@ -1361,6 +1361,11 @@
     def set_solve_yield(self, n):
         self.ctx._chk(self.L.svo_pipeline_group_set_solve_yield(self.h, int(n)), "svo_pipeline_group_set_solve_yield")
 
+    def set_front_chunks(self, sizes):
+        sizes = [int(v) for v in sizes]
+        arr = (C.c_int * max(1, len(sizes)))(*sizes)
+        self.ctx._chk(self.L.svo_pipeline_group_set_front_chunks(self.h, arr, len(sizes)), "svo_pipeline_group_set_front_chunks")
+
     def solve_resumes(self):
         n = self.L.svo_ba_wave_chunks_limit() + 2
         out = (C.c_long * n)()
diff --git a/stereo_vo_amd/csrc/corner.hip b/stereo_vo_amd/csrc/corner.hip
--- a/stereo_vo_amd/csrc/corner.hip
+++ b/stereo_vo_amd/csrc/corner.hip
@@ -1,4 +1,5 @@
 #include "common.h"
+#include "front_chunks.h"
 
 namespace {
 constexpr int SEL_THREADS = 1024;
@@ -145,9 +146,9 @@
 __global__ __launch_bounds__(256) void corner_response_nms_kernel(const uint8_t* __restrict__ imgs, int W, int H, int row_stride,
                                                                   size_t image_stride, unsigned* __restrict__ maxkey, double quality,
                                                                   unsigned long long* __restrict__ raw, size_t raw_stride ,
-                                                                  int* __restrict__ ncand, int* __restrict__ status) {
+                                                                  int* __restrict__ ncand, int* __restrict__ status, SvoFrontMap map) {
   __shared__ unsigned long long sBuf[4][RN_BUF];
-  const int b = blockIdx.z;
+  const int b = svo_front_image(map, (int)blockIdx.z);
   const uint8_t* img = imgs + (size_t)b * image_stride;
   const int lane = threadIdx.x & 63, wave = __builtin_amdgcn_readfirstlane(threadIdx.x >> 6);
   const int ncs = (W + RN_COLS - 1) / RN_COLS, nrs = (H + RS_ROWS - 1) / RS_ROWS;
@@ -291,8 +292,8 @@
 __global__ __launch_bounds__(256) void corner_threshold_kernel(const unsigned long long* __restrict__ raw, size_t raw_stride,
                                                                const unsigned* __restrict__ maxkey, double quality,
                                                                unsigned long long* __restrict__ cand, int* __restrict__ ncand, int cap,
-                                                               int* __restrict__ status) {
-  const int b = blockIdx.z;
+                                                               int* __restrict__ status, SvoFrontMap map) {
+  const int b = svo_front_image(map, (int)blockIdx.z);
   const int n = min(ncand[b * NC_STRIDE + NC_RAW], (int)raw_stride);
   const float thr = (float)((double)key_f32(maxkey[b]) * quality);
   __shared__ int sCount, sBase;
@@ -378,12 +379,12 @@
     const unsigned long long* __restrict__ cand, const int* __restrict__ ncand, int cap, int W, int H,
     float min_distance, int max_corners, int* __restrict__ cell_count, int* __restrict__ cell_start, int max_cells,
     unsigned long long* __restrict__ sorted, uint8_t* __restrict__ state_g, float* __restrict__ out_xy,
-    int* __restrict__ out_n, int* __restrict__ status) {
+    int* __restrict__ out_n, int* __restrict__ status, SvoFrontMap map) {
   extern __shared__ __align__(16) unsigned char lds_raw[];
   unsigned long long* sKeys = reinterpret_cast<unsigned long long*>(lds_raw);
   __shared__ int sPart[SEL_THREADS];
   __shared__ int sFlag, sCount;
-  const int b = blockIdx.x, tid = threadIdx.x;
+  const int b = svo_front_image(map, (int)blockIdx.x), tid = threadIdx.x;
   const unsigned long long* C = cand + (size_t)b * cap;
   int n = ncand[b * NC_STRIDE];
   if (n > cap) n = cap;
@@ -650,23 +651,36 @@
   if (tid == 0) out_n[b] = m;
 }
 
-static int corner_launch(svo_ctx* ctx, const uint8_t* imgs, int batch, int W, int H, int row_stride,
-                         size_t image_stride, int max_corners, double quality, double min_distance,
-                         float* xy, int* n) {
+static bool corner_two_pass() {
+  static const bool on = [] { const char* e = getenv("SVO_CORNER_TWO_PASS"); return e && *e && atoi(e) != 0; }();
+  return on;
+}
+bool svo_k_corner_chunkable() { return !corner_two_pass(); }
+
+int svo_k_corner_clear(svo_ctx* ctx, int n_images) {
+  hipStream_t st = ctx->stream;
+  SVO_HIP_CHECK(ctx, hipMemsetAsync(ctx->d_maxkey, 0, sizeof(unsigned) * n_images, st));
+  SVO_HIP_CHECK(ctx, hipMemsetAsync(ctx->d_ncand, 0, sizeof(int) * NC_STRIDE * n_images, st));
+  return SVO_OK;
+}
+
+int svo_k_corner_chunk(svo_ctx* ctx, const uint8_t* imgs, SvoFrontMap map, int lanes, int W, int H, int row_stride,
+                       size_t image_stride, int max_corners, double quality, double min_distance, float* xy, int* n) {
   SVO_REQUIRE(ctx, W <= 65535 && H <= 65535, "corner_detect: image sides above 65535 (candidate keys pack y << 16 | x)");
+  SVO_REQUIRE(ctx, lanes >= 1 && map.fc >= 1 && map.f0 >= 0 && map.f0 + map.fc <= map.batch && (long long)lanes * map.batch <= ctx->lim.max_batch,
+              "corner_detect: image map outside the batch");
   hipStream_t st = ctx->stream;
-  SVO_HIP_CHECK(ctx, hipMemsetAsync(ctx->d_maxkey, 0, sizeof(unsigned) * batch, st));
-  SVO_HIP_CHECK(ctx, hipMemsetAsync(ctx->d_ncand, 0, sizeof(int) * NC_STRIDE * batch, st));
-  static const bool two_pass = [] { const char* e = getenv("SVO_CORNER_TWO_PASS"); return e && *e && atoi(e) != 0; }();
-  if (two_pass) {
+  const int items = lanes * map.fc;
+  if (corner_two_pass()) {
+    SVO_REQUIRE(ctx, map.f0 == 0 && map.fc == map.batch, "corner_detect: the two-pass form takes whole batches only");
     { const int rce = svo_ensure_eig(ctx, (size_t)ctx->lim.max_batch); if (rce) return rce; }
     {
       SvoProfScope prof(ctx, SVO_PROF_CORNER_RESPONSE);
-      hipLaunchKernelGGL(corner_response_kernel, dim3(svo_div_up(svo_div_up(W, RS_COLS) * svo_div_up(H, RS_ROWS), 4), 1, batch), dim3(256), 0, st,
+      hipLaunchKernelGGL(corner_response_kernel, dim3(svo_div_up(svo_div_up(W, RS_COLS) * svo_div_up(H, RS_ROWS), 4), 1, items), dim3(256), 0, st,
                          imgs, W, H, row_stride, image_stride, ctx->d_eig, ctx->d_maxkey);
     }
     SvoProfScope prof(ctx, SVO_PROF_CORNER_NMS);
-    hipLaunchKernelGGL(corner_nms_kernel, dim3(svo_div_up(W, 64), svo_div_up(H, 4 * NMS_ROWS), batch), dim3(256), 0, st,
+    hipLaunchKernelGGL(corner_nms_kernel, dim3(svo_div_up(W, 64), svo_div_up(H, 4 * NMS_ROWS), items), dim3(256), 0, st,
                        ctx->d_eig, W, H, ctx->d_maxkey, quality, ctx->d_cand, ctx->d_ncand, ctx->lim.max_candidates,
                        ctx->d_status);
   } else {
@@ -674,12 +688,12 @@
     const size_t raw_stride = ctx->raw_cap;
     {
       SvoProfScope prof(ctx, SVO_PROF_CORNER_RESPONSE);
-      hipLaunchKernelGGL(corner_response_nms_kernel, dim3(svo_div_up(svo_div_up(W, RN_COLS) * svo_div_up(H, RS_ROWS), 4), 1, batch), dim3(256), 0, st,
-                         imgs, W, H, row_stride, image_stride, ctx->d_maxkey, quality, raw, raw_stride, ctx->d_ncand, ctx->d_status);
+      hipLaunchKernelGGL(corner_response_nms_kernel, dim3(svo_div_up(svo_div_up(W, RN_COLS) * svo_div_up(H, RS_ROWS), 4), 1, items), dim3(256), 0, st,
+                         imgs, W, H, row_stride, image_stride, ctx->d_maxkey, quality, raw, raw_stride, ctx->d_ncand, ctx->d_status, map);
     }
     SvoProfScope prof(ctx, SVO_PROF_CORNER_NMS);
-    hipLaunchKernelGGL(corner_threshold_kernel, dim3(32, 1, batch), dim3(256), 0, st, raw, raw_stride, ctx->d_maxkey, quality, ctx->d_cand,
-                       ctx->d_ncand, ctx->lim.max_candidates, ctx->d_status);
+    hipLaunchKernelGGL(corner_threshold_kernel, dim3(32, 1, items), dim3(256), 0, st, raw, raw_stride, ctx->d_maxkey, quality, ctx->d_cand,
+                       ctx->d_ncand, ctx->lim.max_candidates, ctx->d_status, map);
   }
   static bool attr_set = false;
   if (!attr_set) {
@@ -688,12 +702,21 @@
     attr_set = true;
   }
   SvoProfScope ps(ctx, SVO_PROF_CORNER_SELECT);
-  hipLaunchKernelGGL(corner_select_kernel, dim3(batch), dim3(SEL_THREADS), SEL_LDS_BYTES, st, ctx->d_cand,
+  hipLaunchKernelGGL(corner_select_kernel, dim3(items), dim3(SEL_THREADS), SEL_LDS_BYTES, st, ctx->d_cand,
                      ctx->d_ncand, ctx->lim.max_candidates, W, H, (float)min_distance, max_corners,
                      ctx->d_cell_count, ctx->d_cell_start, ctx->max_cells, ctx->d_sorted, ctx->d_state, xy, n,
-                     ctx->d_status);
+                     ctx->d_status, map);
   SVO_HIP_CHECK(ctx, hipGetLastError());
   return SVO_OK;
+}
+
+static int corner_launch(svo_ctx* ctx, const uint8_t* imgs, int batch, int W, int H, int row_stride,
+                         size_t image_stride, int max_corners, double quality, double min_distance,
+                         float* xy, int* n) {
+  SVO_REQUIRE(ctx, W <= 65535 && H <= 65535, "corner_detect: image sides above 65535 (candidate keys pack y << 16 | x)");
+  const int rc = svo_k_corner_clear(ctx, batch);
+  if (rc) return rc;
+  return svo_k_corner_chunk(ctx, imgs, svo_front_identity(batch), 1, W, H, row_stride, image_stride, max_corners, quality, min_distance, xy, n);
 }
 
 static int corner_check_args(svo_ctx* ctx, const void* img, int batch, int W, int H, int row_stride,
diff --git a/stereo_vo_amd/csrc/kernels.h b/stereo_vo_amd/csrc/kernels.h
--- a/stereo_vo_amd/csrc/kernels.h
+++ b/stereo_vo_amd/csrc/kernels.h
@@ -1,6 +1,7 @@
 #ifndef SVO_KERNELS_H_
 #define SVO_KERNELS_H_
 #include "common.h"
+#include "front_chunks.h"
 
 struct SvoMat4 { float m[16]; };
 
@@ -19,6 +20,14 @@
                         size_t image_stride, uint8_t* pyr, size_t pyr_stride, bool level0_in_place = false);
 int svo_k_pyramid_level0(svo_ctx* ctx, const uint8_t* imgs, int batch, int w, int h, int row_stride, size_t image_stride, uint8_t* pyr,
                          size_t pyr_stride, hipStream_t st);
+int svo_k_build_pyramid_mapped(svo_ctx* ctx, const uint8_t* imgs, SvoFrontMap map, int lanes, int w, int h, int row_stride, size_t image_stride,
+                               uint8_t* pyr, size_t pyr_stride, bool level0_in_place);
+int svo_k_pyramid_level0_mapped(svo_ctx* ctx, const uint8_t* imgs, SvoFrontMap map, int lanes, int w, int h, int row_stride, size_t image_stride,
+                                uint8_t* pyr, size_t pyr_stride, hipStream_t st);
+bool svo_k_corner_chunkable();
+int svo_k_corner_clear(svo_ctx* ctx, int n_images);
+int svo_k_corner_chunk(svo_ctx* ctx, const uint8_t* imgs, SvoFrontMap map, int lanes, int W, int H, int row_stride, size_t image_stride,
+                       int max_corners, double quality, double min_distance, float* xy, int* n);
 struct SvoTrackCarry {
   const float* init_src = nullptr; const long long* ids_src = nullptr;
   float* init_dst = nullptr; long long* ids_dst = nullptr;
diff --git a/stereo_vo_amd/csrc/lk.hip b/stereo_vo_amd/csrc/lk.hip
--- a/stereo_vo_amd/csrc/lk.hip
+++ b/stereo_vo_amd/csrc/lk.hip
@@ -475,18 +475,20 @@
 }
 
 __global__ __launch_bounds__(256) void pyr_copy_kernel(const uint8_t* __restrict__ imgs, int w, int h, int row_stride,
-                                                       size_t image_stride, uint8_t* __restrict__ pyr, size_t pyr_stride) {
+                                                       size_t image_stride, uint8_t* __restrict__ pyr, size_t pyr_stride, SvoFrontMap map) {
   const int x = blockIdx.x * 64 + (threadIdx.x & 63), y = blockIdx.y * 4 + (threadIdx.x >> 6);
   if (x >= w || y >= h) return;
-  pyr[(size_t)blockIdx.z * pyr_stride + (size_t)y * w + x] = imgs[(size_t)blockIdx.z * image_stride + (size_t)y * row_stride + x];
+  const int b = svo_front_image(map, (int)blockIdx.z);
+  pyr[(size_t)b * pyr_stride + (size_t)y * w + x] = imgs[(size_t)b * image_stride + (size_t)y * row_stride + x];
 }
 
 __global__ __launch_bounds__(256) void pyr_down_kernel(uint8_t* __restrict__ pyr, size_t pyr_stride, size_t src_off, int sw,
                                                        int sh, size_t dst_off, int dw, int dh, const uint8_t* __restrict__ src_imgs,
-                                                       size_t src_image_stride, int src_row_stride) {
+                                                       size_t src_image_stride, int src_row_stride, SvoFrontMap map) {
   const int x = blockIdx.x * 64 + (threadIdx.x & 63), y = blockIdx.y * 4 + (threadIdx.x >> 6);
   if (x >= dw || y >= dh) return;
-  const uint8_t* src = src_imgs ? src_imgs + (size_t)blockIdx.z * src_image_stride : pyr + (size_t)blockIdx.z * pyr_stride + src_off;
+  const int b = svo_front_image(map, (int)blockIdx.z);
+  const uint8_t* src = src_imgs ? src_imgs + (size_t)b * src_image_stride : pyr + (size_t)b * pyr_stride + src_off;
   const int k[5] = {1, 4, 6, 4, 1};
   int s = 0;
 #pragma unroll
@@ -497,7 +499,7 @@
     for (int i = 0; i < 5; ++i) r += k[i] * row[reflect101(2 * x + i - 2, sw)];
     s += k[j] * r;
   }
-  pyr[(size_t)blockIdx.z * pyr_stride + dst_off + (size_t)y * dw + x] = (uint8_t)((s + 128) >> 8);
+  pyr[(size_t)b * pyr_stride + dst_off + (size_t)y * dw + x] = (uint8_t)((s + 128) >> 8);
 }
 
 constexpr int PB_T1W = 128, PB_T1H = 64;
@@ -506,14 +508,15 @@
 constexpr int PB_R2W = PB_T1W / 2 + 3, PB_R2H = PB_T1H / 2 + 3;
 constexpr int PB_P0 = 280, PB_P1 = 140, PB_P2 = 68;
 __global__ __launch_bounds__(256) void pyr_build_kernel(const uint8_t* __restrict__ imgs, size_t image_stride, int row_stride, int w0, int h0,
-                                                        uint8_t* __restrict__ pyr, size_t pyr_stride, int tiles_x, int tiles_y, int n_images) {
+                                                        uint8_t* __restrict__ pyr, size_t pyr_stride, int tiles_x, int tiles_y, int n_images, SvoFrontMap map) {
   __shared__ __align__(16) uint8_t s0[PB_R0H * PB_P0];
   __shared__ __align__(16) uint8_t s1[PB_R1H * PB_P1];
   __shared__ __align__(16) uint8_t s2[PB_R2H * PB_P2];
   const int per_img = tiles_x * tiles_y, total = per_img * n_images;
   const int per_xcd = (total + 7) >> 3, v = ((int)blockIdx.x & 7) * per_xcd + ((int)blockIdx.x >> 3);
   if (v >= total) return;
-  const int img = v / per_img, t = v - img * per_img, ty = t / tiles_x, tx = t - ty * tiles_x;
+  const int item = v / per_img, t = v - item * per_img, ty = t / tiles_x, tx = t - ty * tiles_x;
+  const int img = svo_front_image(map, item);
   const int w1 = (w0 + 1) >> 1, h1 = (h0 + 1) >> 1, w2 = (w1 + 1) >> 1, h2 = (h1 + 1) >> 1, w3 = (w2 + 1) >> 1, h3 = (h2 + 1) >> 1;
   const int x0lo = max(0, 2 * PB_T1W * tx - 14), x0hi = min(w0 - 1, 2 * PB_T1W * tx + 2 * PB_T1W + 6);
   const int y0lo = max(0, 2 * PB_T1H * ty - 14), y0hi = min(h0 - 1, 2 * PB_T1H * ty + 2 * PB_T1H + 6);
@@ -780,10 +783,17 @@
 
 int svo_k_build_pyramid(svo_ctx* ctx, const uint8_t* imgs, int batch, int w, int h, int row_stride, size_t image_stride,
                         uint8_t* pyr, size_t pyr_stride, bool level0_in_place) {
+  return svo_k_build_pyramid_mapped(ctx, imgs, svo_front_identity(batch), 1, w, h, row_stride, image_stride, pyr, pyr_stride, level0_in_place);
+}
+
+int svo_k_build_pyramid_mapped(svo_ctx* ctx, const uint8_t* imgs, SvoFrontMap map, int lanes, int w, int h, int row_stride, size_t image_stride,
+                               uint8_t* pyr, size_t pyr_stride, bool level0_in_place) {
+  SVO_REQUIRE(ctx, lanes >= 1 && map.fc >= 1 && map.f0 >= 0 && map.f0 + map.fc <= map.batch, "build_pyramid: image map outside the batch");
+  const int batch = lanes * map.fc;
   hipStream_t st = ctx->stream;
   if (!level0_in_place)
     hipLaunchKernelGGL(pyr_copy_kernel, dim3(svo_div_up(w, 64), svo_div_up(h, 4), batch), dim3(256), 0, st, imgs, w, h,
-                       row_stride, image_stride, pyr, pyr_stride);
+                       row_stride, image_stride, pyr, pyr_stride, map);
   static const bool per_level = [] { const char* e = getenv("SVO_PYR_PER_LEVEL"); return e && *e && atoi(e) != 0; }();
   if (LEVELS == 4 && !per_level && w >= 64 && h >= 64) {
     const int w1 = (w + 1) / 2, h1 = (h + 1) / 2, tiles_x = svo_div_up(w1, PB_T1W), tiles_y = svo_div_up(h1, PB_T1H);
@@ -791,7 +801,7 @@
     if (total > 0 && total < (1ll << 30)) {
       SvoProfScope prof(ctx, SVO_PROF_PYR_DOWN);
       hipLaunchKernelGGL(pyr_build_kernel, dim3((unsigned)(8 * ((total + 7) / 8))), dim3(256), 0, st, imgs, image_stride, row_stride, w, h, pyr, pyr_stride,
-                         tiles_x, tiles_y, batch);
+                         tiles_x, tiles_y, batch, map);
       SVO_HIP_CHECK(ctx, hipGetLastError());
       return SVO_OK;
     }
@@ -804,7 +814,7 @@
     SvoProfScope prof(ctx, SVO_PROF_PYR_DOWN);
     const bool from_images = level0_in_place && l == 1;
     hipLaunchKernelGGL(pyr_down_kernel, dim3(svo_div_up(dw, 64), svo_div_up(dh, 4), batch), dim3(256), 0, st, pyr, pyr_stride,
-                       src_off, sw, sh, dst_off, dw, dh, from_images ? imgs : (const uint8_t*)nullptr, image_stride, row_stride);
+                       src_off, sw, sh, dst_off, dw, dh, from_images ? imgs : (const uint8_t*)nullptr, image_stride, row_stride, map);
     src_off = dst_off; sw = dw; sh = dh;
   }
   SVO_HIP_CHECK(ctx, hipGetLastError());
@@ -813,8 +823,13 @@
 
 int svo_k_pyramid_level0(svo_ctx* ctx, const uint8_t* imgs, int batch, int w, int h, int row_stride, size_t image_stride, uint8_t* pyr,
                          size_t pyr_stride, hipStream_t st) {
-  hipLaunchKernelGGL(pyr_copy_kernel, dim3(svo_div_up(w, 64), svo_div_up(h, 4), batch), dim3(256), 0, st, imgs, w, h, row_stride, image_stride,
-                     pyr, pyr_stride);
+  return svo_k_pyramid_level0_mapped(ctx, imgs, svo_front_identity(batch), 1, w, h, row_stride, image_stride, pyr, pyr_stride, st);
+}
+int svo_k_pyramid_level0_mapped(svo_ctx* ctx, const uint8_t* imgs, SvoFrontMap map, int lanes, int w, int h, int row_stride, size_t image_stride,
+                                uint8_t* pyr, size_t pyr_stride, hipStream_t st) {
+  SVO_REQUIRE(ctx, lanes >= 1 && map.fc >= 1 && map.f0 >= 0 && map.f0 + map.fc <= map.batch, "pyramid_level0: image map outside the batch");
+  hipLaunchKernelGGL(pyr_copy_kernel, dim3(svo_div_up(w, 64), svo_div_up(h, 4), lanes * map.fc), dim3(256), 0, st, imgs, w, h, row_stride, image_stride,
+                     pyr, pyr_stride, map);
   SVO_HIP_CHECK(ctx, hipGetLastError());
   return SVO_OK;
 }
diff --git a/stereo_vo_amd/host/front_chunks.h b/stereo_vo_amd/host/front_chunks.h
--- /dev/null
+++ b/stereo_vo_amd/host/front_chunks.h
@@ -0,0 +1,55 @@
+#ifndef SVO_FRONT_CHUNKS_H_
+#define SVO_FRONT_CHUNKS_H_
+#include <stdlib.h>
+
+#if defined(__HIPCC__)
+#define SVO_FRONT_HD __host__ __device__ inline
+#else
+#define SVO_FRONT_HD inline
+#endif
+
+constexpr int SVO_FRONT_MAX_CHUNKS = 8;
+
+struct SvoFrontSpec {
+  int n = 0;
+  int size[SVO_FRONT_MAX_CHUNKS - 1] = {};
+};
+
+struct SvoFrontPlan {
+  int n = 0;
+  int f0[SVO_FRONT_MAX_CHUNKS] = {}, f1[SVO_FRONT_MAX_CHUNKS] = {};
+};
+
+inline SvoFrontPlan svo_front_plan(int batch, const SvoFrontSpec& spec) {
+  SvoFrontPlan p;
+  int f = 0;
+  for (int i = 0; i < spec.n && i < SVO_FRONT_MAX_CHUNKS - 1 && f < batch; ++i) {
+    const int want = spec.size[i] < 1 ? 1 : spec.size[i];
+    const int take = want < batch - f ? want : batch - f;
+    p.f0[p.n] = f; p.f1[p.n] = f + take; ++p.n;
+    f += take;
+  }
+  if (f < batch) { p.f0[p.n] = f; p.f1[p.n] = batch; ++p.n; }
+  return p;
+}
+
+inline SvoFrontSpec svo_front_spec_parse(const char* s) {
+  SvoFrontSpec spec;
+  while (s && *s && spec.n < SVO_FRONT_MAX_CHUNKS - 1) {
+    char* end = nullptr;
+    const long v = strtol(s, &end, 10);
+    if (end == s) break;
+    if (v >= 1) spec.size[spec.n++] = v > 1000000 ? 1000000 : (int)v;
+    s = end;
+    while (*s == ',' || *s == ' ') ++s;
+  }
+  return spec;
+}
+
+struct SvoFrontMap {
+  int f0, fc, batch;
+};
+SVO_FRONT_HD int svo_front_image(const SvoFrontMap& m, int j) { return (j / m.fc) * m.batch + m.f0 + j % m.fc; }
+inline SvoFrontMap svo_front_identity(int n_images) { return SvoFrontMap{0, n_images, n_images}; }
+
+#endif
diff --git a/stereo_vo_amd/host/group.cpp b/stereo_vo_amd/host/group.cpp
--- a/stereo_vo_amd/host/group.cpp
+++ b/stereo_vo_amd/host/group.cpp
@@ -17,6 +17,7 @@
 #include "chain_math.h"
 #include "dense_args.h"
 #include "det_trig.h"
+#include "front_chunks.h"
 #include "group_kernels.h"
 #include "group_lines.h"
 #include "ref_constants.h"
@@ -28,6 +29,12 @@
 int group_solve_yield_default() {
   const char* e = getenv("SVO_BA_YIELD_ITERS");
   return e && *e ? std::max(0, atoi(e)) : GROUP_SOLVE_YIELD_DEFAULT;
+}
+
+constexpr const char* GROUP_FRONT_CHUNKS_DEFAULT = "4";
+SvoFrontSpec group_front_chunks_default() {
+  static const SvoFrontSpec spec = [] { const char* e = getenv("SVO_GROUP_FRONT_CHUNKS"); return svo_front_spec_parse(e && *e ? e : GROUP_FRONT_CHUNKS_DEFAULT); }();
+  return spec;
 }
 
 enum LaneState { L_IDLE = 0, L_TRACK_WAIT, L_NEED_SOLVE, L_PNP_WAIT, L_TRI_WAIT, L_DONE };
@@ -142,6 +149,7 @@
   int xcd_chunks = SVO_XCD_CHUNKS;
   bool xcd_map = true, xcd_map_tri = true;
   double t_get_points = 0, t_add_keyframe = 0, t_finish = 0, t_loop = 0; long n_kf = 0; bool timing = false;
+  double t_front = 0, t_call = 0; long n_calls = 0;
   double gather_us = 0.0;
   hipStream_t st_lk[MAX_LINES] = {}, st_chain[MAX_LINES] = {}, st_ba[MAX_LINES] = {};
   int ba_launch_id = 0;
@@ -149,6 +157,10 @@
   float* d_corners = nullptr; int* d_ncorners = nullptr; uint8_t* d_pyr[2] = {nullptr, nullptr}; int pyr_cur = 0;
   size_t pyr_stride = 0;
   int* h_counts = nullptr;
+  SvoFrontSpec front_spec = group_front_chunks_default();
+  hipEvent_t ev_chunk[SVO_FRONT_MAX_CHUNKS] = {};
+  hipStream_t st_front = nullptr;
+  hipEvent_t ev_front_gate = nullptr;
   Pool pool;
   int pnp_iterations = 0, mask_words_cap = 0;
   long launches[ST_COUNT] = {}, lanes_carried[ST_COUNT] = {};
@@ -228,6 +240,7 @@
     if (g->st_chain[i]) (void)hipStreamSynchronize(g->st_chain[i]);
     if (g->st_ba[i]) (void)hipStreamSynchronize(g->st_ba[i]);
   }
+  if (g->st_front) (void)hipStreamSynchronize(g->st_front);
   for (Lane* l : g->lanes) {
     (void)hipMemset(l->d_arrive, 0, sizeof(unsigned) * 16 * C_COUNT);
     for (int c = 0; c < C_COUNT; ++c) l->arrive_total[c] = 0;
@@ -251,6 +264,9 @@
   if (g->timing && g->n_kf)
     fprintf(stderr, "[svo group] %d lanes, %ld keyframes; group thread per keyframe (us): get_world_points %.1f, add_keyframe %.1f, join + write-back of the solve %.1f\n",
             g->n_lanes, g->n_kf, 1e-3 * g->t_get_points / g->n_kf, 1e-3 * g->t_add_keyframe / g->n_kf, 1e-3 * g->t_finish / g->n_kf);
+  if (g->timing && g->n_calls)
+    fprintf(stderr, "[svo group] %d lanes, %ld batch calls; wall time per call (ms): front end until the main loop starts %.3f, whole call %.3f (%.1f %%)\n",
+            g->n_lanes, g->n_calls, 1e-6 * g->t_front / g->n_calls, 1e-6 * g->t_call / g->n_calls, 100.0 * g->t_front / g->t_call);
   (void)hipStreamSynchronize(g->ctx->stream);
   for (Lane* l : g->lanes) { if (l->ba) { svo_ba_destroy(l->ba); l->ba = nullptr; } }
   for (int i = 0; i < svo_pipeline_group::MAX_LINES; ++i) {
@@ -259,6 +275,9 @@
     if (g->st_ba[i]) { (void)hipStreamSynchronize(g->st_ba[i]); (void)hipStreamDestroy(g->st_ba[i]); }
   }
   if (g->st_copy) { (void)hipStreamSynchronize(g->st_copy); (void)hipStreamDestroy(g->st_copy); }
+  for (hipEvent_t e : g->ev_chunk) if (e) (void)hipEventDestroy(e);
+  if (g->ev_front_gate) (void)hipEventDestroy(g->ev_front_gate);
+  if (g->st_front) { (void)hipStreamSynchronize(g->st_front); (void)hipStreamDestroy(g->st_front); }
   for (int sl = 0; sl < 2; ++sl) {
     if (g->ev_up[sl]) (void)hipEventDestroy(g->ev_up[sl]);
     for (int e = 0; e < 2; ++e) { if (g->h_stage[sl][e]) (void)hipHostFree(g->h_stage[sl][e]); if (g->d_stage[sl][e]) (void)hipFree(g->d_stage[sl][e]); }
@@ -317,17 +336,19 @@
     for (int i = 1; i < g->n_lk; ++i) chk(hipStreamCreateWithFlags(&g->st_lk[i], hipStreamNonBlocking), "stream");
     for (int i = 0; i < g->n_chain; ++i) chk(hipStreamCreateWithFlags(&g->st_chain[i], hipStreamNonBlocking), "stream");
     for (int i = 0; i < g->n_ba + g->n_cmp; ++i) chk(hipStreamCreateWithFlags(&g->st_ba[i], hipStreamNonBlocking), "stream");
+    { const char* e = getenv("SVO_GROUP_FRONT_STREAM"); if (!(e && *e && atoi(e) == 0)) { chk(hipStreamCreateWithFlags(&g->st_front, hipStreamNonBlocking), "stream"); chk(hipEventCreateWithFlags(&g->ev_front_gate, hipEventDisableTiming), "hipEventCreate"); } }
   }
   g->pyr_stride = svo_k_pyramid_bytes(p->width, p->height);
   if (!rc) rc = dev_alloc(g, &g->d_corners, 2 * mc * S * B);
   if (!rc) {
     const char* e = getenv("SVO_GROUP_TOUCH");
     if (!(e && *e && atoi(e) == 0)) {
-      hipStream_t order[3 * svo_pipeline_group::MAX_LINES];
+      hipStream_t order[3 * svo_pipeline_group::MAX_LINES + 1];
       int no = 0;
       for (int i = 0; i < g->n_ba + g->n_cmp; ++i) order[no++] = g->st_ba[i];
       for (int i = 0; i < g->n_chain; ++i) order[no++] = g->st_chain[i];
       for (int i = 0; i < g->n_lk; ++i) order[no++] = g->st_lk[i];
+      if (g->st_front) order[no++] = g->st_front;
       for (int i = 0; i < no && !rc; ++i) {
         chk(hipMemsetAsync(g->d_corners, 0, 16, order[i]), "hipMemsetAsync");
         chk(hipStreamSynchronize(order[i]), "hipStreamSynchronize");
@@ -341,6 +362,8 @@
     void* hp = nullptr;
     chk(hipHostMalloc(&hp, sizeof(int) * (S * B + 16), hipHostMallocDefault), "hipHostMalloc");
     if (hp) { g->pin_allocs.push_back(hp); g->h_counts = (int*)hp; memset(hp, 0, sizeof(int) * (S * B + 16)); }
+    static_assert(SVO_FRONT_MAX_CHUNKS <= 16, "one status slot per chunk behind the counts");
+    for (hipEvent_t& e : g->ev_chunk) chk(hipEventCreateWithFlags(&e, hipEventDisableTiming), "hipEventCreate");
   }
   for (int li = 0; li < n_lanes && !rc; ++li) {
     Lane* l = new Lane();
@@ -463,6 +486,17 @@
   return SVO_OK;
 }
 
+extern "C" int svo_pipeline_group_set_front_chunks(svo_pipeline_group* g, const int* sizes, int n) {
+  if (!g || n < 0 || n > SVO_FRONT_MAX_CHUNKS - 1 || (n > 0 && !sizes)) return SVO_ERR_INVALID;
+  SvoFrontSpec spec;
+  for (int i = 0; i < n; ++i) {
+    if (sizes[i] < 1) return SVO_ERR_INVALID;
+    spec.size[spec.n++] = sizes[i];
+  }
+  g->front_spec = spec;
+  return SVO_OK;
+}
+
 extern "C" int svo_pipeline_group_solve_work(svo_pipeline_group* g, double* out4, int reset) {
   if (!g || !out4) return SVO_ERR_INVALID;
   out4[0] = out4[1] = out4[2] = out4[3] = 0.0;
@@ -516,6 +550,9 @@
   const size_t istride;
   uint8_t* pyr = nullptr;
   int* hc = nullptr;
+  SvoFrontPlan plan;
+  int chunks_done = 0;
+  int frames_ready = 0;
   std::vector<int> q_track, q_pnp, q_tri, q_ba;
   int error = SVO_OK;
   const int MODEL = svo_pnp_model_points();
@@ -685,6 +722,7 @@
       again = false;
       switch (l->state) {
         case L_IDLE:
+          if (l->frame >= frames_ready) break;
           error = start_frame(li);
           progressed = true;
           again = l->state == L_IDLE;
@@ -736,7 +774,6 @@
     bool tight = true;
     for (int l = 1; l < S; ++l) tight = tight && lbase[l] == lbase[0] + (size_t)l * batch * istride;
     const uint8_t* const left = lbase[0];
-    const size_t lane_stride = istride * (size_t)batch;
     for (int i = 0; i < ST_COUNT; ++i) { g->launches[i] = 0; g->lanes_carried[i] = 0; }
     g->pyr_cur ^= 1;
     pyr = g->d_pyr[g->pyr_cur];
@@ -749,33 +786,83 @@
       l->last_pyr = l->d_own_pyr;
       l->last_l0 = l->d_own_pyr;
     }
-    if (tight) {
-      rc = svo_corner_detect_batch_dev(ctx, left, S * batch, W, H, W, istride, mc, g->prm.quality, (double)g->prm.min_feature_distance, g->d_corners, g->d_ncorners);
-      if (!rc) rc = svo_k_build_pyramid(ctx, left, S * batch, W, H, W, istride, pyr, g->pyr_stride, true);
-      if (!rc) rc = svo_k_pyramid_level0(ctx, left + (size_t)(batch - 1) * istride, S, W, H, W, lane_stride, pyr + (size_t)(batch - 1) * g->pyr_stride,
-                                         (size_t)batch * g->pyr_stride, st);
-    } else {
-      for (int l = 0; l < S && !rc; ++l) {
-        rc = svo_corner_detect_batch_dev(ctx, lbase[l], batch, W, H, W, istride, mc, g->prm.quality, (double)g->prm.min_feature_distance,
-                                         g->d_corners + (size_t)l * batch * 2 * mc, g->d_ncorners + (size_t)l * batch);
-        if (!rc) rc = svo_k_build_pyramid(ctx, lbase[l], batch, W, H, W, istride, pyr + (size_t)l * batch * g->pyr_stride, g->pyr_stride, true);
-        if (!rc) rc = svo_k_pyramid_level0(ctx, lbase[l] + (size_t)(batch - 1) * istride, 1, W, H, W, istride,
-                                           pyr + ((size_t)l * batch + (size_t)(batch - 1)) * g->pyr_stride, g->pyr_stride, st);
-      }
+    hc = g->h_counts;
+    if (tight) return front_end_chunks(left);
+    plan = svo_front_plan(batch, SvoFrontSpec());
+    for (int l = 0; l < S && !rc; ++l) {
+      rc = svo_corner_detect_batch_dev(ctx, lbase[l], batch, W, H, W, istride, mc, g->prm.quality, (double)g->prm.min_feature_distance,
+                                       g->d_corners + (size_t)l * batch * 2 * mc, g->d_ncorners + (size_t)l * batch);
+      if (!rc) rc = svo_k_build_pyramid(ctx, lbase[l], batch, W, H, W, istride, pyr + (size_t)l * batch * g->pyr_stride, g->pyr_stride, true);
+      if (!rc) rc = svo_k_pyramid_level0(ctx, lbase[l] + (size_t)(batch - 1) * istride, 1, W, H, W, istride,
+                                         pyr + ((size_t)l * batch + (size_t)(batch - 1)) * g->pyr_stride, g->pyr_stride, st);
     }
     if (rc) return rc;
     g->launches[ST_FRONT_END] += 7; g->lanes_carried[ST_FRONT_END] += 7 * S;
-    hc = g->h_counts;
     SVO_HIP_CHECK(ctx, hipMemcpyAsync(hc, g->d_ncorners, sizeof(int) * S * batch, hipMemcpyDeviceToHost, st));
-    SVO_HIP_CHECK(ctx, hipMemcpyAsync(hc + S * batch, ctx->d_status, sizeof(int), hipMemcpyDeviceToHost, st));
+    SVO_HIP_CHECK(ctx, hipMemcpyAsync(chunk_status(0), ctx->d_status, sizeof(int), hipMemcpyDeviceToHost, st));
     SVO_HIP_CHECK(ctx, hipStreamSynchronize(st));
-    if (hc[S * batch]) {
-      (void)hipMemsetAsync(ctx->d_status, 0, sizeof(int), st);
-      ctx->err = (hc[S * batch] & 8) ? "corner detection: more raw local maxima than the streaming pass's list holds (raw_cap: width x height / 4 per image under a 1 GiB budget)"
-                           : "corner detection exceeded a workspace bound (svo_limits.max_candidates)";
+    return chunk_arrived();
+  }
+
+  int* chunk_status(int c) const { return hc + (size_t)S * g->max_batch + c; }
+  int front_end_chunks(const uint8_t* left) {
+    const int mc = g->prm.max_corners;
+    plan = svo_front_plan(batch, svo_k_corner_chunkable() ? g->front_spec : SvoFrontSpec());
+    struct Swap {
+      svo_ctx* c; hipStream_t saved;
+      Swap(svo_ctx* c_, hipStream_t s) : c(c_), saved(c_->stream) { if (s) c->stream = s; }
+      ~Swap() { c->stream = saved; }
+    };
+    const bool own_line = g->st_front && plan.n > 1;
+    if (own_line) {
+      SVO_HIP_CHECK(ctx, hipEventRecord(g->ev_front_gate, ctx->stream));
+      SVO_HIP_CHECK(ctx, hipStreamWaitEvent(g->st_front, g->ev_front_gate, 0));
+    }
+    Swap swap(ctx, own_line ? g->st_front : nullptr);
+    hipStream_t st = ctx->stream;
+    int rc = svo_k_corner_clear(ctx, S * batch);
+    for (int c = 0; c < plan.n && !rc; ++c) {
+      const SvoFrontMap map{plan.f0[c], plan.f1[c] - plan.f0[c], batch};
+      rc = svo_k_corner_chunk(ctx, left, map, S, W, H, W, istride, mc, g->prm.quality, (double)g->prm.min_feature_distance, g->d_corners, g->d_ncorners);
+      if (!rc) rc = svo_k_build_pyramid_mapped(ctx, left, map, S, W, H, W, istride, pyr, g->pyr_stride, true);
+      if (!rc && c == plan.n - 1) rc = svo_k_pyramid_level0_mapped(ctx, left, SvoFrontMap{batch - 1, 1, batch}, S, W, H, W, istride, pyr, g->pyr_stride, st);
+      if (rc) break;
+      hipError_t e;
+      if (plan.n == 1) e = hipMemcpyAsync(hc, g->d_ncorners, sizeof(int) * S * batch, hipMemcpyDeviceToHost, st);
+      else e = hipMemcpy2DAsync(hc + map.f0, sizeof(int) * batch, g->d_ncorners + map.f0, sizeof(int) * batch, sizeof(int) * map.fc, (size_t)S, hipMemcpyDeviceToHost, st);
+      if (e == hipSuccess) e = hipMemcpyAsync(chunk_status(c), ctx->d_status, sizeof(int), hipMemcpyDeviceToHost, st);
+      if (e == hipSuccess) e = hipEventRecord(g->ev_chunk[c], st);
+      if (e != hipSuccess) rc = fail(g, "front-end chunk", e);
+    }
+    g->launches[ST_FRONT_END] += 3 + 4 * plan.n; g->lanes_carried[ST_FRONT_END] += (3 + 4 * plan.n) * S;
+    if (rc) { (void)hipStreamSynchronize(st); (void)hipMemsetAsync(ctx->d_status, 0, sizeof(int), st); return rc; }
+    const hipError_t e = plan.n == 1 ? hipStreamSynchronize(st) : hipEventSynchronize(g->ev_chunk[0]);
+    if (e != hipSuccess) { (void)hipStreamSynchronize(st); return fail(g, "front-end wait", e); }
+    rc = chunk_arrived();
+    if (rc) (void)hipStreamSynchronize(st);
+    if (rc) (void)hipMemsetAsync(ctx->d_status, 0, sizeof(int), st);
+    return rc;
+  }
+
+  int chunk_arrived() {
+    const int status = *chunk_status(chunks_done);
+    if (status) {
+      (void)hipMemsetAsync(ctx->d_status, 0, sizeof(int), ctx->stream);
+      ctx->err = (status & 8) ? "corner detection: more raw local maxima than the streaming pass's list holds (raw_cap: width x height / 4 per image under a 1 GiB budget)"
+                              : "corner detection exceeded a workspace bound (svo_limits.max_candidates)";
       return SVO_ERR_CAPACITY;
     }
+    frames_ready = plan.f1[chunks_done++];
     return SVO_OK;
+  }
+
+  void poll_chunks() {
+    if (chunks_done >= plan.n) return;
+    const hipError_t e = hipEventQuery(g->ev_chunk[chunks_done]);
+    if (e == hipErrorNotReady) return;
+    if (e != hipSuccess) { error = fail(g, "front-end chunk", e); return; }
+    error = chunk_arrived();
+    progressed = true;
   }
 
   void advance_lanes() {
@@ -1123,13 +1210,19 @@
       for (const Ev& e : evs) fprintf(stderr, "[svo group] %10.1f lane %2d %-22s %d\n", e.us, e.lane, e.what, e.arg);
       fprintf(stderr, "[svo group] %10.1f end\n", now_us());
     }
-    if (error) { quiesce_after_error(g); return error; }
+    if (error) {
+      quiesce_after_error(g);
+      if (chunks_done < plan.n) (void)hipMemsetAsync(ctx->d_status, 0, sizeof(int), ctx->stream);
+      return error;
+    }
     if (!ctx->err.empty()) return SVO_ERR_HIP;
     return SVO_OK;
   }
 
   int run() {
+    const auto t_run0 = Clock::now();
     const int rc = front_end();
+    if (g->timing) g->t_front += std::chrono::duration<double, std::nano>(Clock::now() - t_run0).count();
     if (rc) return rc;
     for (int li = 0; li < S; ++li) {
       Lane* l = g->lanes[li];
@@ -1140,14 +1233,17 @@
     for (;;) {
       progressed = false;
       t_pass = Clock::now();
-      advance_lanes();
+      poll_chunks();
+      if (!error) advance_lanes();
       if (!error) launch_tracking();
       if (!error) launch_chains();
       if (!error) join_finished_solves();
       if (!error) launch_solves();
       if (error || all_done || !idle_or_report()) break;
     }
-    return end_of_batch();
+    const int rc_end = end_of_batch();
+    if (g->timing) { g->t_call += std::chrono::duration<double, std::nano>(Clock::now() - t_run0).count(); g->n_calls++; }
+    return rc_end;
   }
 };
 
```

Result: faster. 15700 frames/s (median of 6 runs) (+2.6%).
